# feldroop/floxer

Hardware: AMD Instinct MI355X
Metric: aligned reads/sec, 10 kb ONT-like reads @ 8 % error vs a GRCh38-size reference (seed-and-verify path, CIGAR) (higher is better)
Workload: dtype u64

## Files before the change

floxer_amd/__init__.py:

```python
import ctypes as C

import numpy as np

from . import capi
from .capi import FloxerError, check, lib, ptr, as_u8, u8p, u32p, u64p

if capi.os.path.exists(capi.LIB_PATH):
    lib()

CIGAR_OPS = "MIDNSHP=X"
NULL_ID = 0xFFFFFFFF

ORDER = {"errors_first": 0, "count_first": 1, "none": 2}
CHOICE = {"round_robin": 0, "full_groups": 1, "first_reported": 2}
MODE_EXISTS, MODE_WITHOUT_CIGAR, MODE_WITH_CIGAR = 0, 1, 2


def hw_queue_request():
    requested, found = C.c_int(0), C.c_int(-1)
    check(lib().flx_hw_queue_request(C.byref(requested), C.byref(found)))
    return requested.value, found.value


def cigar_string(words):
# ... 21 lines not shown

def reverse_complement_rank(r):
    r = as_u8(r)
    out = np.zeros_like(r)
    lib().flx_reverse_complement_rank(ptr(r, u8p), len(r), ptr(out, u8p))
    return out


class pex_tree:

    def __init__(self, total_query_length, query_num_errors, leaf_max_num_errors, bottom_up=False):
        cap = 4 * (query_num_errors + 2) + 16
        nodes = (capi.PexNode * cap)()
        ni, nl = C.c_uint64(), C.c_uint64()
        check(lib().flx_pex_tree_build(total_query_length, query_num_errors, leaf_max_num_errors, int(bottom_up), nodes, cap,
                                       C.byref(ni), C.byref(nl)))
        rows = [(n.parent_id, n.from_, n.to, n.num_errors) for n in nodes[: ni.value + nl.value]]
        self.inner_nodes = rows[: ni.value]
        self.leaves = rows[ni.value:]

    def root(self):
        return self.inner_nodes[0] if self.inner_nodes else self.leaves[0]

    def get_leaves(self):
        return self.leaves

    def generate_seeds(self, step=1):
        return [(l[1], l[2] - l[1] + 1, l[3], i) for i, l in enumerate(self.leaves)][::step]


class fmindex:
    def __init__(self, references=None, path=None, device=None):
        self.h = C.c_void_p()
        if path is not None and references is None:
            check(lib().flx_index_load(path.encode(), C.byref(self.h)))
        else:
            refs = [as_u8(r) for r in references]
            pool = np.concatenate(refs) if refs else np.zeros(0, np.uint8)
            lens = np.array([len(r) for r in refs], dtype=np.uint64)
            if device is None:
                check(lib().flx_index_build(ptr(pool, u8p), ptr(lens, u64p), len(refs), C.byref(self.h)))
            else:
                check(lib().flx_index_build_on_device(int(device), ptr(pool, u8p), ptr(lens, u64p), len(refs), C.byref(self.h)))

    def save(self, path):
        check(lib().flx_index_save(self.h, path.encode()))

    def meta(self):
        n = C.c_uint64(0)
        lib().flx_index_meta_export(self.h, None, C.byref(n))
        buf = np.zeros(n.value, dtype=np.uint8)
        check(lib().flx_index_meta_export(self.h, ptr(buf, u8p), C.byref(n)))
        return buf.tobytes()

    @classmethod
    def from_meta(cls, meta):
        self = cls.__new__(cls)
        self.h = C.c_void_p()
        buf = np.frombuffer(meta, dtype=np.uint8).copy()
        check(lib().flx_index_meta_import(ptr(buf, u8p), len(buf), C.byref(self.h)))
        return self

    def image_layout(self):
        out = np.zeros(5, dtype=np.uint64)
        check(lib().flx_index_image_layout(self.h, ptr(out, u64p)))
        return [int(x) for x in out]

    def image_upload(self, device, pointers):
        arr = (C.c_void_p * 5)(*[C.c_void_p(int(p)) for p in pointers])
        check(lib().flx_index_image_upload(self.h, int(device), arr))

    def __del__(self):
        if getattr(self, "h", None):
            lib().flx_index_free(self.h)
            self.h = None

    @property
    def text_length(self):
        return lib().flx_index_text_length(self.h)

    @property
    def num_references(self):
        return lib().flx_index_num_references(self.h)

    @property
    def device_bytes(self):
        return lib().flx_index_device_bytes(self.h)

    @property
    def derived_device_bytes(self):
        return lib().flx_index_derived_device_bytes(self.h)

    def suffix_array(self):
        out = np.zeros(self.text_length, dtype=np.uint64)
        check(lib().flx_index_copy_sa(self.h, ptr(out, u64p)))
        return out

    def suffix_array_u32(self):
        out = np.empty(self.text_length, dtype=np.uint32)
        check(lib().flx_index_copy_sa_u32(self.h, ptr(out, u32p)))
        return out

    def bwt(self, reversed_text=False):
        out = np.zeros(self.text_length, dtype=np.uint8)
        check(lib().flx_index_copy_bwt(self.h, int(reversed_text), ptr(out, u8p)))
        return out


class context:

    def __init__(self, index, device=0, image=None):
        self.index = index
        self.image = image
        self.h = C.c_void_p()
        if image is None:
            check(lib().flx_ctx_create(device, index.h, C.byref(self.h)))
        else:
            arr = (C.c_void_p * 5)(*[C.c_void_p(int(b.data_ptr())) for b in image])
            sizes = np.array([int(b.numel()) * int(b.element_size()) for b in image], dtype=np.uint64)
            check(lib().flx_ctx_create_on_image(device, index.h, arr, ptr(sizes, u64p), C.byref(self.h)))

    def close(self):
        if getattr(self, "h", None):
            lib().flx_ctx_destroy(self.h)
            self.h = None

    __del__ = close

    def set_stream(self, hip_stream):
        check(lib().flx_ctx_set_stream(self.h, hip_stream))

    def enable_kernel_timing(self, on=True):
        check(lib().flx_ctx_enable_kernel_timing(self.h, int(on)))

    def reset_kernel_stats(self):
        check(lib().flx_ctx_reset_kernel_stats(self.h))

    def path_counters(self, reset=False):
        pc = capi.PathCounters()
        check(lib().flx_ctx_get_path_counters(self.h, C.byref(pc)))
        if reset:
            check(lib().flx_ctx_reset_path_counters(self.h))
        out = {n: int(getattr(pc, n)) for n, _ in capi.PathCounters._fields_ if n != "reserved"}
        out["records_dropped"] = int(pc.reserved[0])
        out["partial_records"] = int(pc.reserved[1])
        out["reads_rescued"] = int(pc.reserved[2])
        out["reads_split"] = int(pc.reserved[3])
        return out

    def search_counters(self):
        sc = capi.SearchCounters()
        check(lib().flx_ctx_get_search_counters(self.h, C.byref(sc)))
        return {n: int(getattr(sc, n)) for n, _ in capi.SearchCounters._fields_ if n != "reserved"}

    def derived_info(self):
        di = capi.DerivedInfo()
        check(lib().flx_ctx_derived_info(self.h, C.byref(di)))
        return {n: int(getattr(di, n)) for n, _ in capi.DerivedInfo._fields_ if n != "reserved"}

    def copy_derived(self, which):
        if which == "isa":
            out = np.empty(self.index.text_length, dtype=np.uint32)
        else:
            out = np.empty((4 ** self.derived_info()["filter_k"] + 63) // 64, dtype=np.uint64)
        check(lib().flx_ctx_copy_derived(self.h, {"isa": 0, "filter": 1, "filter_mirrored": 2}[which], out.ctypes.data_as(C.c_void_p), out.nbytes))
        return out

    def lane_overlap(self, n_lanes, iterations):
        start, stop = (C.c_float * n_lanes)(), (C.c_float * n_lanes)()
        check(lib().flx_ctx_lane_overlap(self.h, n_lanes, iterations, start, stop))
        return list(start), list(stop)

    def kernel_stats(self):
        arr = (capi.KernelStat * 64)()
        n = C.c_uint32(64)
        check(lib().flx_ctx_get_kernel_stats(self.h, arr, C.byref(n)))
        return {a.name.decode(): dict(launches=a.launches, device_ms=a.device_ms, algorithmic_bytes=a.algorithmic_bytes,
                                      work_units=a.work_units) for a in arr[: n.value]}


class statistics:

    def __init__(self, input_hint=None):
        self.h = C.c_void_p()
        check(lib().flx_stats_create(input_hint.encode() if input_hint else None, C.byref(self.h)))

    def __del__(self):
        if getattr(self, "h", None):
            lib().flx_stats_free(self.h)
            self.h = None

    def attach(self, ctx):
        check(lib().flx_ctx_set_stats(ctx.h, self.h))
        return self

    @property
    def num_queries(self):
        return lib().flx_stats_num_queries(self.h)

    def format(self, toml=True):
        n = C.c_uint64(0)
        lib().flx_stats_format(self.h, int(toml), None, C.byref(n))
        buf = C.create_string_buffer(n.value)
        check(lib().flx_stats_format(self.h, int(toml), buf, C.byref(n)))
        return buf.value.decode()


def search_config(max_num_anchors_hard=500, max_num_anchors_soft=50, anchor_group_order="count_first",
                  anchor_choice_strategy="round_robin", erase_useless_anchors=True):
    return capi.SearchConfig(max_num_anchors_hard, max_num_anchors_soft, ORDER[anchor_group_order], CHOICE[anchor_choice_strategy],
                             int(erase_useless_anchors), 0)


class searcher:
    def __init__(self, ctx, config=None):
        self.ctx = ctx
        self.config = config or search_config()

    def _seeds(self, seeds):
        arr = (capi.Seed * len(seeds))()
        for i, (off, ln, err, leaf) in enumerate(seeds):
            arr[i] = capi.Seed(off, ln, err, leaf, 0)
        return arr

    def search_seeds(self, sequence, seeds):
        seq = as_u8(sequence)
        arr = self._seeds(seeds)
        cap = max(64, len(seeds) * (self.config.max_num_anchors_soft + 1))
        out = (capi.Anchor * cap)()
        n = C.c_uint64(cap)
        stats = (capi.SeedStats * max(1, len(seeds)))()
        check(lib().flx_search_seeds(self.ctx.h, ptr(seq, u8p), len(seq), arr, len(seeds), C.byref(self.config), out, C.byref(n), stats))
        anchors = np.array([(a.seed_index, a.pex_leaf_index, a.reference_id, a.reference_position, a.num_errors) for a in out[: n.value]],
                           dtype=np.uint64).reshape(-1, 5)
        st = np.array([(s.num_kept_useful_anchors, s.num_kept_raw_anchors, s.num_excluded_raw_anchors_by_soft_cap, s.fully_excluded)
                       for s in stats[: len(seeds)]], dtype=np.uint64).reshape(-1, 4)
        return anchors, st

    def search_groups(self, sequence, seeds, max_hits=501):
        seq = as_u8(sequence)
        arr = self._seeds(seeds)
        cap = 1 << 16
        while True:
            out = (capi.HitGroup * cap)()
            n = C.c_uint64(cap)
            rc = lib().flx_search_groups(self.ctx.h, ptr(seq, u8p), len(seq), arr, len(seeds), max_hits, out, C.byref(n))
            if rc == -3:
                cap = n.value
                continue
            check(rc)
            break
        return np.array([(g.seed_index, g.lb, g.len, g.num_errors) for g in out[: n.value]], dtype=np.uint64).reshape(-1, 4)


def align_batch(ctx, query_pool, jobs, reference_pool=None, md=False, gaps=None):
    q = as_u8(query_pool)
    arr = (capi.AlignJob * max(1, len(jobs)))()
    cap_words = 16
    for i, (ro, rl, qo, ql, k, mode) in enumerate(jobs):
        arr[i] = capi.AlignJob(ro, qo, rl, ql, k, mode)
        cap_words += 2 * k + 2
    res = (capi.AlignResult * max(1, len(jobs)))()
    cig = np.zeros(cap_words, dtype=np.uint32)
    words = C.c_uint64(cap_words)
    if reference_pool is None:
        rp, rl_ = None, 0
    else:
        ref = as_u8(reference_pool)
        rp, rl_ = ptr(ref, u8p), len(ref)
    if md:
        cap_md = 16 + sum(8 * k + 6 for (_, _, _, _, k, mode) in jobs if mode == MODE_WITH_CIGAR)
        refs = (capi.MdRef * max(1, len(jobs)))()
        mdp = np.zeros(cap_md, dtype=np.uint8)
        md_bytes = C.c_uint64(cap_md)
        if gaps is not None:
            check(lib().flx_align_batch_gaps(ctx.h, rp, rl_, ptr(q, u8p), len(q), arr, len(jobs), res, ptr(cig, u32p), C.byref(words),
                                             refs, ptr(mdp, u8p), C.byref(md_bytes), C.byref(gaps)))
        else:
            check(lib().flx_align_batch_md(ctx.h, rp, rl_, ptr(q, u8p), len(q), arr, len(jobs), res, ptr(cig, u32p), C.byref(words),
                                           refs, ptr(mdp, u8p), C.byref(md_bytes)))
        out = []
        for r, m in zip(res[: len(jobs)], refs[: len(jobs)]):
            out.append((r.num_errors, r.begin, cigar_string(cig[r.cigar_offset: r.cigar_offset + r.cigar_length]),
                        mdp[m.offset: m.offset + m.length].tobytes() if m.length else None) if r.exists else None)
        return out
    if gaps is not None:
        check(lib().flx_align_batch_gaps(ctx.h, rp, rl_, ptr(q, u8p), len(q), arr, len(jobs), res, ptr(cig, u32p), C.byref(words),
                                         None, None, None, C.byref(gaps)))
    else:
        check(lib().flx_align_batch(ctx.h, rp, rl_, ptr(q, u8p), len(q), arr, len(jobs), res, ptr(cig, u32p), C.byref(words)))
    out = []
    for r in res[: len(jobs)]:
        out.append((r.num_errors, r.begin, cigar_string(cig[r.cigar_offset: r.cigar_offset + r.cigar_length])) if r.exists else None)
    return out


def _realign_room(options):
    if options is None or not options.enable:
        return (lambda nm: 2 * nm + 2), (lambda nm: 8 * nm + 6)
    sc = {k: int(getattr(options, k)) or v for k, v in REALIGN_DEFAULTS.items()}
    c_max = max(sc["match"] + sc["mismatch"], sc["gap_open"] + sc["gap_extend"] + sc["match"])
    c_min = min(sc["match"] + sc["mismatch"], sc["gap_open"] + sc["gap_extend"])
    col_min = min(sc["match"] + sc["mismatch"], sc["gap_extend"])
    return (lambda nm: max(2 * nm + 2, 2 * (nm * c_max // c_min) + 1)), (lambda nm: 8 * (nm * c_max // col_min) + 6)


# ... 1395 lines not shown
```

floxer_amd/capi.py:

```python
import ctypes as C
import importlib.util
import os
import sys

import numpy as np

_HERE = os.path.dirname(os.path.abspath(__file__))
LIB_PATH = os.environ.get("FLX_LIBRARY") or os.path.join(_HERE, "libfloxer_amd.so")

u8p = C.POINTER(C.c_uint8)
u32p = C.POINTER(C.c_uint32)
u64p = C.POINTER(C.c_uint64)


class FloxerError(RuntimeError):
    pass


class PexNode(C.Structure):
    _fields_ = [("parent_id", C.c_uint32), ("from_", C.c_uint32), ("to", C.c_uint32), ("num_errors", C.c_uint32)]


class Seed(C.Structure):
    _fields_ = [("seq_offset", C.c_uint64), ("length", C.c_uint32), ("num_errors", C.c_uint32), ("pex_leaf_index", C.c_uint32),
# ... 100 lines not shown
    _fields_ = [("offset", C.c_uint64), ("length", C.c_uint32), ("num_errors", C.c_uint32), ("score", C.c_int32), ("diag_lo", C.c_int32),
                ("diag_hi", C.c_int32), ("kept", C.c_uint32)]


class RealignCounters(C.Structure):
    _fields_ = [("paths_realigned", C.c_uint64), ("paths_changed", C.c_uint64), ("paths_kept", C.c_uint64), ("reserved", C.c_uint64 * 5)]


class CsOptions(C.Structure):
    _fields_ = [("form", C.c_uint32), ("reserved", C.c_uint32 * 7)]


CsJob = LeftAlignJob


class CoverageOptions(C.Structure):
    _fields_ = [("count_deletions", C.c_uint32), ("count_secondary", C.c_uint32), ("min_mapq", C.c_uint32), ("report_zero", C.c_uint32),
                ("reserved", C.c_uint32 * 4)]


class DepthRun(C.Structure):
    _fields_ = [("reference_id", C.c_int32), ("depth", C.c_uint32), ("start", C.c_uint64), ("end", C.c_uint64)]


class DepthWindow(C.Structure):
    _fields_ = [("reference_id", C.c_int32), ("max_depth", C.c_uint32), ("start", C.c_uint64), ("end", C.c_uint64), ("depth_sum", C.c_uint64),
                ("covered", C.c_uint64)]


class PileupOptions(C.Structure):
    _fields_ = [("count_secondary", C.c_uint32), ("min_mapq", C.c_uint32), ("min_depth", C.c_uint32), ("min_count", C.c_uint32),
                ("min_permille", C.c_uint32), ("reserved", C.c_uint32 * 3)]


class PileupSite(C.Structure):
    _fields_ = [("reference_id", C.c_int32), ("position", C.c_uint32), ("depth", C.c_uint32), ("del_", C.c_uint32), ("ins", C.c_uint32),
                ("alt", C.c_uint32 * 4), ("reserved", C.c_uint32)]


class SvOptions(C.Structure):
    _fields_ = [("min_length", C.c_uint32), ("max_distance", C.c_uint32), ("min_support", C.c_uint32), ("count_secondary", C.c_uint32),
                ("min_mapq", C.c_uint32), ("reserved", C.c_uint32 * 3), ("initial_capacity", C.c_uint64)]


class SvSignature(C.Structure):
    _fields_ = [("type", C.c_uint32), ("side_a", C.c_uint32), ("side_b", C.c_uint32), ("reserved", C.c_uint32), ("ref_a", C.c_int32),
                ("ref_b", C.c_int32), ("pos_a", C.c_uint32), ("q", C.c_uint32)]


class SvCluster(C.Structure):
    _fields_ = [("type", C.c_uint32), ("side_a", C.c_uint32), ("side_b", C.c_uint32), ("support", C.c_uint32), ("ref_a", C.c_int32),
                ("ref_b", C.c_int32), ("pos_a_min", C.c_uint32), ("pos_a_max", C.c_uint32), ("q_min", C.c_uint32), ("q_median", C.c_uint32),
                ("q_max", C.c_uint32), ("reserved", C.c_uint32)]


class ErrprofOptions(C.Structure):
    _fields_ = [("count_secondary", C.c_uint32), ("min_mapq", C.c_uint32), ("flush_threshold", C.c_uint32), ("reserved", C.c_uint32 * 5)]


class ConsensusOptions(C.Structure):
    _fields_ = [("count_secondary", C.c_uint32), ("min_mapq", C.c_uint32), ("min_depth", C.c_uint32), ("min_count", C.c_uint32),
                ("min_permille", C.c_uint32), ("mask_low_depth", C.c_uint32), ("reserved", C.c_uint32 * 2)]


class ConsensusChange(C.Structure):
    _fields_ = [("reference_id", C.c_int32), ("position", C.c_uint32), ("kind", C.c_uint32), ("ref_rank", C.c_uint32), ("alt_rank", C.c_uint32),
                ("length", C.c_uint32), ("count", C.c_uint32), ("cov", C.c_uint32), ("letters", C.c_uint64)]


class ConsensusAllele(C.Structure):
    _fields_ = [("reference_id", C.c_int32), ("position", C.c_uint32), ("length", C.c_uint32), ("count", C.c_uint32), ("letters", C.c_uint64)]


class VariantsOptions(C.Structure):
    _fields_ = [("count_secondary", C.c_uint32), ("min_mapq", C.c_uint32), ("min_depth", C.c_uint32), ("min_qual", C.c_uint32), ("max_del", C.c_uint32),
                ("cost_match", C.c_uint32), ("cost_mismatch", C.c_uint32), ("cost_het", C.c_uint32), ("prior_het", C.c_uint32), ("prior_hom", C.c_uint32),
                ("reserved", C.c_uint32 * 2)]


class Variant(C.Structure):
    _fields_ = [("reference_id", C.c_int32), ("position", C.c_uint32), ("kind", C.c_uint32), ("ref_rank", C.c_uint32), ("alt_rank", C.c_uint32),
                ("length", C.c_uint32), ("ref_count", C.c_uint32), ("alt_count", C.c_uint32), ("cov", C.c_uint32), ("gt", C.c_uint32), ("gq", C.c_uint32),
                ("qual", C.c_uint32), ("pl", C.c_uint32 * 3), ("reserved", C.c_uint32), ("letters", C.c_uint64)]


class VariantAllele(C.Structure):
    _fields_ = [("reference_id", C.c_int32), ("position", C.c_uint32), ("kind", C.c_uint32), ("length", C.c_uint32), ("count", C.c_uint32),
                ("reserved", C.c_uint32), ("letters", C.c_uint64)]


ERRPROF_SECTIONS = (("PAIR_EQ", 36), ("PAIR_X", 36), ("INS_LEN", 64), ("DEL_LEN", 64), ("INS_LETTER", 6), ("DEL_LETTER", 6), ("HP_DEL", 34), ("HP_INS", 34),
                    ("POS_MATCH", 100), ("POS_MISMATCH", 100), ("POS_INS", 100), ("POS_CLIP", 100), ("POS_DEL", 100), ("EQ_RUN", 256), ("IDENTITY", 101),
                    ("TOTALS", 8), ("reserved", 7))


class ErrprofTable(C.Structure):
    _fields_ = [(name, C.c_uint64 * n) for name, n in ERRPROF_SECTIONS]


class SortOptions(C.Structure):
    _fields_ = [("initial_capacity", C.c_uint64), ("tile_keys", C.c_uint32), ("reserved", C.c_uint32 * 5)]


class SortEntry(C.Structure):
    _fields_ = [("ordinal", C.c_uint64), ("reference_id", C.c_int32), ("position", C.c_int32), ("end", C.c_uint32), ("flag", C.c_uint32)]


class PafSummary(C.Structure):
    _fields_ = [(n, C.c_uint32) for n in ("query_start", "query_end", "ref_end", "matches", "mismatches", "ins_bases", "del_bases", "gap_opens")]


class PafOptions(C.Structure):
    _fields_ = [("write_cigar", C.c_uint32), ("write_unmapped", C.c_uint32), ("mapq_from_records", C.c_uint32), ("skip_secondary", C.c_uint32),
                ("reserved", C.c_uint32 * 4)]


class TailJob(C.Structure):
    _fields_ = [("cigar_offset", C.c_uint64), ("cigar_length", C.c_uint32), ("error_weight", C.c_uint32), ("x_drop", C.c_uint32),
                ("min_tail_rows", C.c_uint32)]


class TailResult(C.Structure):
    _fields_ = [(n, C.c_uint32) for n in ("left_rows", "left_cols", "left_errors", "left_words", "right_rows", "right_cols", "right_errors",
                                          "right_words")]


class ExtendJob(C.Structure):
    _fields_ = [("text_pos", C.c_uint64), ("q_pos", C.c_uint64), ("ref_limit", C.c_uint32), ("row_limit", C.c_uint32),
                ("direction", C.c_int32), ("error_weight", C.c_uint32), ("x_drop", C.c_uint32), ("max_errors", C.c_uint32)]


class ExtendResult(C.Structure):
    _fields_ = [("rows", C.c_uint32), ("cols", C.c_uint32), ("errors", C.c_uint32), ("stop_reason", C.c_uint32)]


class PartialCandidate(C.Structure):
    _fields_ = [("read_index", C.c_uint64), ("q_from", C.c_uint32), ("q_to", C.c_uint32), ("orientation", C.c_uint32),
                ("reference_id", C.c_int32), ("start", C.c_uint64), ("nm", C.c_uint32), ("cigar_length", C.c_uint32),
                ("cigar_offset", C.c_uint64)]


class MdRef(C.Structure):
    _fields_ = [("offset", C.c_uint64), ("length", C.c_uint32), ("reserved", C.c_uint32)]


class PathCounters(C.Structure):
    _fields_ = [(n, C.c_uint64) for n in ("seeds", "seeds_with_anchors", "seeds_excluded_by_hard_cap", "seeds_selected_on_host", "anchors",
                                          "cursor_extensions", "inner_tests_requested", "root_alignments_requested",
                                          "root_alignments_found", "records", "reads", "search_reruns")] + [("reserved", C.c_uint64 * 4)]


class SearchCounters(C.Structure):
    _fields_ = [(n, C.c_uint64) for n in ("launches", "subtrees_queued", "lane_handovers", "wave_handovers", "walks_abandoned")] + [("reserved", C.c_uint64 * 3)]


class ClimbAnchor(C.Structure):
    _fields_ = [("read", C.c_uint32), ("orientation", C.c_uint32), ("leaf", C.c_uint32), ("reference_id", C.c_uint32), ("position", C.c_uint64)]


class ClimbOptions(C.Structure):
    _fields_ = [("driver", C.c_uint32), ("reserved", C.c_uint32 * 3)]


class DerivedInfo(C.Structure):
    _fields_ = [(n, C.c_uint32) for n in ("filter_k", "filter_tmin", "have_isa", "have_filter", "have_filter_mirrored")] + [("reserved", C.c_uint32 * 3)]


class KernelStat(C.Structure):
    _fields_ = [("name", C.c_char * 32), ("launches", C.c_uint64), ("device_ms", C.c_double), ("algorithmic_bytes", C.c_uint64),
                ("work_units", C.c_uint64)]


EXPORTED = [
    "flx_last_error", "flx_version", "flx_ceil_div", "flx_floating_point_error_aware_ceil", "flx_saturate_value_to_int32_max",
    "flx_chars_to_rank_sequence", "flx_reverse_complement_rank", "flx_pex_tree_build", "flx_index_build", "flx_index_build_on_device", "flx_index_save",
    "flx_index_load", "flx_index_free", "flx_index_text_length", "flx_index_num_references", "flx_index_device_bytes", "flx_index_derived_device_bytes",
    "flx_index_copy_sa", "flx_index_copy_sa_u32", "flx_index_copy_bwt", "flx_ctx_create", "flx_ctx_destroy", "flx_ctx_set_stream", "flx_search_seeds",
    "flx_search_groups", "flx_align_batch", "flx_params_default", "flx_align_reads", "flx_reads_upload", "flx_reads_free",
    "flx_align_reads_resident", "flx_run_num_records",
    "flx_run_num_cigar_words", "flx_run_copy", "flx_run_free", "flx_ctx_enable_kernel_timing", "flx_ctx_reset_kernel_stats",
    "flx_ctx_get_kernel_stats", "flx_sam_open", "flx_sam_write", "flx_sam_close", "flx_sim_genome", "flx_sim_genome_repeats", "flx_sim_reads", "flx_ctx_get_path_counters",
    "flx_ctx_reset_path_counters", "flx_stats_create", "flx_stats_free", "flx_stats_merge", "flx_stats_num_queries", "flx_stats_format",
    "flx_ctx_set_stats", "flx_device_count", "flx_index_matches_reference", "flx_sam_set_threads", "flx_index_image_layout",
    "flx_index_image_upload", "flx_index_meta_export", "flx_index_meta_import", "flx_ctx_create_on_image",
    "flx_align_reads_with_options", "flx_align_reads_resident_with_options", "flx_select_records", "flx_assign_mapq", "flx_sam_set_mapq",
    "flx_align_reads_with_tags", "flx_align_reads_resident_with_tags", "flx_run_num_md_bytes", "flx_run_copy_md", "flx_align_batch_md",
    "flx_sam_write_tagged", "flx_align_reads_opt", "flx_align_reads_resident_opt", "flx_choose_partials", "flx_partial_mapq",
    "flx_extend_batch", "flx_sam_set_sa", "flx_align_reads_split", "flx_align_reads_resident_split", "flx_cigar_tails", "flx_cigar_tails_batch",
    "flx_align_shapes", "flx_align_reads_gaps", "flx_align_reads_resident_gaps", "flx_align_batch_gaps", "flx_left_align", "flx_left_align_batch",
    "flx_realign", "flx_realign_batch", "flx_align_batch_realign", "flx_ctx_get_realign_counters", "flx_align_reads_realign",
    "flx_align_reads_resident_realign", "flx_run_copy_scores", "flx_sam_write_scored",
    "flx_ctx_get_search_counters", "flx_climb_anchors", "flx_ctx_derived_info", "flx_ctx_copy_derived",
    "flx_hw_queue_request", "flx_ctx_lane_overlap",
    "flx_align_reads_cs", "flx_align_reads_resident_cs", "flx_run_num_cs_bytes", "flx_run_copy_cs", "flx_align_batch_cs", "flx_cs", "flx_cs_batch",
    "flx_sam_write_cs",
    "flx_coverage_create", "flx_coverage_create_for_lengths", "flx_coverage_free", "flx_coverage_add_run", "flx_coverage_add_records",
    "flx_coverage_absorb", "flx_coverage_finish", "flx_coverage_num_runs", "flx_coverage_copy_runs", "flx_coverage_num_windows",
    "flx_coverage_copy_windows", "flx_coverage_copy_depth", "flx_coverage_geometry", "flx_coverage_host",
    "flx_pileup_create", "flx_pileup_create_for_lengths", "flx_pileup_free", "flx_pileup_add_records", "flx_pileup_add_run",
    "flx_pileup_add_run_resident", "flx_pileup_absorb", "flx_pileup_finish", "flx_pileup_num_sites", "flx_pileup_copy_sites",
    "flx_pileup_copy_counts", "flx_pileup_host", "flx_pileup_sites_host",
    "flx_sort_create", "flx_sort_free", "flx_sort_add_records", "flx_sort_add_run", "flx_sort_finish", "flx_sort_num_records", "flx_sort_copy",
    "flx_sort_geometry", "flx_sort_host", "flx_sam_open_sorted",
    "flx_paf_create", "flx_paf_free", "flx_paf_summarize", "flx_paf_summarize_host", "flx_paf_open", "flx_paf_write", "flx_paf_close",
    "flx_sv_create", "flx_sv_create_for_lengths", "flx_sv_free", "flx_sv_add_records", "flx_sv_add_run", "flx_sv_absorb", "flx_sv_finish",
    "flx_sv_num_signatures", "flx_sv_copy_signatures", "flx_sv_num_clusters", "flx_sv_copy_clusters", "flx_sv_host", "flx_sv_clusters_host",
    "flx_errprof_create", "flx_errprof_create_for_text", "flx_errprof_free", "flx_errprof_add_records", "flx_errprof_add_run",
    "flx_errprof_add_run_resident", "flx_errprof_absorb", "flx_errprof_copy", "flx_errprof_host",
    "flx_consensus_create", "flx_consensus_create_for_text", "flx_consensus_free", "flx_consensus_add_records", "flx_consensus_add_run",
    "flx_consensus_add_run_resident", "flx_consensus_finish", "flx_consensus_num_letters", "flx_consensus_copy_letters",
    "flx_consensus_num_changes", "flx_consensus_copy_changes", "flx_consensus_num_alleles", "flx_consensus_copy_alleles",
    "flx_consensus_geometry", "flx_consensus_host",
    "flx_variants_create", "flx_variants_create_for_text", "flx_variants_free", "flx_variants_add_records", "flx_variants_add_run",
    "flx_variants_add_run_resident", "flx_variants_finish", "flx_variants_num_rows", "flx_variants_copy_rows", "flx_variants_num_alleles",
    "flx_variants_copy_alleles", "flx_variants_geometry", "flx_variants_genotype", "flx_variants_host",
    "flx_grid_caps",
]

_lib = None


def _share_torchs_hip_runtime():
    if os.environ.get("FLX_SYSTEM_HIP") == "1" or "torch" in sys.modules:
        return
    try:
        spec = importlib.util.find_spec("torch")
    except (ImportError, ValueError):
        spec = None
    if spec is None or not spec.origin:
        return
    path = os.path.join(os.path.dirname(spec.origin), "lib", "libamdhip64.so")
    if os.path.exists(path):
        C.CDLL(path, mode=C.RTLD_GLOBAL)


def hip_runtime_paths():
    with open("/proc/self/maps") as f:
        return sorted({line.split()[-1] for line in f if "libamdhip64" in line})


def lib():
    global _lib
    if _lib is not None:
        return _lib
    if not os.path.exists(LIB_PATH):
        raise FloxerError(f"{LIB_PATH} is missing: build it with `python -c 'import __graft_entry__ as g; g.build()'` "
                          "(floxer_amd has no CPU fallback)")
    _share_torchs_hip_runtime()
    L = C.CDLL(LIB_PATH)
    getenv = C.CDLL(None).getenv
    getenv.restype, getenv.argtypes = C.c_char_p, [C.c_char_p]
    value = getenv(b"GPU_MAX_HW_QUEUES")
    if value is None:
        os.environ.pop("GPU_MAX_HW_QUEUES", None)
    else:
        os.environ["GPU_MAX_HW_QUEUES"] = value.decode()
    L.flx_last_error.restype = C.c_char_p
    L.flx_version.restype = C.c_char_p
    L.flx_ceil_div.restype = C.c_uint64
    L.flx_ceil_div.argtypes = [C.c_uint64, C.c_uint64]
    L.flx_floating_point_error_aware_ceil.restype = C.c_uint64
    L.flx_floating_point_error_aware_ceil.argtypes = [C.c_double]
    L.flx_saturate_value_to_int32_max.restype = C.c_int32
    L.flx_saturate_value_to_int32_max.argtypes = [C.c_uint64]
    L.flx_chars_to_rank_sequence.argtypes = [C.c_char_p, C.c_uint64, u8p]
    L.flx_reverse_complement_rank.argtypes = [u8p, C.c_uint64, u8p]
    L.flx_pex_tree_build.argtypes = [C.c_uint64, C.c_uint64, C.c_uint64, C.c_int, C.POINTER(PexNode), C.c_uint64, u64p, u64p]
    L.flx_index_build.argtypes = [u8p, u64p, C.c_uint32, C.POINTER(C.c_void_p)]
    L.flx_index_build_on_device.argtypes = [C.c_int, u8p, u64p, C.c_uint32, C.POINTER(C.c_void_p)]
    L.flx_index_save.argtypes = [C.c_void_p, C.c_char_p]
    L.flx_index_load.argtypes = [C.c_char_p, C.POINTER(C.c_void_p)]
    L.flx_index_free.argtypes = [C.c_void_p]
    L.flx_index_text_length.restype = C.c_uint64
    L.flx_index_text_length.argtypes = [C.c_void_p]
    L.flx_index_num_references.restype = C.c_uint32
    L.flx_index_num_references.argtypes = [C.c_void_p]
    L.flx_index_device_bytes.restype = C.c_uint64
    L.flx_index_device_bytes.argtypes = [C.c_void_p]
    L.flx_index_derived_device_bytes.restype = C.c_uint64
    L.flx_index_derived_device_bytes.argtypes = [C.c_void_p]
    L.flx_index_copy_sa.argtypes = [C.c_void_p, u64p]
    L.flx_index_copy_sa_u32.argtypes = [C.c_void_p, u32p]
    L.flx_index_copy_bwt.argtypes = [C.c_void_p, C.c_int, u8p]
    L.flx_ctx_create.argtypes = [C.c_int, C.c_void_p, C.POINTER(C.c_void_p)]
    L.flx_ctx_destroy.argtypes = [C.c_void_p]
    L.flx_index_image_layout.argtypes = [C.c_void_p, u64p]
    L.flx_index_image_upload.argtypes = [C.c_void_p, C.c_int, C.POINTER(C.c_void_p)]
    L.flx_index_meta_export.argtypes = [C.c_void_p, u8p, u64p]
    L.flx_index_meta_import.argtypes = [u8p, C.c_uint64, C.POINTER(C.c_void_p)]
    L.flx_ctx_create_on_image.argtypes = [C.c_int, C.c_void_p, C.POINTER(C.c_void_p), u64p, C.POINTER(C.c_void_p)]
    L.flx_ctx_set_stream.argtypes = [C.c_void_p, C.c_void_p]
    L.flx_search_seeds.argtypes = [C.c_void_p, u8p, C.c_uint64, C.POINTER(Seed), C.c_uint64, C.POINTER(SearchConfig),
                                   C.POINTER(Anchor), u64p, C.POINTER(SeedStats)]
    L.flx_search_groups.argtypes = [C.c_void_p, u8p, C.c_uint64, C.POINTER(Seed), C.c_uint64, C.c_uint64, C.POINTER(HitGroup), u64p]
    L.flx_align_batch.argtypes = [C.c_void_p, u8p, C.c_uint64, u8p, C.c_uint64, C.POINTER(AlignJob), C.c_uint64,
                                  C.POINTER(AlignResult), u32p, u64p]
    L.flx_align_shapes.argtypes = [C.POINTER(AlignJob), C.c_uint64, C.POINTER(AlignShape)]
    L.flx_params_default.argtypes = [C.POINTER(Params)]
    L.flx_align_reads.argtypes = [C.c_void_p, C.POINTER(Params), u8p, u64p, C.c_uint64, C.POINTER(C.c_void_p)]
    L.flx_reads_upload.argtypes = [C.c_void_p, u8p, u64p, C.c_uint64, C.POINTER(C.c_void_p)]
    L.flx_reads_free.argtypes = [C.c_void_p]
    L.flx_align_reads_resident.argtypes = [C.c_void_p, C.POINTER(Params), C.c_void_p, C.POINTER(C.c_void_p)]
    L.flx_align_reads_with_options.argtypes = [C.c_void_p, C.POINTER(Params), u8p, u64p, C.c_uint64, C.POINTER(OutputOptions),
                                               C.POINTER(C.c_void_p)]
    L.flx_align_reads_resident_with_options.argtypes = [C.c_void_p, C.POINTER(Params), C.c_void_p, C.POINTER(OutputOptions),
                                                        C.POINTER(C.c_void_p)]
    L.flx_align_reads_with_tags.argtypes = [C.c_void_p, C.POINTER(Params), u8p, u64p, C.c_uint64, C.POINTER(OutputOptions),
                                            C.POINTER(TagOptions), C.POINTER(C.c_void_p)]
    L.flx_align_reads_resident_with_tags.argtypes = [C.c_void_p, C.POINTER(Params), C.c_void_p, C.POINTER(OutputOptions),
                                                     C.POINTER(TagOptions), C.POINTER(C.c_void_p)]
    L.flx_align_reads_opt.argtypes = [C.c_void_p, C.POINTER(Params), u8p, u64p, C.c_uint64, C.POINTER(RunOptions), C.POINTER(C.c_void_p)]
    L.flx_align_reads_resident_opt.argtypes = [C.c_void_p, C.POINTER(Params), C.c_void_p, C.POINTER(RunOptions), C.POINTER(C.c_void_p)]
    L.flx_align_reads_split.argtypes = [C.c_void_p, C.POINTER(Params), u8p, u64p, C.c_uint64, C.POINTER(RunOptions), C.POINTER(SplitOptions),
                                        C.POINTER(C.c_void_p)]
    L.flx_align_reads_resident_split.argtypes = [C.c_void_p, C.POINTER(Params), C.c_void_p, C.POINTER(RunOptions), C.POINTER(SplitOptions),
                                                 C.POINTER(C.c_void_p)]
    L.flx_align_reads_gaps.argtypes = [C.c_void_p, C.POINTER(Params), u8p, u64p, C.c_uint64, C.POINTER(RunOptions), C.POINTER(SplitOptions),
                                       C.POINTER(GapOptions), C.POINTER(C.c_void_p)]
    L.flx_align_reads_resident_gaps.argtypes = [C.c_void_p, C.POINTER(Params), C.c_void_p, C.POINTER(RunOptions), C.POINTER(SplitOptions),
                                                C.POINTER(GapOptions), C.POINTER(C.c_void_p)]
    L.flx_align_batch_gaps.argtypes = [C.c_void_p, u8p, C.c_uint64, u8p, C.c_uint64, C.POINTER(AlignJob), C.c_uint64,
                                       C.POINTER(AlignResult), u32p, u64p, C.POINTER(MdRef), u8p, u64p, C.POINTER(GapOptions)]
    L.flx_left_align.argtypes = [u8p, C.c_uint64, u8p, C.c_uint64, u32p, C.c_uint64, C.POINTER(LeftAlignJob), C.c_uint64, u32p, u64p,
                                 C.POINTER(CigarRef)]
    L.flx_left_align_batch.argtypes = [C.c_void_p] + L.flx_left_align.argtypes
    L.flx_realign.argtypes = [u8p, C.c_uint64, u8p, C.c_uint64, u32p, C.c_uint64, C.POINTER(RealignJob), C.c_uint64, C.POINTER(RealignOptions), u32p, u64p,
                              C.POINTER(RealignResult)]
    L.flx_realign_batch.argtypes = [C.c_void_p] + L.flx_realign.argtypes
    L.flx_align_batch_realign.argtypes = L.flx_align_batch_gaps.argtypes + [C.POINTER(RealignOptions), C.POINTER(C.c_int32)]
    L.flx_ctx_get_realign_counters.argtypes = [C.c_void_p, C.POINTER(RealignCounters)]
    L.flx_align_reads_realign.argtypes = L.flx_align_reads_gaps.argtypes[:-1] + [C.POINTER(RealignOptions), C.POINTER(C.c_void_p)]
    L.flx_align_reads_resident_realign.argtypes = L.flx_align_reads_resident_gaps.argtypes[:-1] + [C.POINTER(RealignOptions), C.POINTER(C.c_void_p)]
    L.flx_run_copy_scores.argtypes = [C.c_void_p, C.POINTER(C.c_int32)]
    L.flx_align_reads_cs.argtypes = L.flx_align_reads_realign.argtypes[:-1] + [C.POINTER(CsOptions), C.POINTER(C.c_void_p)]
    L.flx_align_reads_resident_cs.argtypes = L.flx_align_reads_resident_realign.argtypes[:-1] + [C.POINTER(CsOptions), C.POINTER(C.c_void_p)]
    L.flx_run_num_cs_bytes.restype = C.c_uint64
    L.flx_run_num_cs_bytes.argtypes = [C.c_void_p]
    L.flx_run_copy_cs.argtypes = [C.c_void_p, C.POINTER(MdRef), u8p]
    L.flx_align_batch_cs.argtypes = L.flx_align_batch_realign.argtypes + [C.POINTER(CsOptions), C.POINTER(MdRef), u8p, u64p]
    L.flx_cs.argtypes = [u8p, C.c_uint64, u8p, C.c_uint64, u32p, C.c_uint64, C.POINTER(CsJob), C.c_uint64, C.POINTER(CsOptions), u8p, u64p,
                         C.POINTER(MdRef)]
    L.flx_cs_batch.argtypes = [C.c_void_p] + L.flx_cs.argtypes
    L.flx_coverage_create.argtypes = [C.c_void_p, C.POINTER(CoverageOptions), C.POINTER(C.c_void_p)]
    L.flx_coverage_create_for_lengths.argtypes = [C.c_int, u64p, C.c_uint32, C.POINTER(CoverageOptions), C.POINTER(C.c_void_p)]
    L.flx_coverage_free.restype = None
# ... 7 lines not shown
    L.flx_coverage_copy_runs.argtypes = [C.c_void_p, C.POINTER(DepthRun), C.c_uint64]
    L.flx_coverage_num_windows.restype = C.c_uint64
    L.flx_coverage_num_windows.argtypes = [C.c_void_p, C.c_uint64]
    L.flx_coverage_copy_windows.argtypes = [C.c_void_p, C.c_uint64, C.POINTER(DepthWindow), C.c_uint64]
    L.flx_coverage_copy_depth.argtypes = [C.c_void_p, C.c_uint32, C.c_uint64, C.c_uint64, u32p]
    L.flx_coverage_geometry.argtypes = [u32p]
    L.flx_coverage_host.argtypes = [u64p, C.c_uint32, C.POINTER(CoverageOptions), C.POINTER(Record), C.c_uint64, u32p, C.c_uint64, u32p]
    L.flx_sort_create.argtypes = [C.c_int, C.c_uint32, C.POINTER(SortOptions), C.POINTER(C.c_void_p)]
    L.flx_sort_free.restype = None
    L.flx_sort_free.argtypes = [C.c_void_p]
    L.flx_sort_add_records.argtypes = [C.c_void_p, C.POINTER(Record), C.c_uint64, u32p, C.c_uint64, C.c_uint64, u32p]
    L.flx_sort_add_run.argtypes = [C.c_void_p, C.c_void_p, C.c_uint64, u32p]
    L.flx_sort_finish.argtypes = [C.c_void_p]
    L.flx_sort_num_records.restype = C.c_uint64
    L.flx_sort_num_records.argtypes = [C.c_void_p]
    L.flx_sort_copy.argtypes = [C.c_void_p, C.c_uint64, C.c_uint64, C.POINTER(SortEntry)]
    L.flx_sort_geometry.argtypes = [u32p]
    L.flx_grid_caps.argtypes = [u32p]
    L.flx_sort_host.argtypes = [C.c_uint32, C.POINTER(Record), C.c_uint64, u32p, C.c_uint64, u64p, C.POINTER(SortEntry)]
    L.flx_pileup_create.argtypes = [C.c_void_p, C.POINTER(PileupOptions), C.POINTER(C.c_void_p)]
    L.flx_pileup_create_for_lengths.argtypes = [C.c_int, u64p, C.c_uint32, C.POINTER(PileupOptions), C.POINTER(C.c_void_p)]
    L.flx_pileup_free.restype = None
    L.flx_pileup_free.argtypes = [C.c_void_p]
    L.flx_pileup_add_records.argtypes = [C.c_void_p, C.POINTER(Record), C.c_uint64, u32p, C.c_uint64, u8p, u64p, C.c_uint64]
    L.flx_pileup_add_run.argtypes = [C.c_void_p, C.c_void_p, u8p, u64p, C.c_uint64]
    L.flx_pileup_add_run_resident.argtypes = [C.c_void_p, C.c_void_p, C.c_void_p]
    L.flx_pileup_absorb.argtypes = [C.c_void_p, C.c_void_p]
    L.flx_pileup_finish.argtypes = [C.c_void_p]
    L.flx_pileup_num_sites.restype = C.c_uint64
    L.flx_pileup_num_sites.argtypes = [C.c_void_p]
    L.flx_pileup_copy_sites.argtypes = [C.c_void_p, C.POINTER(PileupSite), C.c_uint64]
    L.flx_pileup_copy_counts.argtypes = [C.c_void_p, C.c_uint32, C.c_uint64, C.c_uint64, u32p]
    L.flx_pileup_host.argtypes = [u64p, C.c_uint32, C.POINTER(PileupOptions), C.POINTER(Record), C.c_uint64, u32p, C.c_uint64, u8p, u64p, C.c_uint64, u32p]
    L.flx_pileup_sites_host.argtypes = [u64p, C.c_uint32, C.POINTER(PileupOptions), u32p, C.POINTER(PileupSite), u64p]
    L.flx_sv_create.argtypes = [C.c_void_p, C.POINTER(SvOptions), C.POINTER(C.c_void_p)]
    L.flx_sv_create_for_lengths.argtypes = [C.c_int, u64p, C.c_uint32, C.POINTER(SvOptions), C.POINTER(C.c_void_p)]
    L.flx_sv_free.restype = None
    L.flx_sv_free.argtypes = [C.c_void_p]
    L.flx_sv_add_records.argtypes = [C.c_void_p, C.POINTER(Record), C.c_uint64, u32p, C.c_uint64, u64p, C.c_uint64]
    L.flx_sv_add_run.argtypes = [C.c_void_p, C.c_void_p, u64p, C.c_uint64]
    L.flx_sv_absorb.argtypes = [C.c_void_p, C.c_void_p]
    L.flx_sv_finish.argtypes = [C.c_void_p]
    L.flx_sv_num_signatures.restype = C.c_uint64
    L.flx_sv_num_signatures.argtypes = [C.c_void_p]
    L.flx_sv_copy_signatures.argtypes = [C.c_void_p, C.c_uint64, C.c_uint64, C.POINTER(SvSignature)]
    L.flx_sv_num_clusters.restype = C.c_uint64
    L.flx_sv_num_clusters.argtypes = [C.c_void_p]
    L.flx_sv_copy_clusters.argtypes = [C.c_void_p, C.POINTER(SvCluster), C.c_uint64]
    L.flx_sv_host.argtypes = [u64p, C.c_uint32, C.POINTER(SvOptions), C.POINTER(Record), C.c_uint64, u32p, C.c_uint64, u64p, C.c_uint64,
                              C.POINTER(SvSignature), u64p]
    L.flx_sv_clusters_host.argtypes = [C.POINTER(SvOptions), C.POINTER(SvSignature), C.c_uint64, C.POINTER(SvCluster), u64p]
    L.flx_errprof_create.argtypes = [C.c_void_p, C.POINTER(ErrprofOptions), C.POINTER(C.c_void_p)]
    L.flx_errprof_create_for_text.argtypes = [C.c_int, u8p, u64p, C.c_uint32, C.POINTER(ErrprofOptions), C.POINTER(C.c_void_p)]
    L.flx_errprof_free.restype = None
    L.flx_errprof_free.argtypes = [C.c_void_p]
    L.flx_errprof_add_records.argtypes = [C.c_void_p, C.POINTER(Record), C.c_uint64, u32p, C.c_uint64, u8p, u64p, C.c_uint64]
    L.flx_errprof_add_run.argtypes = [C.c_void_p, C.c_void_p, u8p, u64p, C.c_uint64]
    L.flx_errprof_add_run_resident.argtypes = [C.c_void_p, C.c_void_p, C.c_void_p]
    L.flx_errprof_absorb.argtypes = [C.c_void_p, C.c_void_p]
    L.flx_errprof_copy.argtypes = [C.c_void_p, C.POINTER(ErrprofTable)]
    L.flx_errprof_host.argtypes = [u8p, u64p, C.c_uint32, C.POINTER(ErrprofOptions), C.POINTER(Record), C.c_uint64, u32p, C.c_uint64, u8p, u64p, C.c_uint64,
                                   C.POINTER(ErrprofTable)]
    L.flx_consensus_create.argtypes = [C.c_void_p, C.POINTER(ConsensusOptions), C.POINTER(C.c_void_p)]
    L.flx_consensus_create_for_text.argtypes = [C.c_int, u8p, u64p, C.c_uint32, C.POINTER(ConsensusOptions), C.POINTER(C.c_void_p)]
    L.flx_consensus_free.restype = None
    L.flx_consensus_free.argtypes = [C.c_void_p]
    L.flx_consensus_add_records.argtypes = [C.c_void_p, C.POINTER(Record), C.c_uint64, u32p, C.c_uint64, u8p, u64p, C.c_uint64]
    L.flx_consensus_add_run.argtypes = [C.c_void_p, C.c_void_p, u8p, u64p, C.c_uint64]
    L.flx_consensus_add_run_resident.argtypes = [C.c_void_p, C.c_void_p, C.c_void_p]
    L.flx_consensus_finish.argtypes = [C.c_void_p]
    L.flx_consensus_num_letters.restype = C.c_uint64
    L.flx_consensus_num_letters.argtypes = [C.c_void_p, C.c_uint32]
    L.flx_consensus_copy_letters.argtypes = [C.c_void_p, C.c_uint32, C.c_char_p, C.c_uint64]
    L.flx_consensus_num_changes.restype = C.c_uint64
    L.flx_consensus_num_changes.argtypes = [C.c_void_p]
    L.flx_consensus_copy_changes.argtypes = [C.c_void_p, C.POINTER(ConsensusChange), C.c_uint64]
    L.flx_consensus_num_alleles.restype = C.c_uint64
    L.flx_consensus_num_alleles.argtypes = [C.c_void_p]
    L.flx_consensus_copy_alleles.argtypes = [C.c_void_p, C.POINTER(ConsensusAllele), C.c_uint64]
    L.flx_consensus_geometry.argtypes = [u32p]
    L.flx_consensus_host.argtypes = [u8p, u64p, C.c_uint32, C.POINTER(ConsensusOptions), C.POINTER(Record), C.c_uint64, u32p, C.c_uint64, u8p, u64p, C.c_uint64,
                                     u64p, C.c_char_p, u64p, C.POINTER(ConsensusChange), u64p, C.POINTER(ConsensusAllele), u64p]
    L.flx_variants_create.argtypes = [C.c_void_p, C.POINTER(VariantsOptions), C.POINTER(C.c_void_p)]
    L.flx_variants_create_for_text.argtypes = [C.c_int, u8p, u64p, C.c_uint32, C.POINTER(VariantsOptions), C.POINTER(C.c_void_p)]
    L.flx_variants_free.restype = None
    L.flx_variants_free.argtypes = [C.c_void_p]
    L.flx_variants_add_records.argtypes = [C.c_void_p, C.POINTER(Record), C.c_uint64, u32p, C.c_uint64, u8p, u64p, C.c_uint64]
    L.flx_variants_add_run.argtypes = [C.c_void_p, C.c_void_p, u8p, u64p, C.c_uint64]
    L.flx_variants_add_run_resident.argtypes = [C.c_void_p, C.c_void_p, C.c_void_p]
    L.flx_variants_finish.argtypes = [C.c_void_p]
    L.flx_variants_num_rows.restype = C.c_uint64
    L.flx_variants_num_rows.argtypes = [C.c_void_p]
    L.flx_variants_copy_rows.argtypes = [C.c_void_p, C.POINTER(Variant), C.c_uint64]
    L.flx_variants_num_alleles.restype = C.c_uint64
    L.flx_variants_num_alleles.argtypes = [C.c_void_p]
    L.flx_variants_copy_alleles.argtypes = [C.c_void_p, C.POINTER(VariantAllele), C.c_uint64]
    L.flx_variants_geometry.argtypes = [u32p]
    L.flx_variants_genotype.argtypes = [C.POINTER(VariantsOptions), C.c_uint64, C.c_uint64, C.c_uint64, u32p]
    L.flx_variants_host.argtypes = [u8p, u64p, C.c_uint32, C.POINTER(VariantsOptions), C.POINTER(Record), C.c_uint64, u32p, C.c_uint64, u8p, u64p, C.c_uint64,
                                    C.POINTER(Variant), u64p, C.POINTER(VariantAllele), u64p]
    L.flx_paf_create.argtypes = [C.c_int, C.POINTER(C.c_void_p)]
    L.flx_paf_free.restype = None
    L.flx_paf_free.argtypes = [C.c_void_p]
    L.flx_paf_summarize.argtypes = [C.c_void_p, C.POINTER(Record), C.c_uint64, u32p, C.c_uint64, u64p, C.c_uint64, u64p, C.c_uint32, C.POINTER(PafSummary)]
    L.flx_paf_summarize_host.argtypes = [C.POINTER(Record), C.c_uint64, u32p, C.c_uint64, u64p, C.c_uint64, u64p, C.c_uint32, C.POINTER(PafSummary)]
    L.flx_paf_open.argtypes = [C.c_char_p, C.POINTER(C.c_char_p), u64p, C.c_uint32, C.POINTER(PafOptions), C.POINTER(C.c_void_p)]
    L.flx_paf_write.argtypes = [C.c_void_p, C.POINTER(C.c_char_p), u64p, C.POINTER(Record), C.c_uint64, u32p, C.POINTER(PafSummary), C.POINTER(C.c_int32),
                                C.POINTER(MdRef), u8p]
    L.flx_paf_close.argtypes = [C.c_void_p]
    L.flx_cigar_tails.argtypes = [u32p, C.c_uint64, C.POINTER(TailJob), C.c_uint64, C.POINTER(TailResult)]
    L.flx_cigar_tails_batch.argtypes = [C.c_void_p, u32p, C.c_uint64, C.POINTER(TailJob), C.c_uint64, C.POINTER(TailResult)]
    L.flx_choose_partials.argtypes = [C.POINTER(PartialCandidate), C.c_uint64, u32p, C.POINTER(PartialOptions), C.POINTER(C.c_int32)]
    L.flx_partial_mapq.argtypes = [C.POINTER(PartialCandidate), C.c_uint64, u32p, C.POINTER(C.c_int32), u8p]
    L.flx_run_num_md_bytes.restype = C.c_uint64
    L.flx_run_num_md_bytes.argtypes = [C.c_void_p]
    L.flx_run_copy_md.argtypes = [C.c_void_p, C.POINTER(MdRef), u8p]
    L.flx_align_batch_md.argtypes = [C.c_void_p, u8p, C.c_uint64, u8p, C.c_uint64, C.POINTER(AlignJob), C.c_uint64,
                                     C.POINTER(AlignResult), u32p, u64p, C.POINTER(MdRef), u8p, u64p]
    L.flx_sam_write_tagged.argtypes = [C.c_void_p, C.POINTER(C.c_char_p), u8p, u64p, C.POINTER(C.c_char_p), C.POINTER(Record), C.c_uint64, u32p,
                                       C.POINTER(MdRef), u8p]
    L.flx_sam_write_scored.argtypes = L.flx_sam_write_tagged.argtypes + [C.POINTER(C.c_int32)]
    L.flx_sam_write_cs.argtypes = L.flx_sam_write_scored.argtypes + [C.POINTER(MdRef), u8p]
    L.flx_select_records.argtypes = [C.POINTER(Record), C.c_uint64, u32p, C.POINTER(OutputOptions), u8p]
    L.flx_assign_mapq.argtypes = [C.POINTER(Record), C.c_uint64, u32p, u64p, u8p]
    L.flx_run_num_records.restype = C.c_uint64
    L.flx_run_num_records.argtypes = [C.c_void_p]
    L.flx_run_num_cigar_words.restype = C.c_uint64
    L.flx_run_num_cigar_words.argtypes = [C.c_void_p]
    L.flx_run_copy.argtypes = [C.c_void_p, C.POINTER(Record), u32p, u8p]
    L.flx_run_free.argtypes = [C.c_void_p]
    L.flx_ctx_enable_kernel_timing.argtypes = [C.c_void_p, C.c_int]
    L.flx_ctx_reset_kernel_stats.argtypes = [C.c_void_p]
    L.flx_ctx_get_kernel_stats.argtypes = [C.c_void_p, C.POINTER(KernelStat), u32p]
    L.flx_sam_open.argtypes = [C.c_char_p, C.POINTER(C.c_char_p), u64p, C.c_uint32, C.POINTER(C.c_void_p)]
    L.flx_sam_write.argtypes = [C.c_void_p, C.POINTER(C.c_char_p), u8p, u64p, C.POINTER(C.c_char_p), C.POINTER(Record), C.c_uint64, u32p]
    L.flx_sam_close.argtypes = [C.c_void_p]
    L.flx_sam_open_sorted.argtypes = [C.c_char_p, C.c_char_p, C.c_int, C.c_int, C.POINTER(C.c_char_p), u64p, C.c_uint32, C.POINTER(C.c_void_p)]
    L.flx_stats_create.argtypes = [C.c_char_p, C.POINTER(C.c_void_p)]
    L.flx_stats_free.argtypes = [C.c_void_p]
    L.flx_stats_merge.argtypes = [C.c_void_p, C.c_void_p]
    L.flx_stats_num_queries.restype = C.c_uint64
    L.flx_stats_num_queries.argtypes = [C.c_void_p]
    L.flx_stats_format.argtypes = [C.c_void_p, C.c_int, C.c_char_p, u64p]
    L.flx_ctx_set_stats.argtypes = [C.c_void_p, C.c_void_p]
    L.flx_device_count.restype = C.c_int
    L.flx_index_matches_reference.argtypes = [C.c_void_p, u8p, u64p, C.c_uint32]
    L.flx_sam_set_threads.argtypes = [C.c_void_p, C.c_uint32]
    L.flx_sam_set_mapq.argtypes = [C.c_void_p, C.c_int]
    L.flx_sam_set_sa.argtypes = [C.c_void_p, C.c_int]
    L.flx_extend_batch.argtypes = [C.c_void_p, u8p, C.c_uint64, u8p, C.c_uint64, C.POINTER(ExtendJob), C.c_uint64, C.POINTER(ExtendResult)]
    L.flx_ctx_get_path_counters.argtypes = [C.c_void_p, C.POINTER(PathCounters)]
    L.flx_ctx_reset_path_counters.argtypes = [C.c_void_p]
    L.flx_ctx_get_search_counters.argtypes = [C.c_void_p, C.POINTER(SearchCounters)]
    L.flx_climb_anchors.argtypes = [C.c_void_p, C.POINTER(Params), C.c_void_p, C.c_void_p, C.c_uint64, C.POINTER(ClimbOptions), u8p, u32p, u64p]
    L.flx_ctx_derived_info.argtypes = [C.c_void_p, C.POINTER(DerivedInfo)]
    L.flx_ctx_copy_derived.argtypes = [C.c_void_p, C.c_int, C.c_void_p, C.c_uint64]
    L.flx_hw_queue_request.argtypes = [C.POINTER(C.c_int), C.POINTER(C.c_int)]
    L.flx_ctx_lane_overlap.argtypes = [C.c_void_p, C.c_uint32, C.c_uint32, C.POINTER(C.c_float), C.POINTER(C.c_float)]
    L.flx_sim_genome.argtypes = [C.c_uint64, C.c_uint64, u8p]
    L.flx_sim_genome_repeats.argtypes = [C.c_uint64, C.c_uint64, u8p]
    L.flx_sim_reads.argtypes = [u8p, u64p, C.c_uint32, C.c_uint64, C.c_uint32, C.c_double, C.c_double, C.c_uint64, u8p, C.c_uint64,
                                u64p, u32p, u64p, u8p]
    _lib = L
    return L


def check(rc):
    if rc != 0:
        raise FloxerError(f"floxer_amd error {rc}: {lib().flx_last_error().decode()}")


def ptr(a, t):
    return a.ctypes.data_as(t)


def as_u8(x):
    return np.ascontiguousarray(np.asarray(x, dtype=np.uint8))
```

floxer_amd/csrc/flx_capi.cpp:

```cpp
#include <algorithm>
#include <cstdlib>
#include <cstring>
#include <malloc.h>
#include <memory>
#include <mutex>
#include <thread>

#include "flx_context.hpp"
#include "flx_fm_core.hpp"

namespace flx {
const char* last_error_cstr();
}
using namespace flx;

extern "C" {

int flx_index_build_on_device(int hip_device, const uint8_t* concat, const uint64_t* lens, uint32_t n_refs, flx_index** out) {
    if (!concat || !lens || !out || n_refs == 0) { set_error("flx_index_build_on_device: null argument or no reference"); return FLX_ERR_INVALID; }
    int count = 0;
    if (hipGetDeviceCount(&count) != hipSuccess || count <= 0) { (void)hipGetLastError(); set_error("flx_index_build_on_device: no HIP device"); return FLX_ERR_NO_DEVICE; }
    if (hip_device < 0 || hip_device >= count) { set_error("flx_index_build_on_device: device ordinal out of range"); return FLX_ERR_INVALID; }
    HostIndex* h = build_host_index(concat, lens, n_refs, hip_device);
    if (!h) return FLX_ERR_INVALID;
// ... 126 lines not shown
        (void)DeviceApi::derived_bytes(H.n, &fk);
        bool have_isa = false;
        {
            size_t free_i = 0, total_i = 0;
            FLX_HIP(hipMemGetInfo(&free_i, &total_i));
            size_t const want = (size_t)H.n * 4 + 64;
            have_isa = want < free_i / 2 && ctx->isa.ensure(want, true) == FLX_OK;
        }
        bool have_filter = false, have_filter_m = false;
        if (fk) {
            size_t free_f = 0, total_f = 0;
            FLX_HIP(hipMemGetInfo(&free_f, &total_f));
            size_t const want = (size_t)(((1ull << (2 * fk)) + 63) / 64) * 8;
            have_filter = want < free_f / 2 && ctx->filter.ensure(want, true) == FLX_OK;
            if (have_filter && getenv("FLX_MIRRORED_FILTER")) {
                FLX_HIP(hipMemGetInfo(&free_f, &total_f));
                have_filter_m = want < free_f / 2 && ctx->filter_m.ensure(want, true) == FLX_OK;
            }
        }
        int const e = DeviceApi::derive_index(s0, ctx->didx, have_isa ? ctx->isa.as<u32>() : nullptr, have_filter ? ctx->filter.as<u64>() : nullptr, have_filter_m ? ctx->filter_m.as<u64>() : nullptr);
        if (e) { set_error(std::string("derive_index: ") + hipGetErrorString((hipError_t)e)); return FLX_ERR_NO_DEVICE; }
        FLX_HIP(hipStreamSynchronize(s0));
    }
    if (getenv("FLX_ALLOC_DEBUG"))
        fprintf(stderr, "[flx alloc] context: occ0 %p occ1 %p sa %p text %p kmer %p (n %llu) isa %p filter %p (K %u, tmin %u) seq_start %p\n", img[0], img[1], img[2], img[3],
                img[4], (unsigned long long)H.n, ctx->isa.ptr, ctx->filter.ptr, ctx->didx.filter_k, ctx->didx.filter_tmin, ctx->seq_start.ptr);
    for (auto& lane : ctx->lanes) {
        int const e = DeviceApi::warm_scratch(lane->stream);
        if (e) { set_error(std::string("warm_scratch: ") + hipGetErrorString((hipError_t)e)); return FLX_ERR_NO_DEVICE; }
    }
    for (auto& lane : ctx->lanes) FLX_HIP(hipStreamSynchronize(lane->stream));
    size_t free_b = 0, total_b = 0;
    FLX_HIP(hipMemGetInfo(&free_b, &total_b));
    size_t budget = std::min<size_t>(free_b / 10 * 4, n_lanes * ((size_t)4 << 30));
    if (const char* env = getenv("FLX_TRACE_ARENA_MB")) { size_t const mb = strtoull(env, nullptr, 10); if (mb) budget = mb << 20; }
    budget = std::max<size_t>(budget, (size_t)256 << 20);
    for (auto& lane : ctx->lanes) lane->trace_budget_bytes = std::max<size_t>(budget / n_lanes, (size_t)128 << 20);
    if (const char* env = getenv("FLX_TRACE_ARENA_KB")) { size_t const kb = strtoull(env, nullptr, 10); if (kb) for (auto& lane : ctx->lanes) lane->trace_budget_bytes = kb << 10; }
    *out = ctx.release();
    return FLX_OK;
}
}

int flx_ctx_create(int hip_device, const flx_index* index, flx_ctx** out) {
    if (!index || !out) { set_error("flx_ctx_create: null argument"); return FLX_ERR_INVALID; }
    if (int const rc = check_device(hip_device, "flx_ctx_create")) return rc;
    if (!has_arrays(*index->host)) { set_error("flx_ctx_create: this index holds no arrays (flx_index_meta_import): use flx_ctx_create_on_image"); return FLX_ERR_INVALID; }
    return make_context(hip_device, index, nullptr, true, out);
}

int flx_ctx_create_on_image(int hip_device, const flx_index* index, void* const device_buffers[5], const flx_index_image* sizes, flx_ctx** out) {
    if (!index || !out || !device_buffers || !sizes) { set_error("flx_ctx_create_on_image: null argument"); return FLX_ERR_INVALID; }
    for (int i = 0; i < 5; ++i) if (!device_buffers[i]) { set_error("flx_ctx_create_on_image: null device buffer"); return FLX_ERR_INVALID; }
    {
        uint64_t want[5];
        image_sizes(*index->host, want);
        for (int i = 0; i < 5; ++i)
            if (sizes->bytes[i] != want[i]) { set_error("flx_ctx_create_on_image: the buffers' sizes are not this index's image layout (flx_index_image_layout)"); return FLX_ERR_INVALID; }
    }
    if (int const rc = check_device(hip_device, "flx_ctx_create_on_image")) return rc;
    return make_context(hip_device, index, device_buffers, false, out);
}

int flx_index_image_layout(const flx_index* index, flx_index_image* out) {
    if (!index || !out) { set_error("flx_index_image_layout: null argument"); return FLX_ERR_INVALID; }
    image_sizes(*index->host, out->bytes);
    return FLX_OK;
}

int flx_index_image_upload(const flx_index* index, int hip_device, void* const device_buffers[5]) {
    if (!index || !device_buffers) { set_error("flx_index_image_upload: null argument"); return FLX_ERR_INVALID; }
    if (!has_arrays(*index->host)) { set_error("flx_index_image_upload: this index holds no arrays"); return FLX_ERR_INVALID; }
    if (int const rc = check_device(hip_device, "flx_index_image_upload")) return rc;
    FLX_HIP(hipSetDevice(hip_device));
    return upload_image(*index->host, device_buffers, nullptr);
}

flx_ctx::~flx_ctx() {
    (void)hipSetDevice(device);
    for (auto& lane : lanes) { if (lane->stream) (void)hipStreamSynchronize(lane->stream); lane->release_all(); }
    for (DeviceBuffer* b : {&occ0, &occ1, &sa, &text, &text_rev, &kmer, &seq_start, &isa, &filter}) b->release();
    if (upload_stream) (void)hipStreamDestroy(upload_stream);
}

int flx_ctx_destroy(flx_ctx* ctx) {
    if (!ctx) return FLX_OK;
    {
        std::lock_guard<std::mutex> g(ctx->spare_mu);
        if (ctx->live_reads > 0) { set_error("flx_ctx_destroy: " + std::to_string(ctx->live_reads) + " read batch(es) of this context are still alive (flx_reads_free them first)"); return FLX_ERR_INVALID; }
        if (ctx->live_errprofs > 0) { set_error("flx_ctx_destroy: " + std::to_string(ctx->live_errprofs) + " error-profile object(s) of this context are still alive (flx_errprof_free them first)"); return FLX_ERR_INVALID; }
        if (ctx->live_consensus > 0) { set_error("flx_ctx_destroy: " + std::to_string(ctx->live_consensus) + " consensus object(s) of this context are still alive (flx_consensus_free them first)"); return FLX_ERR_INVALID; }
        if (ctx->live_variants > 0) { set_error("flx_ctx_destroy: " + std::to_string(ctx->live_variants) + " variants object(s) of this context are still alive (flx_variants_free them first)"); return FLX_ERR_INVALID; }
    }
    delete ctx;
    return FLX_OK;
}

int flx_ctx_set_stream(flx_ctx* ctx, void* hip_stream) {
    if (!ctx) { set_error("null context"); return FLX_ERR_INVALID; }
    int rc = ctx->sync_all();
    if (rc) return rc;
    Lane* l0 = ctx->lane0();
    l0->stream = hip_stream ? (hipStream_t)hip_stream : l0->own_stream;
    ctx->external_stream = hip_stream != nullptr;
    return FLX_OK;
}

int flx_ctx_enable_kernel_timing(flx_ctx* ctx, int enable) {
    if (!ctx) { set_error("null context"); return FLX_ERR_INVALID; }
    int rc = ctx->sync_all();
    if (rc) return rc;
    ctx->timing = enable != 0;
    return FLX_OK;
}
int flx_ctx_reset_kernel_stats(flx_ctx* ctx) {
    if (!ctx) { set_error("null context"); return FLX_ERR_INVALID; }
    int rc = ctx->sync_all();
    if (rc) return rc;
    std::lock_guard<std::mutex> g(ctx->mu);
    ctx->stats.clear();
    ctx->stat_order.clear();
    return FLX_OK;
}
int flx_ctx_get_kernel_stats(flx_ctx* ctx, flx_kernel_stat* out, uint32_t* n) {
    if (!ctx || !n) { set_error("null argument"); return FLX_ERR_INVALID; }
    int rc = ctx->sync_all();
    if (rc) return rc;
    std::lock_guard<std::mutex> g(ctx->mu);
    uint32_t const cap = *n;
    *n = (uint32_t)ctx->stat_order.size();
    if (ctx->stat_order.size() > cap || (!out && cap)) { set_error("stat buffer too small"); return FLX_ERR_CAPACITY; }
    for (size_t i = 0; i < ctx->stat_order.size(); ++i) out[i] = ctx->stats[ctx->stat_order[i]];
    return FLX_OK;
}

int flx_ctx_set_stats(flx_ctx* ctx, flx_stats* stats) {
    if (!ctx) { set_error("null context"); return FLX_ERR_INVALID; }
    int const rc = ctx->sync_all();
    if (rc) return rc;
    ctx->read_stats = stats;
    return FLX_OK;
}
int flx_ctx_get_path_counters(flx_ctx* ctx, flx_path_counters* out) {
    if (!ctx || !out) { set_error("null argument"); return FLX_ERR_INVALID; }
    std::lock_guard<std::mutex> g(ctx->mu);
    *out = ctx->path;
    return FLX_OK;
}
int flx_ctx_reset_path_counters(flx_ctx* ctx) {
    if (!ctx) { set_error("null context"); return FLX_ERR_INVALID; }
    std::lock_guard<std::mutex> g(ctx->mu);
    ctx->path = flx_path_counters{};
    ctx->search = flx_search_counters{};
    ctx->realign = flx_realign_counters{};
    return FLX_OK;
}
int flx_ctx_get_realign_counters(flx_ctx* ctx, flx_realign_counters* out) {
    if (!ctx || !out) { set_error("null argument"); return FLX_ERR_INVALID; }
    std::lock_guard<std::mutex> g(ctx->mu);
    *out = ctx->realign;
    return FLX_OK;
}
int flx_ctx_get_search_counters(flx_ctx* ctx, flx_search_counters* out) {
    if (!ctx || !out) { set_error("null argument"); return FLX_ERR_INVALID; }
    std::lock_guard<std::mutex> g(ctx->mu);
    *out = ctx->search;
    return FLX_OK;
}

int flx_ctx_derived_info(flx_ctx* ctx, flx_derived_info* out) {
    if (!ctx || !out) { set_error("flx_ctx_derived_info: null argument"); return FLX_ERR_INVALID; }
    *out = flx_derived_info{};
    out->filter_k = ctx->didx.filter_k;
    out->filter_tmin = ctx->didx.filter_tmin;
    out->have_isa = ctx->didx.isa != nullptr;
    out->have_filter = ctx->didx.filter != nullptr;
    out->have_filter_mirrored = ctx->didx.filter_m != nullptr;
    return FLX_OK;
}
int flx_ctx_copy_derived(flx_ctx* ctx, int which, void* out, uint64_t bytes) {
    if (!ctx || !out) { set_error("flx_ctx_copy_derived: null argument"); return FLX_ERR_INVALID; }
    const void* src = nullptr;
    uint64_t want = 0;
    switch (which) {
        case 0: src = ctx->didx.isa; want = (uint64_t)ctx->didx.n * 4; break;
        case 1: src = ctx->didx.filter; want = filter_words(ctx->didx.filter_k) * 8; break;
        case 2: src = ctx->didx.filter_m; want = filter_words(ctx->didx.filter_k) * 8; break;
        default: set_error("flx_ctx_copy_derived: which must be 0 (inverse suffix array), 1 (filter) or 2 (mirrored filter)"); return FLX_ERR_INVALID;
    }
    if (!src) { set_error("flx_ctx_copy_derived: this context has no such table"); return FLX_ERR_INVALID; }
    if (bytes != want) { set_error("flx_ctx_copy_derived: the table holds " + std::to_string(want) + " bytes, the caller gave " + std::to_string(bytes)); return FLX_ERR_INVALID; }
    FLX_HIP(hipSetDevice(ctx->device));
    FLX_HIP(hipMemcpy(out, src, want, hipMemcpyDeviceToHost));
    return FLX_OK;
}

int flx_ctx_lane_overlap(flx_ctx* ctx, uint32_t n_lanes, uint32_t iterations, float* start_ms, float* stop_ms) {
    if (!ctx || !start_ms || !stop_ms) { set_error("flx_ctx_lane_overlap: null argument"); return FLX_ERR_INVALID; }
    if (n_lanes == 0 || n_lanes > ctx->lanes.size()) { set_error("flx_ctx_lane_overlap: the context has " + std::to_string(ctx->lanes.size()) + " lanes, the caller asked for " + std::to_string(n_lanes)); return FLX_ERR_INVALID; }
    for (uint32_t l = 0; l < n_lanes; ++l)
        if (!ctx->lanes[l]->own_stream) { set_error("flx_ctx_lane_overlap: lane " + std::to_string(l) + " has no stream of its own (FLX_STREAMS)"); return FLX_ERR_INVALID; }
    iterations = std::min<uint32_t>(iterations, 1u << 24);
    int rc = ctx->sync_all();
    if (rc) return rc;
    FLX_HIP(hipSetDevice(ctx->device));
    struct Probe {
        hipEvent_t ref = nullptr;
        std::vector<hipEvent_t> a, b;
        u32* out = nullptr;
        ~Probe() {
            for (hipEvent_t e : a) if (e) (void)hipEventDestroy(e);
            for (hipEvent_t e : b) if (e) (void)hipEventDestroy(e);
            if (ref) (void)hipEventDestroy(ref);
            if (out) (void)hipFree(out);
        }
    } p;
    p.a.assign(n_lanes, nullptr);
    p.b.assign(n_lanes, nullptr);
    FLX_HIP(hipEventCreate(&p.ref));
    for (uint32_t l = 0; l < n_lanes; ++l) { FLX_HIP(hipEventCreate(&p.a[l])); FLX_HIP(hipEventCreate(&p.b[l])); }
    FLX_HIP(hipMalloc((void**)&p.out, (size_t)n_lanes * 64 * sizeof(u32)));
    FLX_HIP(hipEventRecord(p.ref, ctx->lanes[0]->own_stream));
    for (uint32_t l = 0; l < n_lanes && !rc; ++l) {
        hipStream_t const s = ctx->lanes[l]->own_stream;
        FLX_HIP(hipEventRecord(p.a[l], s));
        rc = DeviceApi::lane_overlap_probe(s, iterations, p.out + (size_t)l * 64);
        FLX_HIP(hipEventRecord(p.b[l], s));
    }
    for (uint32_t l = 0; l < n_lanes; ++l) FLX_HIP(hipStreamSynchronize(ctx->lanes[l]->own_stream));
    if (rc) { set_error(std::string("lane_overlap_probe: ") + hipGetErrorString((hipError_t)rc)); return FLX_ERR_NO_DEVICE; }
    for (uint32_t l = 0; l < n_lanes; ++l) {
        FLX_HIP(hipEventElapsedTime(&start_ms[l], p.ref, p.a[l]));
        FLX_HIP(hipEventElapsedTime(&stop_ms[l], p.ref, p.b[l]));
    }
    return FLX_OK;
}

}
```

floxer_amd/csrc/flx_context.hpp:

```cpp
#pragma once

#include <hip/hip_runtime.h>

#include <condition_variable>
#include <map>
#include <memory>
#include <mutex>
#include <string>
#include <vector>

#include "flx_internal.hpp"

namespace flx {

#define FLX_HIP(expr)                                                                                   \
    do {                                                                                                \
        hipError_t const e__ = (expr);                                                                  \
        if (e__ != hipSuccess) {                                                                        \
            set_error(std::string(#expr) + ": " + hipGetErrorString(e__));                              \
            return FLX_ERR_NO_DEVICE;                                                                   \
        }                                                                                               \
    } while (0)

#define FLX_LAUNCH(name, rc)                                                                            \
    do {                                                                                                \
        int const e__ = (rc);                                                                           \
        if (e__ != 0) {                                                                                 \
            set_error(std::string(name) + ": launch failed: " + hipGetErrorString((hipError_t)e__));    \
            return FLX_ERR_NO_DEVICE;                                                                   \
        }                                                                                               \
    } while (0)

struct DeviceBuffer {
    void* ptr = nullptr;
    size_t cap = 0;
    DeviceBuffer() = default;
    DeviceBuffer(DeviceBuffer const&) = delete;
    DeviceBuffer& operator=(DeviceBuffer const&) = delete;
    ~DeviceBuffer() { release(); }
    int ensure(size_t bytes, bool exact = false);
    void release();
    void take(DeviceBuffer& other) { release(); ptr = other.ptr; cap = other.cap; other.ptr = nullptr; other.cap = 0; }
    template <class T> T* as() const { return reinterpret_cast<T*>(ptr); }
};

struct PinnedBuffer {
    void* ptr = nullptr;
    size_t cap = 0;
    PinnedBuffer() = default;
    PinnedBuffer(PinnedBuffer const&) = delete;
    PinnedBuffer& operator=(PinnedBuffer const&) = delete;
    ~PinnedBuffer() { release(); }
    int ensure(size_t bytes);
    void release();
};

struct PendingTiming { std::string name; hipEvent_t start, stop; u64 bytes, units; };

}


struct flx_ctx;
struct flx_stats;

namespace flx {
struct Lane {
    flx_ctx* ctx = nullptr;
    int id = 0;
    hipStream_t own_stream = nullptr, stream = nullptr;
    DeviceBuffer seq, seq_rev, peq, peq_rev, scheme, seeds, stack, hits, counters, rows, rows_out, qpack, items;
    DeviceBuffer jobs, job_out, trace, tjobs, tjob_out, cigar, md, md_out, user_text, user_text_rev, lastrow, row_windows, row_out,
        seed_cnt, hit_off, grouped, sel_stat, sel_n, sel_off, sel_out, sel_tmp, sel_rows, sel_row_off, sel_sparse, sel_lists, vr, seed_gen, mailboxes, ext_jobs, ext_out, tail_jobs, tail_out, cigar_la, la_jobs, la_stat, cigar_ra, ra_jobs, ra_stat, cs, cs_jobs, cs_out;
    size_t trace_budget_bytes = 0;
    std::vector<PendingTiming> pending;
    std::vector<hipEvent_t> event_pool;
    hipEvent_t sync_event = nullptr;
    u32* vr_host_scalars = nullptr;
    PinnedBuffer staging;
    void* stage_begin(size_t bytes);
    PinnedBuffer results;
    size_t results_used = 0;
    static constexpr size_t RESULT_BLOCK_BYTES = 1u << 20;
    size_t results_limit = RESULT_BLOCK_BYTES;
    bool results_limit_read = false;
    void* result_slot(size_t bytes);
    bool has_run = false;
    double hits_per_seed = 0, items_per_seed = 0, sel_rows_per_seed = 0;
    int wait_idle();
    int sync();
    std::vector<DeviceBuffer*> workspaces();
    int size_like(Lane& other);
    hipEvent_t get_event();
    void release_all();
};
}

struct flx_ctx {
    ~flx_ctx();
    int device = 0;
    const flx::HostIndex* hidx = nullptr;
    flx::DevIndex didx{};
    flx::DeviceBuffer occ0, occ1, sa, text, text_rev, kmer, seq_start;
    flx::DeviceBuffer isa, filter, filter_m;
    bool text_rev_ready = false;
    std::mutex mu;
    std::vector<std::unique_ptr<flx::Lane>> lanes;
    hipStream_t upload_stream = nullptr;
    std::mutex spare_mu;
    std::vector<std::unique_ptr<flx::DeviceBuffer>> spare_read_buffers[5];
    int live_reads = 0;
    int live_errprofs = 0;
    int live_consensus = 0;
    int live_variants = 0;
    bool external_stream = false;
    bool timing = false;
    std::map<std::string, flx_kernel_stat> stats;
    std::vector<std::string> stat_order;
    flx_path_counters path{};
    flx_realign_counters realign{};
    flx_search_counters search{};
    flx_stats* read_stats = nullptr;

    std::mutex lane_mu;
    std::condition_variable lane_cv;
    std::vector<int> free_lanes;
    flx::Lane* acquire_lane(int wanted = -1);
    void release_lane(flx::Lane* lane);
    void warm_one_cold_lane(flx::Lane* like);

    int k1_tokens = 0;
    int k1_running = 0;
    void k1_acquire();
    void k1_release();

    flx::Lane* lane0() { return lanes[0].get(); }
    int sync_all();
    void account(const char* name, flx::u64 bytes, flx::u64 units, hipEvent_t start, hipEvent_t stop);
    void account_more(const char* name, flx::u64 bytes, flx::u64 units);
};

namespace flx {

struct LaneLease {
    flx_ctx* ctx;
    Lane* lane;
    explicit LaneLease(flx_ctx* c, int wanted = -1) : ctx(c), lane(c->acquire_lane(wanted)) {}
    ~LaneLease() { ctx->release_lane(lane); }
    LaneLease(LaneLease const&) = delete;
    LaneLease& operator=(LaneLease const&) = delete;
};

struct ResultScope {
    Lane* lane;
    size_t mark;
    explicit ResultScope(Lane* l) : lane(l), mark(l->results_used) {}
    ~ResultScope() { lane->results_used = mark; }
    ResultScope(ResultScope const&) = delete;
    ResultScope& operator=(ResultScope const&) = delete;
};

template <class F>
int timed_launch(Lane* lane, const char* name, u64 bytes, u64 units, F&& launch) {
    if (!lane->ctx->timing) {
        FLX_LAUNCH(name, launch());
        return FLX_OK;
    }
    hipEvent_t const a = lane->get_event(), b = lane->get_event();
    FLX_HIP(hipEventRecord(a, lane->stream));
    int const rc = launch();
    FLX_HIP(hipEventRecord(b, lane->stream));
    FLX_LAUNCH(name, rc);
    lane->pending.push_back(PendingTiming{name, a, b, bytes, units});
    return FLX_OK;
}

}
```

floxer_amd/csrc/flx_device.hip:

```cpp
#include <hip/hip_runtime.h>

#include <algorithm>
#include <cstdio>
#include <cstdlib>
#include <type_traits>
#include <utility>

#include "flx_internal.hpp"
#include "flx_wave.hpp"

namespace flx {

__device__ __forceinline__ u32 wave_max_u32(u32 v) {
#pragma unroll
    for (int off = 32; off > 0; off >>= 1) {
        u32 const o = (u32)__shfl_xor((int)v, off);
        v = v > o ? v : o;
    }
    return (u32)__builtin_amdgcn_readfirstlane((int)v);
}

__global__ void __launch_bounds__(256) peq_build_kernel(const u8* __restrict__ seq, u64 len, u64* __restrict__ peq, u64 n_words) {
    u64 const wave = ((u64)blockIdx.x * blockDim.x + threadIdx.x) >> 6;
    if (wave >= n_words) return;
    u64 const pos = wave * 64 + lane_id();
    u32 const sym = pos < len ? seq[pos] : 7u;
#pragma unroll
    for (u32 s = 0; s < 6; ++s) {
        u64 const m = __ballot(sym == s);
        if (lane_id() == s) peq[wave * 6 + s] = m;
    }
}

int DeviceApi::build_peq(void* stream, const u8* d_seq, u64 len, u64* d_peq) {
    u64 const n_words = len / 64 + 2;
    u64 const threads = n_words * 64;
    hipLaunchKernelGGL(peq_build_kernel, dim3((unsigned)((threads + 255) / 256)), dim3(256), 0, (hipStream_t)stream, d_seq, len,
                       d_peq, n_words);
    return (int)hipGetLastError();
}

static const u32 kWordsPerLane[] = {1, 2, 3, 4, 5, 6, 8, 13, 25};

template <int W, bool TRACE>
__device__ __forceinline__ void ed_block_body(const u8* __restrict__ text, const u64* __restrict__ peq, const DevAlignJob* __restrict__ jobs, u32 n_jobs,
                                              u32 log2_r, DevAlignOut* __restrict__ out, u32 blk, u64* __restrict__ lds_eq,
                                              u64* __restrict__ trace, u16* __restrict__ lastrow, u32 queue, u32* __restrict__ err) {
    u32 const lane = lane_id();
    u32 const R = 1u << log2_r;
    u32 const p = lane & (R - 1u);
    u32 const jobs_per_wave = 64u >> log2_r;
    u32 const job_id = blk * jobs_per_wave + (lane >> log2_r);
    bool valid = job_id < n_jobs;
    DevAlignJob job;
    if (valid) job = jobs[job_id];
    else { job.ref_off = 0; job.q_off = 0; job.trace_off = 0; job.n = 0; job.m = 1; job.k = 0; job.out_index = 0; }
    int const n = (int)job.n, m = (int)job.m, k = (int)job.k;
    if (valid && (n == 0 || n + k < m)) {
        if (p == 0u) { DevAlignOut o; o.score = (n == 0 && m <= k) ? (u32)m : 0xFFFFFFFFu; o.end_col = 0u; out[job.out_index] = o; }
        valid = false;
    }
    int const nw = (m + 63) >> 6;
    int const Lg = (nw + W - 1) / W;
    int const band_hi = n - m + k;
    u32 const src_lane = (lane & ~(R - 1u)) | ((lane - 1u) & (R - 1u));
    int delay = valid ? (int)ring_delay((u32)n, (u32)m, (u32)k, (u32)W, R) : 0;
    if (delay > 0 && (u32)delay + 1u > queue) {
        if (err && p == 0u) atomicOr(err, 1u);
        if (p == 0u) { DevAlignOut o; o.score = 0xFFFFFFFFu; o.end_col = 0u; out[job.out_index] = o; }
        valid = false;
        delay = 0;
    }
    bool const any_delay = __any(delay > 0);
    uint2* __restrict__ const hand = reinterpret_cast<uint2*>(lds_eq + 7u * 64u * W) + (size_t)(lane >> log2_r) * queue;
    u32 const qmask = queue - 1u;
    auto offset_of = [&](int gg) { return gg + (gg >> log2_r) * delay; };
#pragma unroll
    for (int w = 0; w < W; ++w) lds_eq[(6u * 64u + lane) * W + w] = 0ull;

    int const pad = Lg * 64 * W - m;
    int g = (int)p;
    int b_lo = 0, b_hi = -1, rows_g = 0;
    int above_b_hi = 0;
    int off_g = 0;
    u64 vp[W], vn[W];
    auto enter_group = [&]() {
        int const r0 = max(0, 64 * W * g - pad);
        int const r1 = 64 * W * (g + 1) - pad;
        rows_g = r1 - r0;
        b_lo = max(0, r0 - k) >> 4;
        b_hi = min(n - 1, r1 - 1 + band_hi) >> 4;
        if (g + 1 < Lg) b_hi = max(b_hi, max(0, r1 - k) >> 4);
        above_b_hi = max(min(n - 1, r0 - 1 + band_hi) >> 4, b_lo);
        off_g = offset_of(g);
#pragma unroll
        for (int w = 0; w < W; ++w) {
            int const rs = 64 * (g * W + w) - pad;
            u64 const padmask = rs <= -64 ? ~0ull : rs < 0 ? (1ull << (u32)(-rs)) - 1ull : 0ull;
            i64 const off = (i64)job.q_off + rs;
#pragma unroll
            for (u32 s = 0; s < 6; ++s) {
                u64 v = 0;
                if (rs > -64) {
                    if (off >= 0) {
                        u64 const a = (u64)off >> 6;
                        u32 const sh = (u32)off & 63u;
                        u64 const lo = peq[a * 6 + s];
                        u64 const hi = peq[(a + 1) * 6 + s];
                        v = sh ? (lo >> sh) | (hi << (64 - sh)) : lo;
                    } else v = peq[s] << (u32)(-off);
                }
                lds_eq[(s * 64u + lane) * W + w] = v | padmask;
            }
            lds_eq[(6u * 64u + lane) * W + w] = padmask;
            vp[w] = ~padmask;
            vn[w] = 0ull;
        }
    };
    bool const has_group = valid && g < Lg;
    if (has_group) enter_group();
    else {
#pragma unroll
        for (int w = 0; w < W; ++w) { vp[w] = ~0ull; vn[w] = 0ull; }
    }
    u32 const my_steps = valid ? (u32)(((n - 1) >> 4) + offset_of(Lg - 1) + 1) : 0u;
    u32 const t_max = wave_max_u32(my_steps);
    const u8* __restrict__ ref = text + job.ref_off;
    u32* __restrict__ carry_out = nullptr;
    ulonglong2* __restrict__ ckpt_out = nullptr;
    if (TRACE) {
        TraceLayout const tl = ckpt_trace_layout(job.n, job.m, job.k, (u32)W, R);
        carry_out = reinterpret_cast<u32*>(reinterpret_cast<ulonglong2*>(trace) + job.trace_off);
        ckpt_out = reinterpret_cast<ulonglong2*>(trace) + job.trace_off + tl.carry_slots;
    }

    u32 cw_out = 0x55555555u;
    int botv_out = 0;
    int bot = 0, best = m, best_col = 0;
    uint4 tq_pre = make_uint4(0, 0, 0, 0);
    int pre_b = -1;
    bool pend = false, pend_last = false;
    u64 pend_slot = 0;
    int pend_b = 0;
    u32 cbits[W];
    u32 rowv[8];
    auto flush = [&]() {
        if (TRACE && pend) {
#pragma unroll
            for (int w = 0; w < W; ++w) carry_out[pend_slot + w] = cbits[w];
            if (pend_last && lastrow) {
                uint4* __restrict__ dst = reinterpret_cast<uint4*>(lastrow + job.lastrow_off + 16 * (u64)pend_b);
                dst[0] = make_uint4(rowv[0], rowv[1], rowv[2], rowv[3]);
                dst[1] = make_uint4(rowv[4], rowv[5], rowv[6], rowv[7]);
            }
            pend = false;
        }
    };
    for (u32 T = 0; T < t_max; ++T) {
        int b = (int)T - off_g;
        if (has_group && b > b_hi && g + (int)R < Lg) {
            g += (int)R;
            enter_group();
            b = (int)T - off_g;
        }
        u32 cw_in = (u32)__shfl((int)cw_out, (int)src_lane);
        int botv_in = __shfl(botv_out, (int)src_lane);
        if (any_delay) {
            if (delay > 0 && p == R - 1u) hand[(T - 1u) & qmask] = make_uint2(cw_out, (u32)botv_out);
            if (delay > 0 && p == 0u && g >= (int)R) { uint2 const h = hand[(T - 1u - (u32)delay) & qmask]; cw_in = h.x; botv_in = (int)h.y; }
        }
        bool const active = has_group && b >= b_lo && b <= b_hi;
        if (active) {
            if (g == 0) { cw_in = 0u; botv_in = 0; }
            else if (b > above_b_hi) cw_in = 0x55555555u;
            if (b == b_lo) bot = botv_in + rows_g;
            int const bot_start = bot;
            bool const last = g == Lg - 1;
            uint4 tq = tq_pre;
            if (pre_b != b) __builtin_memcpy(&tq, ref + 16 * b, 16);
            u32 const quad[4] = {tq.x, tq.y, tq.z, tq.w};
            u32 cw = 0;
            u64 const slot = ((u64)T * R + p) * W;
            flush();
            if (TRACE) {
#pragma unroll
                for (int w = 0; w < W; ++w) {
                    ulonglong2 v;
                    v.x = vp[w];
                    v.y = vn[w];
                    ckpt_out[slot + w] = v;
                    cbits[w] = 0;
                }
#pragma unroll
                for (int q = 0; q < 8; ++q) rowv[q] = 0xFFFFFFFFu;
            }
            if (b < b_hi) { __builtin_memcpy(&tq_pre, ref + 16 * (b + 1), 16); pre_b = b + 1; }
            auto block16 = [&](auto track_tag) {
                constexpr bool TRACK = decltype(track_tag)::value;
                u32 qv[4] = {quad[0], quad[1], quad[2], quad[3]};
                u32 cwi = cw_in;
                int bb = b;
                asm volatile("" : "+v"(qv[0]), "+v"(qv[1]), "+v"(qv[2]), "+v"(qv[3]), "+v"(cwi), "+v"(bb));
                u32 acc = 0;
#pragma unroll
                for (int qd = 0; qd < 4; ++qd) {
                    __builtin_amdgcn_sched_barrier(0);
#pragma unroll
                    for (int i = 0; i < 4; ++i) {
                        int const j = 4 * qd + i;
                        int const c = 16 * bb + j;
                        u32 sym = (qv[qd] >> (8 * i)) & 0xFFu;
                        sym = c < n ? sym : 6u;
                        u64 c_hp = (cwi >> (2 * j)) & 1u, c_hn = (cwi >> (2 * j + 1)) & 1u;
                        const u64* __restrict__ eqp = &lds_eq[(sym * 64u + lane) * W];
                        u64 hp_last = 0, hn_last = 0;
#pragma unroll
                        for (int w = 0; w < W; ++w) {
                            if (TRACE) cbits[w] |= ((u32)c_hp | ((u32)c_hn << 1)) << (2 * j);
                            u64 const eq = eqp[w];
                            u64 const pv = vp[w], mv = vn[w];
                            u64 const x = eq | mv;
                            u64 const tt = pv + (x & pv) + c_hn;
                            u64 const d0 = (tt ^ pv) | x;
                            u64 const hn = pv & d0;
                            u64 const hp = mv | ~(pv | d0);
                            u64 const xh = (hp << 1) | c_hp;
                            vn[w] = xh & d0;
                            vp[w] = (hn << 1) | ~(xh | d0) | c_hn;
                            if (w + 1 < W || TRACK) { c_hp = hp >> 63; c_hn = hn >> 63; }
                            if (w + 1 == W) { hp_last = hp; hn_last = hn; }
                        }
                        if (TRACK) {
                            acc |= ((u32)c_hp | ((u32)c_hn << 1)) << (2 * j);
                            bot += (int)(u32)c_hp - (int)(u32)c_hn;
                            if (last && c < n && bot <= best) { best = bot; best_col = c + 1; }
                            if (TRACE && c < n) {
                                u32 const v16 = (u32)min(bot, 0xFFFF);
                                rowv[j >> 1] = (j & 1) ? (rowv[j >> 1] & 0xFFFFu) | (v16 << 16) : (rowv[j >> 1] & 0xFFFF0000u) | v16;
                            }
                        } else {
                            acc = (acc >> 2) | (((u32)(hp_last >> 32) >> 1) & 0x40000000u) | ((u32)(hn_last >> 32) & 0x80000000u);
                        }
                    }
                }
                if (!TRACK) bot += (int)__popc(acc & 0x55555555u) - (int)__popc(acc & 0xAAAAAAAAu);
                return acc;
            };
            cw = __any(last) ? block16(std::true_type{}) : block16(std::false_type{});
            if (TRACE) { pend = true; pend_last = last; pend_slot = slot; pend_b = b; }
            cw_out = cw;
            botv_out = bot_start;
        } else {
            cw_out = 0x55555555u;
            botv_out = 0;
        }
    }
    flush();
    if (valid && has_group && g == Lg - 1) {
        DevAlignOut o;
        o.score = best <= k ? (u32)best : 0xFFFFFFFFu;
        o.end_col = (u32)best_col;
        out[job.out_index] = o;
    }
}


template <int W>
__global__ void __launch_bounds__(64, (W <= 2 ? 4 : W <= 5 ? 3 : W <= 8 ? 2 : 1)) ed_exists_block_kernel(const u8* __restrict__ text, const u64* __restrict__ peq,
                                                             const DevAlignJob* __restrict__ jobs, u32 n_jobs, u32 log2_r,
                                                             DevAlignOut* __restrict__ out, const u32* __restrict__ n_jobs_dev, u32 queue, u32* __restrict__ err) {
    extern __shared__ __attribute__((aligned(16))) u64 lds_eq[];
    if (n_jobs_dev) n_jobs = min(n_jobs, *n_jobs_dev);
    u32 const jobs_per_wave = 64u >> log2_r;
    for (u32 blk = blockIdx.x; blk * jobs_per_wave < n_jobs; blk += gridDim.x)
        ed_block_body<W, false>(text, peq, jobs, n_jobs, log2_r, out, blk, lds_eq, nullptr, nullptr, queue, err);
}

template <int W>
__global__ void __launch_bounds__(64, (W <= 4 ? 3 : W <= 6 ? 2 : 1)) ed_trace_block_kernel(const u8* __restrict__ text, const u64* __restrict__ peq,
                                                            const DevAlignJob* __restrict__ jobs, u32 n_jobs, u32 log2_r,
                                                            u64* __restrict__ trace, DevAlignOut* __restrict__ out, u16* __restrict__ lastrow, u32 queue) {
    extern __shared__ __attribute__((aligned(16))) u64 lds_eq[];
    __builtin_amdgcn_s_setprio(2);
    ed_block_body<W, true>(text, peq, jobs, n_jobs, log2_r, out, blockIdx.x, lds_eq, trace, lastrow, queue, nullptr);
}

static u64 shape_width_cap(u32 nw, AlignShape sh) {
    u32 const w = sh.words_per_lane, r = sh.lanes_per_job;
    if ((nw + w - 1) / w <= r) return 0xFFFFFFFFull;
    u64 const no_wait = (u64)64 * w * (r - 1) + r;
    if (sh.queue < 8) return no_wait;
    return no_wait + 16ull * (sh.queue - 5u);
}
u64 DeviceApi::shape_width_cap(u32 nw, AlignShape sh) { return flx::shape_width_cap(nw, sh); }

static AlignShape choose_align_shape_uncached(u32 n, u32 m, u32 k, bool parallel) {
    u32 const nw = (m + 63) / 64;
    i64 const width = (i64)n - (i64)m + 2 * (i64)k;
    static int const stretch = [] { const char* e = getenv("FLX_RING_STRETCH"); int const v = e ? atoi(e) : 135; return v < 100 ? 100 : v; }();
    bool const may_wait = !parallel && stretch > 100;
    AlignShape best{0, 0};
    u64 best_cost = ~0ull;
    u64 shortest = ~0ull, shortest_key = ~0ull;
    for (int pass = 0; pass < (may_wait ? 2 : 1); ++pass)
    for (u32 w : kWordsPerLane)
        for (u32 r = 1; r <= 64; r *= 2) {
            u32 const groups = (nw + w - 1) / w;
            bool ok = groups <= r;
            if (!ok) ok = (i64)64 * w * (r - 1) + r + 1 > width;
            u32 delay = 0;
            if (!ok && may_wait && pass == 1) {
                delay = ring_delay(n, m, k, w, r);
                ok = delay + 1u <= RING_QUEUE_MAX;
            }
            if (!ok) continue;
            u64 const steps = ring_steps(n, m, k, w, r);
            if (pass == 0 && may_wait) { u64 const key = (u64)w * r * 1000 + w; if (key < shortest_key) { shortest_key = key; shortest = steps; } continue; }
            u64 cost;
            if (may_wait) {
                if (steps * 100 > shortest * (u64)stretch) continue;
                cost = steps * r * (8 * w + 1);
            } else cost = parallel ? (u64)w * 1000 + r : (u64)w * r * 1000 + w;
            if (cost < best_cost) { best_cost = cost; best = AlignShape{w, r, ring_queue_for(delay)}; }
        }
    return best;
}

AlignShape choose_align_shape(u32 n, u32 m, u32 k, bool parallel) {
    u32 const nw = (m + 63) / 64;
    i64 const width = (i64)n - (i64)m + 2 * (i64)k;
    if (const char* forced = getenv("FLX_FORCE_SHAPE")) {
        u32 w = 0, r = 0;
        if (sscanf(forced, "%u,%u", &w, &r) == 2 && w && r) {
            if ((nw + w - 1) / w <= r || (i64)64 * w * (r - 1) + r + 1 > width) return AlignShape{w, r};
            u32 const delay = ring_delay(n, m, k, w, r);
            if (delay + 1u <= RING_QUEUE_MAX) return AlignShape{w, r, ring_queue_for(delay)};
        }
    }
    struct Entry { u32 n, m, k; AlignShape shape; bool valid; };
    thread_local Entry memo[2][256] = {};
    Entry& e = memo[parallel ? 1 : 0][(m * 31u + n * 7u + k) & 255u];
    if (e.valid && e.n == n && e.m == m && e.k == k) return e.shape;
    e = Entry{n, m, k, choose_align_shape_uncached(n, m, k, parallel), true};
    return e.shape;
}
u32 align_supported_max_query() { return 25u * 64u * 64u; }

u64 align_trace_slots(u32 n, u32 m, u32 k, AlignShape sh) {
    TraceLayout const tl = ckpt_trace_layout(n, m, k, sh.words_per_lane, sh.lanes_per_job);
    return tl.carry_slots + tl.ckpt_slots;
}

template <class F, int... Ws>
static int with_words_per_lane(u32 words_per_lane, F&& f, std::integer_sequence<int, Ws...>) {
    int rc = (int)hipErrorInvalidValue;
    (void)((words_per_lane == (u32)Ws && ((rc = f(std::integral_constant<int, Ws>{})), true)) || ...);
    return rc;
}
template <class F>
static int with_words_per_lane(u32 words_per_lane, F&& f) {
    return with_words_per_lane(words_per_lane, f, std::integer_sequence<int, 1, 2, 3, 4, 5, 6, 8, 13, 25>{});
}
static u32 log2_lanes(AlignShape shape) {
    u32 log2_g = 0;
    while ((1u << log2_g) < shape.lanes_per_job) ++log2_g;
    return log2_g;
}
static size_t block_lds_bytes(u32 w, u32 jobs_per_wave, u32 queue) {
    return (size_t)7 * 64 * w * sizeof(u64) + (size_t)jobs_per_wave * queue * sizeof(uint2);
}

template <int W>
static int launch_align(hipStream_t s, const u8* d_text, const u64* d_peq, const DevAlignJob* d_jobs, u32 n_jobs, u32 log2_g, bool trace,
                        u64* d_trace, DevAlignOut* d_out, u16* d_lastrow, u32 queue) {
    u32 const jobs_per_wave = 64u >> log2_g;
    u32 const blocks = (n_jobs + jobs_per_wave - 1) / jobs_per_wave;
    size_t const lds_b = block_lds_bytes(W, jobs_per_wave, queue);
    if (trace) {
        (void)hipFuncSetAttribute(reinterpret_cast<const void*>(&ed_trace_block_kernel<W>), hipFuncAttributeMaxDynamicSharedMemorySize, (int)lds_b);
        hipLaunchKernelGGL((ed_trace_block_kernel<W>), dim3(blocks), dim3(64), lds_b, s, d_text, d_peq, d_jobs, n_jobs, log2_g, d_trace, d_out, d_lastrow, queue);
    } else {
        (void)hipFuncSetAttribute(reinterpret_cast<const void*>(&ed_exists_block_kernel<W>), hipFuncAttributeMaxDynamicSharedMemorySize, (int)lds_b);
        hipLaunchKernelGGL((ed_exists_block_kernel<W>), dim3(blocks), dim3(64), lds_b, s, d_text, d_peq, d_jobs, n_jobs, log2_g, d_out, (const u32*)nullptr, queue, (u32*)nullptr);
    }
    return (int)hipGetLastError();
}

template <int W>
static int launch_exists_counted(hipStream_t s, const u8* d_text, const u64* d_peq, const DevAlignJob* d_jobs, u32 max_jobs, u32 log2_g, DevAlignOut* d_out,
                                 const u32* d_n_jobs, u32 max_waves, u32 queue, u32* d_err) {
    u32 const jobs_per_wave = 64u >> log2_g;
    u32 const blocks = std::max(1u, std::min((max_jobs + jobs_per_wave - 1) / jobs_per_wave, max_waves));
    size_t const lds_b = block_lds_bytes(W, jobs_per_wave, queue);
    (void)hipFuncSetAttribute(reinterpret_cast<const void*>(&ed_exists_block_kernel<W>), hipFuncAttributeMaxDynamicSharedMemorySize, (int)lds_b);
    hipLaunchKernelGGL((ed_exists_block_kernel<W>), dim3(blocks), dim3(64), lds_b, s, d_text, d_peq, d_jobs, max_jobs, log2_g, d_out, d_n_jobs, queue, d_err);
    return (int)hipGetLastError();
}
int DeviceApi::align_exists_counted(void* stream, const u8* d_text, const u64* d_peq, const DevAlignJob* d_jobs, u32 max_jobs, const u32* d_n_jobs,
                                    AlignShape shape, u32 max_waves, DevAlignOut* d_out, u32* d_err) {
    if (max_jobs == 0) return 0;
    return with_words_per_lane(shape.words_per_lane, [&](auto w) {
        return launch_exists_counted<decltype(w)::value>((hipStream_t)stream, d_text, d_peq, d_jobs, max_jobs, log2_lanes(shape), d_out, d_n_jobs, max_waves, shape.queue, d_err);
    });
}
AlignShape DeviceApi::shape_holding(u32 nw, i64 width, bool parallel) {
    u32 const m = 64u * nw, k = (u32)(std::max<i64>(width, 1) / 4), n = (u32)((i64)m + std::max<i64>(width, 1) - 2 * (i64)k);
    AlignShape sh = choose_align_shape_uncached(n, m, k, parallel);
    if (sh.queue) { u32 const wider = ring_queue_for(ring_delay(n + (u32)(width / 4), m, k, sh.words_per_lane, sh.lanes_per_job) + 3u); if (wider <= RING_QUEUE_MAX) sh.queue = std::max(sh.queue, wider); }
    return sh;
}

int DeviceApi::align(void* stream, const u8* d_text, const u64* d_peq, const DevAlignJob* d_jobs, u32 n_jobs, AlignShape shape, bool trace,
                     u64* d_trace, DevAlignOut* d_out, u16* d_lastrow) {
    if (n_jobs == 0) return 0;
    u32 const queue = RING_QUEUE_MAX;
    return with_words_per_lane(shape.words_per_lane, [&](auto w) {
        return launch_align<decltype(w)::value>((hipStream_t)stream, d_text, d_peq, d_jobs, n_jobs, log2_lanes(shape), trace, d_trace, d_out, d_lastrow, queue);
    });
}

__global__ void __launch_bounds__(64) lastrow_min_kernel(const u16* __restrict__ lastrow, const DevRowWindow* __restrict__ windows,
                                                         u32 n_windows, DevAlignOut* __restrict__ out) {
    u32 const id = blockIdx.x;
    if (id >= n_windows) return;
    DevRowWindow const w = windows[id];
    u32 const lane = threadIdx.x & 63u;
    const u16* __restrict__ row = lastrow + w.first;
    u32 best = 0xFFFFu, col = 0;
    for (u32 c = lane; c < w.n; c += 64u) {
        u32 const v = c < w.skip ? 0xFFFFu : row[c];
        if (v <= best) { best = v; col = c + 1u; }
    }
    u64 key = ((u64)best << 32) | (u64)(0xFFFFFFFFu - col);
#pragma unroll
    for (int off = 32; off > 0; off >>= 1) {
        u64 const other = __shfl_xor(key, off);
        key = other < key ? other : key;
    }
    if (lane == 0) {
        u32 const v = (u32)(key >> 32), c = 0xFFFFFFFFu - (u32)key;
        DevAlignOut o;
        o.score = (v != 0xFFFFu && v <= w.k) ? v : 0xFFFFFFFFu;
        o.end_col = c;
        out[w.out_index] = o;
    }
}

int DeviceApi::lastrow_min(void* stream, const u16* d_lastrow, const DevRowWindow* d_windows, u32 n_windows, DevAlignOut* d_out) {
    if (n_windows == 0) return 0;
    hipLaunchKernelGGL(lastrow_min_kernel, dim3(n_windows), dim3(64), 0, (hipStream_t)stream, d_lastrow, d_windows, n_windows, d_out);
    return (int)hipGetLastError();
}

constexpr u32 TBW_WORDS = 8, TBW_BLOCKS = 8;
constexpr u32 TBW_REF = 1024;

__global__ void __launch_bounds__(64) ed_traceback_wave_kernel(const u8* __restrict__ text, const u64* __restrict__ peq,
                                                               const u64* __restrict__ trace, const DevTraceJob* __restrict__ jobs,
                                                               u32 n_jobs, u32* __restrict__ cigar, DevTraceOut* __restrict__ out) {
    __shared__ ulonglong2 win[64 * 17];
    __shared__ u32 win_valid[64];
    __shared__ u64 eqm[TBW_WORDS][6];
    __shared__ u8 refs[TBW_REF];
    u32 const lane = threadIdx.x & 63u;
    __builtin_amdgcn_s_setprio(2);
    for (u32 id = blockIdx.x; id < n_jobs; id += gridDim.x) {
    __syncthreads();
    DevTraceJob const job = jobs[id];
    const u8* __restrict__ r = text + job.ref_off;
    u32* __restrict__ slab = cigar + job.cigar_off;
    int const W = (int)job.words_per_lane, R = (int)job.lanes;
    int const n = (int)job.n, m = (int)job.m, k = (int)job.k;
    int const band_hi = n - m + k;
    int const nw = (max(m, 1) + 63) >> 6;
    int const Lg = (nw + W - 1) / W;
    int const pad = Lg * 64 * W - max(m, 1);
    TraceLayout const tl = ckpt_trace_layout(job.n, job.m ? job.m : 1u, job.k, (u32)W, (u32)R);
    int const ring_wait = (int)ring_delay(job.n, job.m ? job.m : 1u, job.k, (u32)W, (u32)R);
    const u32* __restrict__ carry = reinterpret_cast<const u32*>(reinterpret_cast<const ulonglong2*>(trace) + job.trace_off);
    const ulonglong2* __restrict__ ckpt = reinterpret_cast<const ulonglong2*>(trace) + job.trace_off + tl.carry_slots;

    u32 wpos = job.cigar_cap;
    int i = m, j = (int)job.end_col;
    u32 cur_op = 0xFFu, cur_len = 0;
    bool overflow = false;
    auto emit = [&](u32 op, u32 len) {
        if (len == 0) return;
        if (op == cur_op) { cur_len += len; return; }
        if (cur_len) {
            if (wpos == 0) overflow = true;
            else { --wpos; if (lane == 0) slab[wpos] = (cur_len << 4) | cur_op; }
        }
        cur_op = op;
        cur_len = len;
    };
    auto first_block = [&](int w, int diag) {
        int const c_lo = 64 * w - pad + diag;
        return (c_lo >= 0 ? c_lo / 16 : -((-c_lo + 15) / 16)) - 1;
    };

    while (i > 0 && !overflow) {
        if (j == 0) { emit(1u, (u32)i); i = 0; break; }
        int const gw_top = (i - 1 + pad) >> 6;
        int const diag = j - i;
        int const ref_base = max(0, j - 640) & ~15;
        __syncthreads();
        for (u32 x = lane; x < TBW_REF; x += 64u) { int const c = ref_base + (int)x; refs[x] = c < n ? r[c] : (u8)7; }
        __syncthreads();
        {
            int const w = gw_top - (int)(lane / TBW_BLOCKS);
            u32 valid = 0;
            if (w >= 0) {
                int const g = w / W, ww = w - g * W, p = g % R;
                int const b = first_block(w, diag) + (int)(lane % TBW_BLOCKS);
                int const r0 = max(0, 64 * W * g - pad), r1 = 64 * W * (g + 1) - pad;
                int const b_lo = max(0, r0 - k) >> 4;
                int b_hi = min(n - 1, r1 - 1 + band_hi) >> 4;
                if (g + 1 < Lg) b_hi = max(b_hi, max(0, r1 - k) >> 4);
                u64 eq[6];
                int const rs = 64 * w - pad;
                u64 const padmask = rs <= -64 ? ~0ull : rs < 0 ? (1ull << (u32)(-rs)) - 1ull : 0ull;
                {
                    i64 const off = (i64)job.q_off + rs;
#pragma unroll
                    for (u32 sy = 0; sy < 6; ++sy) {
                        u64 v = 0;
                        if (rs > -64) {
                            if (off >= 0) {
                                u64 const a = (u64)off >> 6;
                                u32 const sh = (u32)off & 63u;
                                u64 const lo = peq[a * 6 + sy];
                                u64 const hi = peq[(a + 1) * 6 + sy];
                                v = sh ? (lo >> sh) | (hi << (64 - sh)) : lo;
                            } else v = peq[sy] << (u32)(-off);
                        }
                        eq[sy] = v | padmask;
                    }
                    if (lane % TBW_BLOCKS == 0) {
#pragma unroll
                        for (u32 sy = 0; sy < 6; ++sy) eqm[lane / TBW_BLOCKS][sy] = eq[sy];
                    }
                }
                if (b >= b_lo && b <= b_hi && 16 * b >= ref_base && 16 * b + 16 <= ref_base + (int)TBW_REF) {
                    u64 const slot = ((u64)(b + g + (g / R) * ring_wait) * R + p) * W + ww;
                    ulonglong2 const v = ckpt[slot];
                    u64 pv = v.x, mv = v.y;
                    u32 const cw = carry[slot];
#pragma unroll 4
                    for (u32 sidx = 0; sidx < 16u; ++sidx) {
                        u32 const cb = (cw >> (2u * sidx)) & 3u;
                        u64 const c_hp = cb & 1u, c_hn = cb >> 1;
                        u32 const rsym = refs[16 * b + (int)sidx - ref_base] & 7u;
                        u64 const e = rsym == 0 ? eq[0] : rsym == 1 ? eq[1] : rsym == 2 ? eq[2] : rsym == 3 ? eq[3] : rsym == 4 ? eq[4] : rsym == 5 ? eq[5] : padmask;
                        u64 const x_ = e | mv;
                        u64 const sum = pv + (x_ & pv) + c_hn;
// ... 100 lines not shown
```

floxer_amd/csrc/flx_internal.hpp:

```cpp
#pragma once

#include <atomic>
#include <cstddef>
#include <cstdint>
#include <string>
#include <vector>

#include "../../include/floxer_amd.h"

namespace flx {

using u8 = uint8_t;
using u16 = uint16_t;
using u32 = uint32_t;
using u64 = uint64_t;
using i64 = int64_t;

void set_error(const std::string& msg);

void* host_pool_get(size_t bytes);
void host_pool_put(void* p, size_t bytes);
extern std::atomic<void (*)(void* p, size_t bytes, int pin)> host_pool_pin_hook;
template <class T>
struct PoolAlloc {
// ... 24 lines not shown
    std::vector<u32> kmer_table;
};
constexpr u32 KMER_Q = 8;
inline bool index_has_arrays(HostIndex const& H) { return H.text.size() == H.n && H.sa.size() == H.n && !H.occ[0].empty() && !H.occ[1].empty() && !H.kmer_table.empty(); }

struct DevIndex {
    const OccBlock* occ[2];
    const u32* sa;
    const u8* text;
    const u32* kmer;
    const u32* isa;
    const u64* filter;
    const u64* filter_m;
    u32 filter_k, filter_tmin;
    u32 C[7];
    u32 n;
};

constexpr u32 SCH_POS_MASK = 0xFFFFF;
inline u32 sch_pack(u32 pos, u32 l, u32 u, bool right, bool exact_prefix) {
    return pos | (l << 20) | (u << 23) | ((right ? 1u : 0u) << 26) | ((exact_prefix ? 1u : 0u) << 27);
}

struct DevSeed {
    u64 seq_off;
    u64 stack_off;
    u32 length;
    u32 scheme_off;
    u32 frames_searches;
    u32 id;
    u32 flags;
    u32 pad;
};

struct DevFrame {
    u32 v[16];
};
static_assert(sizeof(DevFrame) == 64, "frame is four 16-byte slots");

struct DevHit { u32 seed, lb, len, errors; u64 key; };
struct DevSeedLeaf { u32 from, length, cls, rank; };
struct DevSeedClass { u32 pos_base, count, scheme_off, frames_searches; };
struct DevSeedRead { u64 pool_fwd, pool_rev; u32 leaf_first, n_leaves, seed_base, class_first, flags, pad; };
struct SeedGen {
    std::vector<DevSeedRead, PoolAlloc<DevSeedRead>> reads;
    std::vector<DevSeedLeaf, PoolAlloc<DevSeedLeaf>> leaves;
    std::vector<DevSeedClass, PoolAlloc<DevSeedClass>> classes;
    std::vector<u64, PoolAlloc<u64>> scheme_table;
    u64 n_seeds = 0;
    u32 max_errors = 0, max_length = 0;
};
struct DevSelStat { u8 useful, raw, flag, excluded; u32 excluded_soft; };
struct DevOutAnchor { u32 seed_index, leaf, ref_id, errors; u64 pos; };

struct DevAlignJob {
    u64 ref_off;
    u64 q_off;
    u64 trace_off;
    u32 n, m, k;
    u32 out_index;
    u64 lastrow_off;
};
struct DevAlignOut { u32 score; u32 end_col; };

struct DevRowWindow { u64 first; u32 n, k; u32 out_index, skip; };

struct DevTraceJob {
    u64 ref_off, q_off, trace_off, cigar_off;
    u32 n, m, lanes, words_per_lane;
    u32 end_col, cigar_cap, out_index;
    u32 k;
};
struct DevTraceOut { u32 begin; u32 cigar_start; u32 cigar_len; u32 pad; };

struct DevMdJob {
    u64 ref_off, cigar_off, md_off;
    u32 n;
    u32 md_cap;
    u32 out_index, pad;
};
struct DevMdOut { u32 len; u32 pad; };
constexpr u64 md_slab_bytes(u64 nm) { return 8 * nm + 6; }
constexpr u32 MD_GRID_CAP = 1u << 16;

struct DevCsJob {
    u64 ref_off, q_off;
    u64 cigar_off, cs_off;
    u32 n, m;
    u32 cs_cap;
    u32 out_index;
};
struct DevCsOut { u32 len; u32 pad; };
static_assert(sizeof(DevCsJob) == 48, "device layout");
constexpr u64 cs_slab_bytes(u64 nm, u64 m, u32 form) { return form == 2u ? m + 3 * nm + 1 : 10 * nm + 7; }
constexpr u32 CS_GRID_CAP = 1u << 16;

struct DevTailJob {
    u64 cigar_off;
    u32 out_index;
    u32 w, x_drop, min_rows;
};
struct DevTailOut { u32 left_rows, left_cols, left_errors, left_words, right_rows, right_cols, right_errors, right_words; };
static_assert(sizeof(DevTailOut) == 32 && sizeof(DevTailOut) == sizeof(flx_tail_result), "one 32-byte result per job");
constexpr u32 TAILS_GRID_CAP = 1u << 16;

struct DevLeftAlignJob {
    u64 ref_off, q_off;
    u64 cigar_off, out_off;
    u32 n, m;
    u32 out_cap;
    u32 out_index;
};
struct DevLeftAlignStat { u32 words_in, letters, gaps, moved; };
constexpr u32 LEFT_ALIGN_GRID_CAP = 1u << 16;

struct DevRealignJob {
    u64 ref_off, q_off;
    u64 cigar_off, out_off;
    u64 trace_off;
    u32 n, m;
    u32 out_cap;
    u32 out_index;
    u32 trace_cap;
    u32 pad;
};
struct DevRealignStat { int32_t score; u32 num_errors; int32_t diag_lo, diag_hi; u32 kept, changed; u64 cells; };
static_assert(sizeof(DevRealignJob) == 64 && sizeof(DevRealignStat) == 32, "device layouts");
struct RealignScores;

struct DevExtendJob {
    u64 text_pos, q_pos;
    u32 ref_limit, row_limit;
    int direction;
    u32 w, x_drop, d_max;
    u32 out_index, pad;
};
struct DevExtendOut { u32 rows, cols, errors, reason; u32 last_d; u32 pad[3]; };
constexpr u32 EXTEND_DEFAULT_WEIGHT = 4, EXTEND_DEFAULT_XDROP = 100, EXTEND_DEFAULT_MAX_ERRORS = 1024;
constexpr u32 EXTEND_MAX_ERRORS = 4093;
constexpr u32 EXTEND_GRID_CAP = 1u << 16;
constexpr u32 EXTEND_MAX_WEIGHT = 0xFFFFu, EXTEND_MAX_XDROP = 1u << 30, EXTEND_MAX_ROWS = (1u << 19) - 1;

struct DevVrAnchor {
    i64 diag_rel;
    u64 seq_start, seq_len;
    u64 q_base;
    u32 tree_base;
    u32 query;
};
struct DevVrNode { u32 parent, from, rows, errors; };
enum : u8 { VR_CLIMBING = 0, VR_DEAD = 1, VR_AT_ROOT = 2, VR_SOLO = 3 };

enum : u32 { VR2_N_JOBS = 0 , VR2_N_CLIMBING = 2, VR2_SMALLEST = 3, VR2_WORD_STEPS = 4, VR2_BYTES = 6, VR2_N_REQ = 8, VR2_DONE = 9,
             VR2_QUEUE_ERR = 11 , VR2_SCALARS = 16 };
struct Vr2Buffers {
    const DevVrAnchor* anchors; const DevVrNode* nodes;
    const u32* q_first;
    u32* node; u8* status;
    u32* a_slot;
    DevAlignJob* jobs; DevAlignOut* outs;
    u32* scalars;
};

struct AlignShape { u32 words_per_lane; u32 lanes_per_job; u32 queue = 0; };

struct TraceLayout { u64 steps, carry_words, carry_slots, ckpt_slots; };
#if defined(__HIPCC__)
#define FLX_HD __host__ __device__
#else
#define FLX_HD
#endif

constexpr u32 RING_QUEUE_MAX = 128;
inline u32 ring_queue_for(u32 delay) {
    if (delay == 0) return 0;
    u32 q = 32;
    while (q < delay + 1u) q *= 2;
    return q;
}
FLX_HD inline void ring_group_blocks(int n, int m, int k, int W, int Lg, int pad, int g, int& b_lo, int& b_hi) {
    int const band_hi = n - m + k;
    int const r0 = 64 * W * g - pad > 0 ? 64 * W * g - pad : 0, r1 = 64 * W * (g + 1) - pad;
    b_lo = (r0 - k > 0 ? r0 - k : 0) >> 4;
    int const hi = r1 - 1 + band_hi < n - 1 ? r1 - 1 + band_hi : n - 1;
    b_hi = hi >> 4;
    if (g + 1 < Lg) { int const next_lo = (r1 - k > 0 ? r1 - k : 0) >> 4; if (next_lo > b_hi) b_hi = next_lo; }
}
FLX_HD inline u32 ring_delay(u32 n, u32 m, u32 k, u32 W, u32 R) {
    if (n == 0 || m == 0 || (u64)n + k < m) return 0;
    int const nw = (int)((m + 63u) / 64u), Lg = (nw + (int)W - 1) / (int)W, pad = Lg * 64 * (int)W - (int)m;
    int delay = 0;
    for (int g = 0; g + (int)R < Lg; ++g) {
        int lo0, hi0, lo1, hi1;
        ring_group_blocks((int)n, (int)m, (int)k, (int)W, Lg, pad, g, lo0, hi0);
        ring_group_blocks((int)n, (int)m, (int)k, (int)W, Lg, pad, g + (int)R, lo1, hi1);
        int const d = hi0 - lo1 + 1 - (int)R;
        if (d > delay) delay = d;
    }
    return (u32)delay;
}
FLX_HD inline u32 lastrow_first_written(u32 n, u32 m, u32 k, u32 W) {
    if (n == 0 || m == 0 || (u64)n + k < m) return n;
    int const nw = (int)((m + 63u) / 64u), Lg = (nw + (int)W - 1) / (int)W, pad = Lg * 64 * (int)W - (int)m;
    int lo, hi;
    ring_group_blocks((int)n, (int)m, (int)k, (int)W, Lg, pad, Lg - 1, lo, hi);
    return (u32)lo * 16u;
}
FLX_HD inline u64 ring_offset(u32 g, u32 R, u32 delay) { return (u64)g + (u64)(g / R) * delay; }
FLX_HD inline u64 ring_steps(u32 n, u32 m, u32 k, u32 W, u32 R) {
    u64 const nw = (m + 63u) / 64u, groups = (nw + W - 1) / W;
    return (n ? (u64)(n - 1) / 16 : 0) + ring_offset((u32)groups - 1u, R, ring_delay(n, m, k, W, R)) + 1;
}
FLX_HD inline TraceLayout ckpt_trace_layout(u32 n, u32 m, u32 k, u32 W, u32 R) {
    TraceLayout l;
    l.steps = ring_steps(n, m, k, W, R);
    l.carry_words = l.steps * R * W;
    l.carry_slots = (l.carry_words + 3) / 4;
    l.ckpt_slots = l.steps * R * W;
    return l;
}
AlignShape choose_align_shape(u32 n, u32 m, u32 k, bool parallel = false);
u64 align_trace_slots(u32 n, u32 m, u32 k, AlignShape sh);
u32 align_supported_max_query();
u32 fm_search_max_keyed_length();

struct KernelTimer;

struct ClearItem { u32* ptr; u32 words; u32 value; };
struct ClearList {
    static constexpr u32 MAX = 8;
    ClearItem item[MAX];
    u32 n = 0;
    bool add(void* p, size_t words, u32 value = 0) {
        if (n == MAX || words > 0xFFFFFFFFull) return false;
        if (words) item[n++] = ClearItem{(u32*)p, (u32)words, value};
        return true;
    }
};
struct PublishItem { const u32* src; u32* dst; u32 words; };
struct PublishList {
    static constexpr u32 MAX = 4;
    PublishItem item[MAX];
    u32 n = 0;
    bool add(const void* src, void* dst, size_t words) {
        if (n == MAX || words > 0xFFFFFFFFull) return false;
        if (words) item[n++] = PublishItem{(const u32*)src, (u32*)dst, (u32)words};
        return true;
    }
};

struct DeviceApi {
    static int clear_stage(void* stream, ClearList const& L);
    static int publish_stage(void* stream, PublishList const& L);
    static int lane_overlap_probe(void* stream, u32 iterations, u32* d_out);
    static int suffix_array(int hip_device, const u8* text, u64 n, u32* out);
    static int index_arrays(int hip_device, const u8* text, u64 n, u32* out_sa, u8* out_bwt0, u8* out_bwt1, OccBlock* out_occ0, OccBlock* out_occ1);
    static int build_peq(void* stream, const u8* d_seq, u64 len, u64* d_peq);
    static int search(void* stream, const DevIndex& idx, const u8* d_seq, const u64* d_scheme, const DevSeed* d_seeds,
                      u32 n_seeds, u32 max_hits_per_seed, DevFrame* d_stack, DevHit* d_hits, u32 hit_cap,
                      u32* d_counters, u32* d_seed_cnt = nullptr);
    static int search_filtered(void* stream, const DevIndex& idx, const u8* d_seq, const u32* d_qpack, const u64* d_scheme, const DevSeed* d_seeds,
                               u32 n_seeds, u32 max_hits_per_seed, u32 frame_levels, DevHit* d_hits, u32 hit_cap, DevHit* d_items, u32 item_cap,
                               u32* d_counters, u32* d_seed_cnt, u32* d_seed_rows, void* d_mailboxes, u32 mailbox_waves, u32 concurrent_launches,
                               bool long_seeds, ClearList clears);
    static size_t mailbox_bytes(u32 waves);
    static size_t derived_bytes(u64 n, u32* filter_k_out);
    static int derive_index(void* stream, DevIndex& idx, u32* d_isa, u64* d_filter, u64* d_filter_mirrored = nullptr);
    static int warm_scratch(void* stream);
    static int build_seeds(void* stream, const DevSeedRead* reads, u32 n_reads, const DevSeedLeaf* leaves, const DevSeedClass* classes, DevSeed* out);
    static int pack_pool(void* stream, const u8* d_seq, u64 len, u32* d_qpack);
    static size_t select_scan_bytes(u32 n_seeds);
    static int select(void* stream, const DevHit* d_hits, const u32* d_counters, u32 hit_cap, u32* d_seed_cnt, u32* d_hit_offset,
                      DevHit* d_grouped, u32 n_seeds, const DevIndex& idx, const u64* d_seq_start, u32 n_ref, u32 hard_cap, u32 soft_cap,
                      bool erase, void* d_stat, u32* d_n_out, u32* d_out_offset, DevOutAnchor* d_out, u32 out_cap, u32* d_rows,
                      u32* d_row_offset, DevOutAnchor* d_sparse, u32 sparse_cap, void* d_scan_tmp, size_t scan_bytes, u32* d_lists);
    static int locate(void* stream, const DevIndex& idx, const u32* d_rows, u32 n, u32* d_out);
    static int align(void* stream, const u8* d_text, const u64* d_peq, const DevAlignJob* d_jobs, u32 n_jobs, AlignShape shape,
                     bool trace, u64* d_trace, DevAlignOut* d_out, u16* d_lastrow = nullptr);
    static int vr2_request(void* stream, Vr2Buffers const& B, u32 n_queries, u32 limit, u32 acct_words, u32 width_cap, u32 parity);
    static int vr2_apply(void* stream, Vr2Buffers const& B, u32 n_anchors, u32* host_scalars);
    static int align_exists_counted(void* stream, const u8* d_text, const u64* d_peq, const DevAlignJob* d_jobs, u32 max_jobs, const u32* d_n_jobs,
                                    AlignShape shape, u32 max_waves, DevAlignOut* d_out, u32* d_err = nullptr);
    static AlignShape shape_holding(u32 nw, i64 width, bool parallel);
    static u64 shape_width_cap(u32 nw, AlignShape sh);
    static int lastrow_min(void* stream, const u16* d_lastrow, const DevRowWindow* d_windows, u32 n_windows, DevAlignOut* d_out);
    static int traceback(void* stream, const u8* d_text, const u64* d_peq, const u64* d_trace, const DevTraceJob* d_jobs, u32 n_jobs,
                         u32* d_cigar, DevTraceOut* d_out);
    static int md_build(void* stream, const u8* d_text, const u32* d_cigar, const DevTraceOut* d_trace_out, const DevMdJob* d_jobs, u32 n_jobs,
                        u8* d_md, DevMdOut* d_out);
    static int cs_build(void* stream, const u8* d_text, const u8* d_query, const u32* d_cigar, const DevTraceOut* d_trace_out, const DevCsJob* d_jobs,
                        u32 n_jobs, u32 form, u8* d_cs, DevCsOut* d_out);
    static int cigar_tails(void* stream, const u32* d_cigar, const DevTraceOut* d_trace_out, const DevTailJob* d_jobs, u32 n_jobs, DevTailOut* d_out);
    static int cigar_left_align(void* stream, const u8* d_text, const u8* d_query, const u32* d_cigar, DevTraceOut* d_trace_out, const DevLeftAlignJob* d_jobs,
                                u32 n_jobs, u32* d_cigar_out, DevLeftAlignStat* d_stats);
    static int cigar_realign(void* stream, const u8* d_text, const u8* d_query, const u32* d_cigar, DevTraceOut* d_trace_out, const DevRealignJob* d_jobs,
                             u32 n_jobs, RealignScores const& scores, u32* d_trace, u32* d_cigar_out, DevRealignStat* d_stats);
    static size_t extend_lds_bytes(u32 d_max);
    static int extend(void* stream, const u8* d_text, const u8* d_query, const DevExtendJob* d_jobs, u32 n_jobs, u32 lds_d, DevExtendOut* d_out);
};

u64 ceil_div(u64 a, u64 b);
u64 fp_aware_ceil(double v);
int32_t saturate_i32(u64 v);
u8 char_to_rank(char c);
char rank_to_char(u8 r);
void reverse_complement(const u8* in, u64 n, u8* out);

struct PexTree {
    std::vector<flx_pex_node> inner, leaves;
    const flx_pex_node& root() const { return inner.empty() ? leaves[0] : inner[0]; }
};
PexTree build_pex_tree(u64 len, u64 k, u64 s, bool bottom_up);

struct SearchDef { std::vector<u32> pi, l, u; };
const std::vector<SearchDef>& optimum_scheme(u32 k);
std::vector<u64> expanded_scheme(u32 k, u32 len);

HostIndex* build_host_index(const u8* concat, const u64* lens, u32 n_refs, int hip_device = -1);
int save_host_index(const HostIndex& idx, const char* path);
HostIndex* load_host_index(const char* path);

}

struct flx_index { flx::HostIndex* host = nullptr; };
```

floxer_amd/csrc/flx_rounds.hip:

```cpp
#include <hip/hip_runtime.h>

#include <algorithm>

#include "flx_internal.hpp"

namespace flx {

namespace {

constexpr u32 VR2_TILE = 256;
constexpr u32 VR2_THREADS = 64;
constexpr u64 VR2_NO_KEY = ~0ull;

__device__ __forceinline__ u64 vr2_word_steps(u32 n, u32 m, u32 k, u32 W) {
    u64 const nw = (m + 63u) / 64u;
    i64 const band_hi = (i64)n - (i64)m + (i64)k;
    u64 total = 0;
    for (i64 g = 0; g * W < (i64)nw; ++g) {
        i64 const r0 = 64 * (i64)W * g, r1 = min((i64)m, r0 + 64 * (i64)W);
        i64 const lo = max((i64)0, r0 - (i64)k), hi = min((i64)n - 1, r1 - 1 + band_hi);
        if (hi >= lo) total += (u64)(hi - lo + 1) * (u64)min((i64)W, (i64)nw - g * W);
    }
    return total;
}

__device__ __forceinline__ u64 vr2_key(u32 node, u64 start, u32 solo) { return ((u64)node << 33) | (start << 1) | solo; }

}

__global__ void __launch_bounds__(VR2_THREADS) vr2_request_kernel(Vr2Buffers B, u32 limit, u32 acct_words, u32 width_cap, u32 parity) {
    __shared__ u64 s_key[VR2_TILE];
    __shared__ u32 s_len[VR2_TILE];
    __shared__ u16 s_val[VR2_TILE];
    __shared__ u8 s_flag[VR2_TILE];
    __shared__ u32 s_jobs[VR2_TILE];
    __shared__ u32 s_count, s_base;
    u32 const tid = threadIdx.x;
    u32 const q = blockIdx.x;
    if (q == 0 && tid == 0) {
        B.scalars[VR2_N_CLIMBING] = 0u; B.scalars[VR2_SMALLEST] = 0xFFFFFFFFu; B.scalars[VR2_DONE] = 0u;
        B.scalars[VR2_N_JOBS + (parity ^ 1u)] = 0u;
    }
    u32 const a0 = B.q_first[q], a1 = B.q_first[q + 1];
    u32* const n_jobs = &B.scalars[VR2_N_JOBS + parity];
    for (u32 tile = a0; tile < a1; tile += VR2_TILE) {
        u32 const n_here = min(VR2_TILE, a1 - tile);
        u32 size = 64;
        while (size < n_here) size <<= 1;
        __syncthreads();
        if (tid == 0) s_count = 0;
        __syncthreads();
        u32 mine = 0;
        u32 tree_base = 0;
        for (u32 t = tid; t < size; t += VR2_THREADS) {
            u64 key = VR2_NO_KEY;
            if (t < n_here) {
                u32 const i = tile + t;
                u8 const st = B.status[i];
                if (st == VR_CLIMBING || st == VR_SOLO) {
                    DevVrAnchor const a = B.anchors[i];
                    u32 const nd_i = B.node[i];
                    DevVrNode const nd = B.nodes[a.tree_base + nd_i];
                    if (nd.rows <= limit) {
                        i64 const start_signed = a.diag_rel + (i64)nd.from - (i64)nd.errors;
                        u64 const start = start_signed > 0 ? (u64)start_signed : 0ull;
                        u64 const base = (u64)nd.rows + 2ull * nd.errors + 1ull;
                        key = vr2_key(nd_i, a.seq_start + start, st == VR_SOLO ? 1u : 0u);
                        s_len[t] = (u32)min(base, a.seq_len - start);
                        ++mine;
                    }
                }
            }
            s_key[t] = key;
            s_val[t] = (u16)t;
        }
        if (mine) atomicAdd(&s_count, mine);
        __syncthreads();
        u32 const cnt = s_count;
        if (cnt == 0) continue;
        DevVrAnchor const a_first = B.anchors[tile];
        tree_base = a_first.tree_base;
        for (u32 k = 2; k <= size; k <<= 1)
            for (u32 j = k >> 1; j > 0; j >>= 1) {
                for (u32 t = tid; t < size; t += VR2_THREADS) {
                    u32 const p = t ^ j;
                    if (p > t) {
                        u64 const x = s_key[t], y = s_key[p];
                        bool const up = (t & k) == 0;
                        if ((x > y) == up) { s_key[t] = y; s_key[p] = x; u16 const v = s_val[t]; s_val[t] = s_val[p]; s_val[p] = v; }
                    }
                }
                __syncthreads();
            }
        for (u32 t = tid; t < cnt; t += VR2_THREADS) {
            u64 const key = s_key[t];
            u32 const node = (u32)(key >> 33);
            if (t > 0 && (u32)(s_key[t - 1] >> 33) == node) continue;
            DevVrNode const nd = B.nodes[tree_base + node];
            u64 const d = max((u64)8, (u64)nd.rows / 8ull);
            u64 const first = (key >> 1) & 0xFFFFFFFFull;
            u64 prev_key = VR2_NO_KEY, prev_bucket = ~0ull, c_lo = 0, c_hi = 0;
            bool prev_solo = false;
            for (u32 j = t; j < cnt && (u32)(s_key[j] >> 33) == node; ++j) {
                u64 const kj = s_key[j];
                bool const solo = kj & 1ull;
                u64 const st = (kj >> 1) & 0xFFFFFFFFull;
                u64 const bucket = (st - first) / d;
                u8 f = 0;
                if (kj != prev_key) {
                    u64 const en = st + s_len[s_val[j]];
                    f = 1;
                    u64 const u_hi = max(c_hi, en);
                    bool const too_wide = (u_hi - c_lo) + 2ull * nd.errors > (u64)nd.rows + width_cap;
                    if (j == t || solo || prev_solo || bucket != prev_bucket || too_wide) { f = 3; c_lo = st; c_hi = en; }
                    else c_hi = u_hi;
                }
                s_flag[j] = f;
                prev_key = kj; prev_bucket = bucket; prev_solo = solo;
            }
        }
        __syncthreads();
        for (u32 t = tid; t < size; t += VR2_THREADS) {
            u32 nj = 0;
            if (t < cnt && (s_flag[t] & 2u)) {
                u32 distinct = 0;
                u64 hi_start = 0, lo_end = 0;
                for (u32 j = t; j < cnt && (j == t || !(s_flag[j] & 2u)); ++j) {
                    if (!(s_flag[j] & 1u)) continue;
                    u64 const st = (s_key[j] >> 1) & 0xFFFFFFFFull, en = st + s_len[s_val[j]];
                    if (distinct == 0) { hi_start = st; lo_end = en; } else { hi_start = max(hi_start, st); lo_end = min(lo_end, en); }
                    ++distinct;
                }
                nj = distinct > 1 && lo_end > hi_start ? 2u : 1u;
            }
            s_jobs[t] = nj;
        }
        __syncthreads();
        {
            u32 const per = size / VR2_THREADS;
            u32 const first = tid * per;
            u32 run = 0;
            for (u32 x = 0; x < per; ++x) run += s_jobs[first + x];
            u32 incl = run;
#pragma unroll
            for (u32 off = 1; off < 64u; off <<= 1) { u32 const up = (u32)__shfl_up((int)incl, off); if (tid >= off) incl += up; }
            u32 at = incl - run;
            for (u32 x = 0; x < per; ++x) { u32 const v = s_jobs[first + x]; s_jobs[first + x] = at; at += v; }
            if (tid == VR2_THREADS - 1u) s_base = incl ? atomicAdd(n_jobs, incl) : 0u;
            __syncthreads();
        }
        u32 const base_slot = s_base;
        u64 steps = 0, bytes = 0;
        u32 n_req = 0;
        for (u32 t = tid; t < cnt; t += VR2_THREADS) {
            if (!(s_flag[t] & 2u)) continue;
            u32 const slot = base_slot + s_jobs[t];
            u32 distinct = 0;
            u64 lo_start = 0, hi_start = 0, lo_end = 0, hi_end = 0;
            u32 last = t;
            for (u32 j = t; j < cnt && (j == t || !(s_flag[j] & 2u)); ++j) {
                last = j;
                if (!(s_flag[j] & 1u)) continue;
                u64 const st = (s_key[j] >> 1) & 0xFFFFFFFFull, en = st + s_len[s_val[j]];
                if (distinct == 0) { lo_start = hi_start = st; lo_end = hi_end = en; }
                else { hi_start = max(hi_start, st); lo_start = min(lo_start, st); lo_end = min(lo_end, en); hi_end = max(hi_end, en); }
                ++distinct;
            }
            DevVrNode const nd = B.nodes[tree_base + (u32)(s_key[t] >> 33)];
            u64 const q_off = a_first.q_base + nd.from;
            u32 code;
            if (distinct == 1) {
                B.jobs[slot] = DevAlignJob{lo_start, q_off, 0, (u32)(hi_end - lo_start), nd.rows, nd.errors, slot, 0};
                code = (slot << 2) | 1u;
                steps += vr2_word_steps((u32)(hi_end - lo_start), nd.rows, nd.errors, acct_words); bytes += (hi_end - lo_start) + nd.rows;
            } else if (lo_end > hi_start) {
                B.jobs[slot] = DevAlignJob{hi_start, q_off, 0, (u32)(lo_end - hi_start), nd.rows, nd.errors, slot, 0};
                B.jobs[slot + 1u] = DevAlignJob{lo_start, q_off, 0, (u32)(hi_end - lo_start), nd.rows, nd.errors, slot + 1u, 0};
                code = (slot << 2) | 3u;
                steps += vr2_word_steps((u32)(lo_end - hi_start), nd.rows, nd.errors, acct_words) + vr2_word_steps((u32)(hi_end - lo_start), nd.rows, nd.errors, acct_words);
                bytes += (lo_end - hi_start) + (hi_end - lo_start) + 2ull * nd.rows;
            } else {
                B.jobs[slot] = DevAlignJob{lo_start, q_off, 0, (u32)(hi_end - lo_start), nd.rows, nd.errors, slot, 0};
                code = (slot << 2) | 2u;
                steps += vr2_word_steps((u32)(hi_end - lo_start), nd.rows, nd.errors, acct_words); bytes += (hi_end - lo_start) + nd.rows;
            }
            for (u32 j = t; j <= last; ++j) B.a_slot[tile + s_val[j]] = code;
            n_req += last - t + 1u;
        }
#pragma unroll
        for (int off = 32; off > 0; off >>= 1) { steps += __shfl_xor(steps, off); bytes += __shfl_xor(bytes, off); n_req += (u32)__shfl_xor((int)n_req, off); }
        if (tid == 0u && n_req) {
            atomicAdd(&B.scalars[VR2_N_REQ], n_req);
            atomicAdd((unsigned long long*)&B.scalars[VR2_WORD_STEPS], (unsigned long long)steps);
            atomicAdd((unsigned long long*)&B.scalars[VR2_BYTES], (unsigned long long)bytes);
        }
    }
}

__global__ void __launch_bounds__(256) vr2_apply_kernel(Vr2Buffers B, u32 n, u32* __restrict__ host_scalars) {
    __shared__ u32 s_cnt[4], s_min[4];
    u32 count = 0, smallest = 0xFFFFFFFFu;
    for (u32 i = blockIdx.x * blockDim.x + threadIdx.x; i < n; i += gridDim.x * blockDim.x) {
        u8 st = B.status[i];
        u32 const code = B.a_slot[i];
        if (code != 0xFFFFFFFFu) {
            B.a_slot[i] = 0xFFFFFFFFu;
            u32 const slot = code >> 2;
            bool const has_a = code & 1u, has_b = code & 2u;
            u8 dec;
            if (has_a && B.outs[slot].score != 0xFFFFFFFFu) dec = 1;
            else if (!has_b) dec = 2;
            else if (B.outs[slot + (has_a ? 1u : 0u)].score == 0xFFFFFFFFu) dec = 2;
            else dec = 0;
            if (dec == 1) {
                u32 const tb = B.anchors[i].tree_base;
                u32 const parent = B.nodes[tb + B.node[i]].parent;
                B.node[i] = parent;
                st = B.nodes[tb + parent].parent == 0xFFFFFFFFu ? VR_AT_ROOT : VR_CLIMBING;
            } else st = dec == 2 ? VR_DEAD : VR_SOLO;
            B.status[i] = st;
        }
        if (st == VR_CLIMBING || st == VR_SOLO) {
            ++count;
            u32 const rows = B.nodes[B.anchors[i].tree_base + B.node[i]].rows;
            smallest = min(smallest, rows);
        }
    }
#pragma unroll
    for (int off = 32; off > 0; off >>= 1) {
        count += (u32)__shfl_xor((int)count, off);
        smallest = min(smallest, (u32)__shfl_xor((int)smallest, off));
    }
    if ((threadIdx.x & 63u) == 0u) { s_cnt[threadIdx.x >> 6] = count; s_min[threadIdx.x >> 6] = smallest; }
    __syncthreads();
    if (threadIdx.x == 0) {
        u32 const c = s_cnt[0] + s_cnt[1] + s_cnt[2] + s_cnt[3], m = min(min(s_min[0], s_min[1]), min(s_min[2], s_min[3]));
        if (c) { atomicAdd(&B.scalars[VR2_N_CLIMBING], c); atomicMin(&B.scalars[VR2_SMALLEST], m); }
        __threadfence();
        if (atomicAdd(&B.scalars[VR2_DONE], 1u) == gridDim.x - 1u && host_scalars) {
            __threadfence();
            for (u32 w = 0; w < VR2_SCALARS; ++w) host_scalars[w] = __hip_atomic_load(&B.scalars[w], __ATOMIC_RELAXED, __HIP_MEMORY_SCOPE_AGENT);
            __threadfence_system();
        }
    }
}

int DeviceApi::vr2_request(void* stream, Vr2Buffers const& B, u32 n_queries, u32 limit, u32 acct_words, u32 width_cap, u32 parity) {
    if (n_queries == 0) return 0;
    hipLaunchKernelGGL(vr2_request_kernel, dim3(n_queries), dim3(VR2_THREADS), 0, (hipStream_t)stream, B, limit, std::max(1u, acct_words), width_cap, parity & 1u);
    return (int)hipGetLastError();
}
int DeviceApi::vr2_apply(void* stream, Vr2Buffers const& B, u32 n_anchors, u32* host_scalars) {
    if (n_anchors == 0) return 0;
    hipLaunchKernelGGL(vr2_apply_kernel, dim3(std::min<u32>((n_anchors + 255) / 256, 1024u)), dim3(256), 0, (hipStream_t)stream, B, n_anchors, host_scalars);
    return (int)hipGetLastError();
}

}
```

floxer_amd/csrc/flx_verify.cpp:

```cpp
#include <algorithm>
#include <chrono>
#include <cstdio>
#include <cstdlib>
#include <cstring>
#include <map>
#include <memory>
#include <mutex>
#include <queue>
#include <string>
#include <tuple>
#include <vector>

#include "flx_fm_core.hpp"
#include "flx_mapq.hpp"
#include "flx_partial.hpp"
#include "flx_pipeline.hpp"
#include "flx_realign.hpp"
#include "flx_select.hpp"
#include "flx_tails.hpp"

namespace flx {

namespace {

// ... 117 lines not shown
            }
            for (size_t c = 0; c < it->second.class_key.size(); ++c) global[it->second.class_key[c]].pos += 2ull * it->second.class_count[c];
        }
        if (gen.max_errors > 3) { set_error("seed errors must be in [0,3] (floxer_cli.cpp:299)"); return FLX_ERR_INVALID; }
        u64 pos = 0;
        for (auto& kv : global) {
            u32 const errors = 3u - (kv.first >> 24), length = kv.first & 0xFFFFFFu;
            auto const e = expanded_scheme(errors, length);
            kv.second.scheme_off = (u32)gen.scheme_table.size();
            kv.second.nsearch = e.empty() ? 0 : (u32)(e.size() / length);
            gen.scheme_table.insert(gen.scheme_table.end(), e.begin(), e.end());
            u64 const n = kv.second.pos;
            kv.second.pos = pos;
            pos += n;
        }
        gen.reads.reserve(reads.size());
        for (size_t r = 0; r < reads.size(); ++r) {
            ReadState const& rs = reads[r];
            TreePlan const& tp = plans.find(rs.tree_ptr)->second;
            gen.reads.push_back(DevSeedRead{rs.pool_off[0], rs.pool_off[1], tp.leaf_first, n_sampled(rs), seed_first[r], (u32)gen.classes.size(), RD->flags[rs.read_index], 0});
            for (size_t c = 0; c < tp.class_key.size(); ++c) {
                auto& g = global[tp.class_key[c]];
                u32 const errors = 3u - (tp.class_key[c] >> 24), length = tp.class_key[c] & 0xFFFFFFu;
                gen.classes.push_back(DevSeedClass{(u32)g.pos, tp.class_count[c], g.scheme_off, (length + errors + 3) | (g.nsearch << 24)});
                g.pos += 2ull * tp.class_count[c];
            }
        }
        gen.n_seeds = n_seeds_total;
    } else build_host_seeds(S, RD);
    return FLX_OK;
}

int search_seeds(Slice& S, Lane* lane, const flx_params* P, const flx_reads* RD) {
    hvec<u8> const& pool = RD->pool;
    const u8* d_pool = RD->d_pool.as<u8>();
    hvec<HostAnchor>& anchors = S.anchors;
    hvec<SeedStats>& sstats = S.sstats;
    if (lane->ctx->read_stats) S.st_local = std::make_unique<Stats>(stats_simulated(lane->ctx->read_stats));
    S.t_slice = std::chrono::steady_clock::now();
    FLX_HIP(hipStreamWaitEvent(lane->stream, RD->peq_event, 0));
    int rc = S.use_gen ? search_seeds_device(lane, d_pool, pool.data(), pool.size(), nullptr, 0, P->search, anchors, sstats, nullptr, 0,
                                       RD->d_pack.ptr ? RD->d_pack.as<u32>() : nullptr, nullptr, &S.gen)
                 : SEARCH_NEEDS_HOST_SEEDS;
    if (rc == SEARCH_NEEDS_HOST_SEEDS) {
        if (S.use_gen) build_host_seeds(S, RD);
        rc = search_seeds_device(lane, d_pool, pool.data(), pool.size(), S.seeds.data(), S.seeds.size(), P->search, anchors, sstats, nullptr, 0,
                                 RD->d_pack.ptr ? RD->d_pack.as<u32>() : nullptr, S.seed_flags.data());
    }
    return rc;
}

void anchors_to_reads(Slice& S) {
    hvec<ReadState>& reads = S.reads;
    hvec<u32> const& seed_first = S.seed_first;
    hvec<HostAnchor> const& anchors = S.anchors;
    hvec<SeedStats> const& sstats = S.sstats;
    u64 const step = S.step;
    auto n_sampled = [&](ReadState const& r) { return S.n_sampled(r); };
    Stats* const st_local = S.st_local.get();
    double const search_ms = S.search_ms = std::chrono::duration<double, std::milli>(std::chrono::steady_clock::now() - S.t_slice).count();
    if (st_local) {
        hvec<SeedStatRow> rows;
        for (size_t r = 0; r < reads.size(); ++r) {
            st_local->at(Stats::QUERY_LENGTHS).add(reads[r].len);
            rows.clear();
            u32 const nl = n_sampled(reads[r]);
            for (u32 si = seed_first[r]; si < seed_first[r + 1]; ++si) {
                flx_pex_node const& leaf = reads[r].tree_ref().leaves[(u64)((si - seed_first[r]) % nl) * step];
                st_local->at(Stats::ERRORS_PER_SEED).add(leaf.num_errors);
                st_local->at(Stats::SEED_LENGTHS).add(leaf.to - leaf.from + 1);
                rows.push_back(SeedStatRow{sstats[si].useful, sstats[si].raw, sstats[si].excluded_soft});
            }
            st_local->at(Stats::SEEDS_PER_QUERY).add(rows.size());
            st_local->add_search_result(rows.data(), rows.size());
            st_local->at(Stats::MS_SEARCH).add((u64)(search_ms / (double)std::max<size_t>(1, reads.size())));
        }
    }
    hvec<AnchorState>& A = S.A;
    A.assign(anchors.size(), AnchorState{});
    u32 rd_i = 0;
    for (size_t a = 0; a < anchors.size(); ++a) {
        u32 const si = anchors[a].seed_index;
        if (si < seed_first[rd_i] || si >= seed_first[rd_i + 1]) {
            if (si >= seed_first[rd_i + 1] && rd_i + 2 < seed_first.size() && si < seed_first[rd_i + 2]) ++rd_i;
            else rd_i = (u32)(std::upper_bound(seed_first.begin(), seed_first.end(), si) - seed_first.begin() - 1);
        }
        u32 const nl = n_sampled(reads[rd_i]), local = si - seed_first[rd_i];
        u8 const orientation = local >= nl ? 1 : 0;
        A[a].read = rd_i;
        A[a].orientation = orientation;
        A[a].leaf = (u32)((u64)(local - (orientation ? nl : 0u)) * step);
        A[a].ref_id = anchors[a].ref_id;
        A[a].pos = anchors[a].pos;
        reads[rd_i].anchor_ids[orientation].push_back((u32)a);
    }
}

void verification_order(Slice& S, const flx_params* P) {
    hvec<ReadState> const& reads = S.reads;
    hvec<hvec<u32>>& exec_order = S.exec_order;
    exec_order.assign(reads.size(), hvec<u32>{});
    for (size_t r = 0; r < reads.size(); ++r) {
        hvec<std::pair<u32, u32>> pkgs;
        hvec<u32> concat;
        for (int o = 0; o < 2; ++o) {
            auto const& ids = reads[r].anchor_ids[o];
            for (size_t i = 0; i < ids.size(); i += P->num_anchors_per_verification_task) {
                u32 const cnt = (u32)std::min<size_t>(P->num_anchors_per_verification_task, ids.size() - i);
                pkgs.emplace_back((u32)concat.size(), cnt);
                concat.insert(concat.end(), ids.begin() + i, ids.begin() + i + cnt);
            }
        }
        for (int pid : package_order((int)pkgs.size()))
            for (u32 j = 0; j < pkgs[pid].second; ++j) exec_order[r].push_back(concat[pkgs[pid].first + j]);
    }
}

u32 start_climb(Slice& S, const flx_params* P) {
    u32 n_climbing = 0;
    for (auto& a : S.A) {
        ReadState const& rs = S.reads[a.read];
        flx_pex_node const& leaf = rs.tree_ref().leaves[a.leaf];
        if (P->direct_full_verification || leaf.parent_id == FLX_NULL_ID) { a.at_root = true; continue; }
        a.node = leaf.parent_id;
        if (rs.tree_ref().inner[a.node].parent_id == FLX_NULL_ID) a.at_root = true;
        n_climbing += !a.at_root;
    }
    return n_climbing;
}

int climb_on_device(Slice& S, Lane* lane, const flx_reads* RD) {
    flx_ctx* ctx = lane->ctx;
    HostIndex const& H = *ctx->hidx;
    hvec<ReadState> const& reads = S.reads;
    hvec<AnchorState>& A = S.A;
    const u8* d_text = ctx->didx.text;
    const u64* const d_peq = RD->d_peq.as<u64>();
    int rc;
    u32 const n = (u32)A.size();
    PhaseTimer vprof("rounds");
    std::map<const PexTree*, u32> tree_base;
    hvec<DevVrNode> nodes;
    for (auto const& kv : S.tree_cache) {
        PexTree const& t = *kv.second;
        tree_base[&t] = (u32)nodes.size();
        for (auto const& nd : t.inner) nodes.push_back(DevVrNode{nd.parent_id, nd.from, nd.to - nd.from + 1, nd.num_errors});
    }
    if (nodes.empty()) nodes.push_back(DevVrNode{0xFFFFFFFFu, 0, 1, 0});
    u32 const n_queries = (u32)(2 * reads.size());
    size_t off = 0;
    auto take = [&](size_t bytes) { size_t const at = off; off += (bytes + 255) & ~(size_t)255; return at; };
    size_t const o_anchors = take((size_t)n * sizeof(DevVrAnchor)), o_nodes = take(nodes.size() * sizeof(DevVrNode)), o_qfirst = take(((size_t)n_queries + 1) * 4),
                 o_node = take((size_t)n * 4), o_status = take(n), o_slot = take((size_t)n * 4), o_scalars = take(VR2_SCALARS * 4), image_bytes = off,
                 o_jobs = take((size_t)n * 2 * sizeof(DevAlignJob)), o_outs = take((size_t)n * 2 * sizeof(DevAlignOut));
    if ((rc = lane->vr.ensure(off))) return rc;
    char* const image = (char*)lane->stage_begin(image_bytes);
    if (!image) return FLX_ERR_NO_DEVICE;
    memset(image, 0, image_bytes);
    DevVrAnchor* const da = (DevVrAnchor*)(image + o_anchors);
    u32* const q_first = (u32*)(image + o_qfirst);
    u32* const h_node = (u32*)(image + o_node);
    u8* const h_status = (u8*)(image + o_status);
    memcpy(image + o_nodes, nodes.data(), nodes.size() * sizeof(DevVrNode));
    memset(image + o_slot, 0xFF, (size_t)n * 4);
    u32 n_climbing = 0, smallest = 0xFFFFFFFFu;
    for (u32 i = 0; i < n; ++i) {
        AnchorState const& a = A[i];
        ReadState const& rs = reads[a.read];
        flx_pex_node const& leaf = rs.tree_ref().leaves[a.leaf];
        u32 const tb = tree_base[rs.tree_ptr];
        u32 const query = 2u * a.read + a.orientation;
        q_first[query + 1]++;
        da[i] = DevVrAnchor{(i64)a.pos - (i64)leaf.from, H.seq_start[a.ref_id], H.seq_len[a.ref_id], rs.pool_off[a.orientation], tb, query};
        bool const climbs = a.alive && !a.at_root;
        h_node[i] = climbs ? a.node : 0u;
        h_status[i] = climbs ? VR_CLIMBING : a.at_root ? VR_AT_ROOT : VR_DEAD;
        if (climbs) { ++n_climbing; smallest = std::min(smallest, nodes[tb + a.node].rows); }
        if (i > 0 && 2u * A[i - 1].read + A[i - 1].orientation > query) { set_error("verification rounds: anchors out of query order"); return FLX_ERR_INTERNAL; }
    }
    for (u32 qi = 0; qi < n_queries; ++qi) q_first[qi + 1] += q_first[qi];
    vprof.mark("anchor-table");
    char* const base = (char*)lane->vr.ptr;
    Vr2Buffers B{};
    B.anchors = (const DevVrAnchor*)(base + o_anchors); B.nodes = (const DevVrNode*)(base + o_nodes); B.q_first = (const u32*)(base + o_qfirst);
    B.node = (u32*)(base + o_node); B.status = (u8*)(base + o_status); B.a_slot = (u32*)(base + o_slot);
    B.jobs = (DevAlignJob*)(base + o_jobs); B.outs = (DevAlignOut*)(base + o_outs); B.scalars = (u32*)(base + o_scalars);
    FLX_HIP(hipMemcpyAsync(base, image, image_bytes, hipMemcpyHostToDevice, lane->stream));
    if (!lane->vr_host_scalars) FLX_HIP(hipHostMalloc((void**)&lane->vr_host_scalars, VR2_SCALARS * 4, hipHostMallocMapped));
    vprof.mark("upload");
    u64 const few_waves = align_few_waves();
    u64 prev_jobs = n_climbing / 2, acc_steps = 0, acc_bytes = 0, acc_req = 0;
    for (u32 round = 0; n_climbing > 0; ++round) {
        u64 const limit = (u64)smallest * round_span_percent() / 100;
        u32 nw_max = 0;
        i64 width_max = 0;
        for (auto const& nd : nodes)
            if (nd.rows >= smallest && nd.rows <= limit) {
                nw_max = std::max(nw_max, (nd.rows + 63u) / 64u);
                width_max = std::max<i64>(width_max, 4 * (i64)nd.errors + 1);
            }
        AlignShape const shape_t = DeviceApi::shape_holding(nw_max, width_max, false), shape_p = DeviceApi::shape_holding(nw_max, width_max, true);
        if (shape_t.words_per_lane == 0 || shape_p.words_per_lane == 0) { set_error("query longer than the supported maximum"); return FLX_ERR_UNSUPPORTED; }
        AlignShape const shape = prev_jobs * shape_t.lanes_per_job / 64 >= few_waves ? shape_t : shape_p;
        u64 const width_cap = DeviceApi::shape_width_cap(nw_max, shape);
        u32 const max_jobs = (u32)std::min<u64>(2ull * n_climbing, 2ull * n);
        int const e1 = DeviceApi::vr2_request(lane->stream, B, n_queries, (u32)std::min<u64>(limit, 0xFFFFFFFFu), shape.words_per_lane,
                                              (u32)std::min<u64>(width_cap, 0xFFFFFFFFull), round);
        if (e1) { set_error(std::string("verification round: ") + hipGetErrorString((hipError_t)e1)); return FLX_ERR_NO_DEVICE; }
        rc = timed_launch(lane, "ed_align_exists", 0, 0, [&] {
            static u32 const exists_waves = [] { const char* e = getenv("FLX_EXISTS_MAX_WAVES"); return (u32)(e ? std::max(64, atoi(e)) : 8192); }();
            return DeviceApi::align_exists_counted(lane->stream, d_text, d_peq, B.jobs, max_jobs, B.scalars + VR2_N_JOBS + (round & 1u), shape, exists_waves, B.outs, B.scalars + VR2_QUEUE_ERR);
        });
        if (rc) return rc;
        int const e2 = DeviceApi::vr2_apply(lane->stream, B, n, lane->vr_host_scalars);
        if (e2) { set_error(std::string("verification round: ") + hipGetErrorString((hipError_t)e2)); return FLX_ERR_NO_DEVICE; }
        if ((rc = lane->sync())) return rc;
        u32 sc[VR2_SCALARS];
        memcpy(sc, lane->vr_host_scalars, sizeof(sc));
        if (sc[VR2_QUEUE_ERR]) { set_error("existence tests: a window did not fit the row buffers"); return FLX_ERR_INTERNAL; }
        u64 ws, by;
        memcpy(&ws, &sc[VR2_WORD_STEPS], 8);
        memcpy(&by, &sc[VR2_BYTES], 8);
        if (ctx->timing) {
            std::lock_guard<std::mutex> g(ctx->mu);
            auto it = ctx->stats.find("ed_align_exists");
            if (it != ctx->stats.end()) { it->second.algorithmic_bytes += by - acc_bytes; it->second.work_units += ws - acc_steps; }
        }
        u64 const round_req = sc[VR2_N_REQ] - acc_req;
        acc_steps = ws; acc_bytes = by; acc_req = sc[VR2_N_REQ];
        S.n_inner_requested += round_req;
        if (round_req == 0 && sc[VR2_N_CLIMBING] >= n_climbing) { set_error("verification rounds do not advance"); return FLX_ERR_INTERNAL; }
        prev_jobs = sc[VR2_N_JOBS + (round & 1u)];
        n_climbing = sc[VR2_N_CLIMBING];
        smallest = sc[VR2_SMALLEST];
        vprof.mark("round");
    }
    if ((rc = lane->wait_idle())) return rc;
    if (n) FLX_HIP(hipMemcpyAsync(image + o_node, base + o_node, o_status + n - o_node, hipMemcpyDeviceToHost, lane->stream));
    if ((rc = lane->sync())) return rc;
    for (u32 i = 0; i < n; ++i) {
        AnchorState& a = A[i];
        if (h_status[i] == VR_DEAD && a.alive && !a.at_root) { a.alive = false; a.node = h_node[i]; }
        else if (h_status[i] == VR_AT_ROOT && !a.at_root) { a.at_root = true; a.node = h_node[i]; }
    }
    vprof.mark("read-back");
    return FLX_OK;
}

int climb_on_host(Slice& S, Lane* lane, const flx_reads* RD, ExistsTimes& times) {
    flx_ctx* ctx = lane->ctx;
    HostIndex const& H = *ctx->hidx;
    hvec<ReadState> const& reads = S.reads;
    hvec<AnchorState>& A = S.A;
    const u8* d_text = ctx->didx.text;
    const u64* const d_peq = RD->d_peq.as<u64>();
    int rc;
    hvec<u32> climbing;
    for (u32 ai = 0; ai < A.size(); ++ai) if (A[ai].alive && !A[ai].at_root) climbing.push_back(ai);
    hvec<AlignRequest> reqs;
    hvec<DevAlignOut> outs;
    auto rows_of = [&](AnchorState const& a) { flx_pex_node const& nd = reads[a.read].tree_ref().inner[a.node]; return nd.to - nd.from + 1; };
    struct Climber { u32 anchor, rows; };
    hvec<Climber> climbers, sel, wait, surv;
    u32 smallest = 0xFFFFFFFFu;
    climbers.reserve(climbing.size());
    for (u32 ai : climbing) { u32 const r = rows_of(A[ai]); climbers.push_back(Climber{ai, r}); smallest = std::min(smallest, r); }
    while (!climbers.empty()) {
        u64 const limit = (u64)smallest * round_span_percent() / 100;
        auto const tb0 = std::chrono::steady_clock::now();
        sel.clear();
        wait.clear();
        surv.clear();
        reqs.clear();
        u32 next_smallest = 0xFFFFFFFFu;
        for (Climber const& c : climbers) {
            if (c.rows <= limit) {
                sel.push_back(c);
                reqs.push_back(window_request(S, H, A[c.anchor], reads[A[c.anchor].read].tree_ref().inner[A[c.anchor].node], 0.0, nullptr));
            } else { wait.push_back(c); next_smallest = std::min(next_smallest, c.rows); }
        }
        times.build_requests += std::chrono::duration<double, std::milli>(std::chrono::steady_clock::now() - tb0).count();
        S.n_inner_requested += reqs.size();
        if ((rc = run_exists_jobs(lane, d_text, d_peq, reqs, outs, times))) return rc;
        for (size_t i = 0; i < outs.size(); ++i) {
            AnchorState& a = A[sel[i].anchor];
            if (outs[i].score == 0xFFFFFFFFu) { a.alive = false; continue; }
            a.node = reads[a.read].tree_ref().inner[a.node].parent_id;
            if (reads[a.read].tree_ref().inner[a.node].parent_id == FLX_NULL_ID) a.at_root = true;
            else { u32 const r = rows_of(a); surv.push_back(Climber{sel[i].anchor, r}); next_smallest = std::min(next_smallest, r); }
        }
        climbers.resize(wait.size() + surv.size());
        std::merge(wait.begin(), wait.end(), surv.begin(), surv.end(), climbers.begin(), [](Climber const& x, Climber const& y) { return x.anchor < y.anchor; });
        smallest = next_smallest;
    }
    return FLX_OK;
}

void interval_pass(Slice& S, const flx_params* P, HostIndex const& H) {
    hvec<ReadState> const& reads = S.reads;
    hvec<AnchorState>& A = S.A;
    hvec<hvec<u32>> const& exec_order = S.exec_order;
    Stats* const st_local = S.st_local.get();
    hvec<AlignRequest>& root_reqs = S.root_reqs;
    hvec<u32>& root_anchor = S.root_anchor;
    hvec<Span>& root_spans = S.root_spans;
    auto add_inner_spans = [&](AnchorState const& a) {
        auto const& tree = reads[a.read].tree_ref();
        flx_pex_node const& leaf = tree.leaves[a.leaf];
        if (P->direct_full_verification || leaf.parent_id == FLX_NULL_ID) return;
        for (u32 nd = leaf.parent_id; tree.inner[nd].parent_id != FLX_NULL_ID; nd = tree.inner[nd].parent_id) {
            st_local->at(Stats::SPAN_INNER).add(window_request(S, H, a, tree.inner[nd], 0.0, nullptr).n);
            if (!a.alive && nd == a.node) break;
        }
    };
    for (size_t r = 0; r < reads.size(); ++r) {
        hvec<VerifiedIntervals> cache[2];
        if (P->use_interval_optimization) { cache[0].resize(H.seq_len.size()); cache[1].resize(H.seq_len.size()); }
        for (u32 ai : exec_order[r]) {
            AnchorState& a = A[ai];
            ReadState const& rs = reads[a.read];
            Span sp;
            AlignRequest const req = window_request(S, H, a, rs.tree_ref().root(), P->extra_verification_ratio, &sp);
            if (P->use_interval_optimization) {
                auto& ivs = cache[a.orientation][a.ref_id];
                if (ivs.contains(trim_both({sp.offset, sp.offset + sp.length}, sp.extra))) {
                    if (st_local) st_local->at(Stats::SPAN_ROOT_AVOIDED).add(sp.length);
                    continue;
                }
                if (st_local) add_inner_spans(a);
                if (!(a.alive && a.at_root)) continue;
                ivs.insert({sp.offset, sp.offset + sp.length});
            } else {
                if (st_local) add_inner_spans(a);
                if (!(a.alive && a.at_root)) continue;
            }
            a.wants_root = true;
            if (st_local) st_local->at(Stats::SPAN_ROOT).add(sp.length);
            root_reqs.push_back(req);
            root_anchor.push_back(ai);
            root_spans.push_back(sp);
        }
    }
}

int align_roots(Slice& S, Lane* lane, const flx_params* P, RunOptions const& R, const flx_reads* RD) {
    flx_ctx* ctx = lane->ctx;
    HostIndex const& H = *ctx->hidx;
    hvec<u8> const& pool = RD->pool;
    hvec<AlignRequest> const& root_reqs = S.root_reqs;
    hvec<Span> const& root_spans = S.root_spans;
    hvec<RootAlignment>& root_res = S.root_res;
    root_res.assign(root_reqs.size(), RootAlignment{});
    int rc;
    if (P->without_cigar) {
        if ((rc = ensure_reversed_text(lane))) return rc;
        {
            std::lock_guard<std::mutex> g(RD->peq_mu);
            if (!RD->rev_built) {
                hvec<u8> qrev(pool.rbegin(), pool.rend());
                take_spare_read_buffer(ctx, 3, RD->d_pool_rev);
                take_spare_read_buffer(ctx, 4, RD->d_peq_rev);
                if ((rc = RD->d_pool_rev.ensure(qrev.size() + 256))) return rc;
                FLX_HIP(hipMemcpyAsync(RD->d_pool_rev.ptr, qrev.data(), qrev.size(), hipMemcpyHostToDevice, lane->stream));
                FLX_HIP(hipMemsetAsync((char*)RD->d_pool_rev.ptr + qrev.size(), 0, 192, lane->stream));
                if ((rc = build_peq(lane, RD->d_pool_rev.as<u8>(), qrev.size(), RD->d_peq_rev))) return rc;
                if (!RD->rev_event) FLX_HIP(hipEventCreateWithFlags(&RD->rev_event, hipEventDisableTiming));
                FLX_HIP(hipEventRecord(RD->rev_event, lane->stream));
                FLX_HIP(hipStreamSynchronize(lane->stream));
                RD->rev_built = true;
            }
        }
        FLX_HIP(hipStreamWaitEvent(lane->stream, RD->rev_event, 0));
        hvec<AlignRequest> rev(root_reqs.size());
        for (size_t i = 0; i < rev.size(); ++i)
            rev[i] = AlignRequest{H.n - root_reqs[i].ref_off - root_reqs[i].n, pool.size() - root_reqs[i].q_off - root_reqs[i].m,
                                  root_reqs[i].n, root_reqs[i].m, root_reqs[i].k};
        hvec<DevAlignOut> outs;
        if ((rc = run_score_jobs(lane, ctx->text_rev.as<u8>() + TEXT_PAD, RD->d_peq_rev.as<u64>(), rev, outs, "ed_align_exists"))) return rc;
        for (size_t i = 0; i < outs.size(); ++i)
            if (outs[i].score != 0xFFFFFFFFu) { root_res[i].exists = true; root_res[i].nm = root_res[i].ed = outs[i].score; root_res[i].start = root_spans[i].offset + (root_reqs[i].n - outs[i].end_col); }
    } else {
        hvec<TraceResult> tres;
        TailParams const tails{split_weight(R.split.error_weight), split_x_drop(R.split.x_drop), split_min_tail_rows(R.split.min_tail_rows)};
        if ((rc = S.trace_windows(lane, RD, root_reqs, tres, R.split.enable ? &tails : nullptr))) return rc;
        for (size_t i = 0; i < tres.size(); ++i)
            if (tres[i].exists)
                root_res[i] = RootAlignment{true, root_spans[i].offset + tres[i].begin, tres[i].nm, tres[i].cigar_off, tres[i].cigar_len, tres[i].md_off, tres[i].md_len, tres[i].tail, tres[i].ed, tres[i].cs_off, tres[i].cs_len};
    }
// ... 597 lines not shown
```

include/floxer_amd.h:

```cpp
#ifndef FLOXER_AMD_H
#define FLOXER_AMD_H

#include <stddef.h>
#include <stdint.h>

#ifdef __cplusplus
extern "C" {
#endif

typedef enum flx_status {
    FLX_OK = 0,
    FLX_ERR_INVALID = -1,
    FLX_ERR_NO_DEVICE = -2,
    FLX_ERR_CAPACITY = -3,
    FLX_ERR_UNSUPPORTED = -4,
    FLX_ERR_INTERNAL = -5,
    FLX_ERR_IO = -6
} flx_status;

const char* flx_last_error(void);
const char* flx_version(void);

uint64_t flx_ceil_div(uint64_t a, uint64_t b);
uint64_t flx_floating_point_error_aware_ceil(double value);
// ... 385 lines not shown
int  flx_grid_caps(uint32_t out[16]);

typedef struct flx_sv flx_sv;
typedef struct flx_sv_options { uint32_t min_length, max_distance, min_support, count_secondary, min_mapq; uint32_t reserved[3]; uint64_t initial_capacity; } flx_sv_options;
typedef struct flx_sv_signature { uint32_t type, side_a, side_b, reserved; int32_t ref_a, ref_b; uint32_t pos_a, q; } flx_sv_signature;
typedef struct flx_sv_cluster { uint32_t type, side_a, side_b, support; int32_t ref_a, ref_b; uint32_t pos_a_min, pos_a_max, q_min, q_median, q_max, reserved; } flx_sv_cluster;
int  flx_sv_create(flx_ctx* ctx, const flx_sv_options* o, flx_sv** out);
int  flx_sv_create_for_lengths(int hip_device, const uint64_t* ref_lens, uint32_t n_refs, const flx_sv_options* o, flx_sv** out);
void flx_sv_free(flx_sv* s);
int  flx_sv_add_records(flx_sv* s, const flx_record* records, uint64_t n, const uint32_t* cigar_words, uint64_t n_words,
                        const uint64_t* read_offsets, uint64_t n_reads);
int  flx_sv_add_run(flx_sv* s, const flx_run* run, const uint64_t* read_offsets, uint64_t n_reads);
int  flx_sv_absorb(flx_sv* into, flx_sv* from);
int  flx_sv_finish(flx_sv* s);
uint64_t flx_sv_num_signatures(const flx_sv* s);
int  flx_sv_copy_signatures(const flx_sv* s, uint64_t from, uint64_t to, flx_sv_signature* out);
uint64_t flx_sv_num_clusters(const flx_sv* s);
int  flx_sv_copy_clusters(const flx_sv* s, flx_sv_cluster* out, uint64_t capacity);
int  flx_sv_host(const uint64_t* ref_lens, uint32_t n_refs, const flx_sv_options* o, const flx_record* records, uint64_t n,
                 const uint32_t* cigar_words, uint64_t n_words, const uint64_t* read_offsets, uint64_t n_reads,
                 flx_sv_signature* out, uint64_t* n_signatures );
int  flx_sv_clusters_host(const flx_sv_options* o, const flx_sv_signature* signatures, uint64_t n, flx_sv_cluster* out,
                          uint64_t* n_clusters );

typedef struct flx_errprof flx_errprof;
typedef struct flx_errprof_options { uint32_t count_secondary, min_mapq, flush_threshold; uint32_t reserved[5]; } flx_errprof_options;
typedef struct flx_errprof_table {
    uint64_t pair_eq[36], pair_x[36], ins_len[64], del_len[64], ins_letter[6], del_letter[6], hp_del[34], hp_ins[34];
    uint64_t pos_match[100], pos_mismatch[100], pos_ins[100], pos_clip[100], pos_del[100], eq_run[256], identity[101], totals[8];
    uint64_t reserved[7];
} flx_errprof_table;
int  flx_errprof_create(flx_ctx* ctx, const flx_errprof_options* o, flx_errprof** out);
int  flx_errprof_create_for_text(int hip_device, const uint8_t* ref_ranks_concat, const uint64_t* ref_lens, uint32_t n_refs,
                                 const flx_errprof_options* o, flx_errprof** out);
void flx_errprof_free(flx_errprof* p);
int  flx_errprof_add_records(flx_errprof* p, const flx_record* records, uint64_t n, const uint32_t* cigar_words, uint64_t n_words,
                             const uint8_t* read_pool, const uint64_t* read_offsets, uint64_t n_reads);
int  flx_errprof_add_run(flx_errprof* p, const flx_run* run, const uint8_t* read_pool, const uint64_t* read_offsets, uint64_t n_reads);
int  flx_errprof_add_run_resident(flx_errprof* p, const flx_run* run, const flx_reads* reads);
int  flx_errprof_absorb(flx_errprof* into, flx_errprof* from);
int  flx_errprof_copy(const flx_errprof* p, flx_errprof_table* out);
int  flx_errprof_host(const uint8_t* ref_ranks_concat, const uint64_t* ref_lens, uint32_t n_refs, const flx_errprof_options* o,
                      const flx_record* records, uint64_t n, const uint32_t* cigar_words, uint64_t n_words, const uint8_t* read_pool,
                      const uint64_t* read_offsets, uint64_t n_reads, flx_errprof_table* table );

typedef struct flx_consensus flx_consensus;
typedef struct flx_consensus_options { uint32_t count_secondary, min_mapq, min_depth, min_count, min_permille, mask_low_depth; uint32_t reserved[2]; } flx_consensus_options;
typedef struct flx_consensus_change { int32_t reference_id; uint32_t position , kind, ref_rank, alt_rank, length, count, cov; uint64_t letters; } flx_consensus_change;
typedef struct flx_consensus_allele { int32_t reference_id; uint32_t position , length, count; uint64_t letters; } flx_consensus_allele;
int  flx_consensus_create(flx_ctx* ctx, const flx_consensus_options* o, flx_consensus** out);
int  flx_consensus_create_for_text(int hip_device, const uint8_t* ref_ranks_concat, const uint64_t* ref_lens, uint32_t n_refs,
                                   const flx_consensus_options* o, flx_consensus** out);
void flx_consensus_free(flx_consensus* p);
int  flx_consensus_add_records(flx_consensus* p, const flx_record* records, uint64_t n, const uint32_t* cigar_words, uint64_t n_words,
                               const uint8_t* read_pool, const uint64_t* read_offsets, uint64_t n_reads);
int  flx_consensus_add_run(flx_consensus* p, const flx_run* run, const uint8_t* read_pool, const uint64_t* read_offsets, uint64_t n_reads);
int  flx_consensus_add_run_resident(flx_consensus* p, const flx_run* run, const flx_reads* reads);
int  flx_consensus_finish(flx_consensus* p);
uint64_t flx_consensus_num_letters(const flx_consensus* p, uint32_t reference_id);
int  flx_consensus_copy_letters(const flx_consensus* p, uint32_t reference_id, char* out, uint64_t capacity);
uint64_t flx_consensus_num_changes(const flx_consensus* p);
int  flx_consensus_copy_changes(const flx_consensus* p, flx_consensus_change* out, uint64_t capacity);
uint64_t flx_consensus_num_alleles(const flx_consensus* p);
int  flx_consensus_copy_alleles(const flx_consensus* p, flx_consensus_allele* out, uint64_t capacity);
int  flx_consensus_geometry(uint32_t out[4]);
int  flx_consensus_host(const uint8_t* ref_ranks_concat, const uint64_t* ref_lens, uint32_t n_refs, const flx_consensus_options* o,
                        const flx_record* records, uint64_t n, const uint32_t* cigar_words, uint64_t n_words, const uint8_t* read_pool,
                        const uint64_t* read_offsets, uint64_t n_reads, uint64_t* letter_offsets, char* letters, uint64_t* n_letters,
                        flx_consensus_change* changes, uint64_t* n_changes, flx_consensus_allele* alleles, uint64_t* n_alleles);

typedef struct flx_variants flx_variants;
typedef struct flx_variants_options {
    uint32_t count_secondary, min_mapq, min_depth, min_qual, max_del, cost_match, cost_mismatch, cost_het, prior_het, prior_hom;
    uint32_t reserved[2];
} flx_variants_options;
typedef struct flx_variant {
    int32_t reference_id;
    uint32_t position , kind, ref_rank, alt_rank, length, ref_count, alt_count, cov, gt, gq, qual, pl[3], reserved;
    uint64_t letters;
} flx_variant;
typedef struct flx_variant_allele { int32_t reference_id; uint32_t position , kind, length, count, reserved; uint64_t letters; } flx_variant_allele;
int  flx_variants_create(flx_ctx* ctx, const flx_variants_options* o, flx_variants** out);
int  flx_variants_create_for_text(int hip_device, const uint8_t* ref_ranks_concat, const uint64_t* ref_lens, uint32_t n_refs,
                                  const flx_variants_options* o, flx_variants** out);
void flx_variants_free(flx_variants* p);
int  flx_variants_add_records(flx_variants* p, const flx_record* records, uint64_t n, const uint32_t* cigar_words, uint64_t n_words,
                              const uint8_t* read_pool, const uint64_t* read_offsets, uint64_t n_reads);
int  flx_variants_add_run(flx_variants* p, const flx_run* run, const uint8_t* read_pool, const uint64_t* read_offsets, uint64_t n_reads);
int  flx_variants_add_run_resident(flx_variants* p, const flx_run* run, const flx_reads* reads);
int  flx_variants_finish(flx_variants* p);
uint64_t flx_variants_num_rows(const flx_variants* p);
int  flx_variants_copy_rows(const flx_variants* p, flx_variant* out, uint64_t capacity);
uint64_t flx_variants_num_alleles(const flx_variants* p);
int  flx_variants_copy_alleles(const flx_variants* p, flx_variant_allele* out, uint64_t capacity);
int  flx_variants_geometry(uint32_t out[4]);
int  flx_variants_genotype(const flx_variants_options* o, uint64_t ref_n, uint64_t alt_n, uint64_t oth, uint32_t out[8]);
int  flx_variants_host(const uint8_t* ref_ranks_concat, const uint64_t* ref_lens, uint32_t n_refs, const flx_variants_options* o,
                       const flx_record* records, uint64_t n, const uint32_t* cigar_words, uint64_t n_words, const uint8_t* read_pool,
                       const uint64_t* read_offsets, uint64_t n_reads, flx_variant* rows, uint64_t* n_rows, flx_variant_allele* alleles,
                       uint64_t* n_alleles);

typedef struct flx_paf flx_paf;
typedef struct flx_paf_summary { uint32_t query_start, query_end, ref_end, matches , mismatches , ins_bases, del_bases, gap_opens; } flx_paf_summary;
typedef struct flx_paf_options { uint32_t write_cigar, write_unmapped, mapq_from_records, skip_secondary; uint32_t reserved[4]; } flx_paf_options;
typedef struct flx_paf_writer flx_paf_writer;
int  flx_paf_create(int hip_device, flx_paf** out);
void flx_paf_free(flx_paf* p);
int  flx_paf_summarize(flx_paf* p, const flx_record* records, uint64_t n, const uint32_t* cigar_words, uint64_t n_words,
                       const uint64_t* read_offsets, uint64_t n_reads, const uint64_t* ref_lens, uint32_t n_refs, flx_paf_summary* out);
int  flx_paf_summarize_host(const flx_record* records, uint64_t n, const uint32_t* cigar_words, uint64_t n_words,
                            const uint64_t* read_offsets, uint64_t n_reads, const uint64_t* ref_lens, uint32_t n_refs, flx_paf_summary* out);
int  flx_paf_open(const char* path, const char* const* ref_ids, const uint64_t* ref_lens, uint32_t n_refs, const flx_paf_options* o,
                  flx_paf_writer** out);
int  flx_paf_write(flx_paf_writer* w, const char* const* read_ids, const uint64_t* read_offsets, const flx_record* records, uint64_t n,
                   const uint32_t* cigar_words, const flx_paf_summary* summaries, const int32_t* scores ,
                   const flx_md_ref* cs_refs , const uint8_t* cs_bytes);
int  flx_paf_close(flx_paf_writer* w);

uint64_t flx_run_num_records(const flx_run* run);
uint64_t flx_run_num_cigar_words(const flx_run* run);
int flx_run_copy(const flx_run* run, flx_record* records, uint32_t* cigar_words, uint8_t* skipped);
void flx_run_free(flx_run* run);

typedef struct flx_kernel_stat {
    char name[32];
    uint64_t launches;
    double device_ms;
    uint64_t algorithmic_bytes;
    uint64_t work_units;
} flx_kernel_stat;
int flx_ctx_enable_kernel_timing(flx_ctx* ctx, int enable);
int flx_ctx_reset_kernel_stats(flx_ctx* ctx);
int flx_ctx_get_kernel_stats(flx_ctx* ctx, flx_kernel_stat* out, uint32_t* n );

typedef struct flx_path_counters {
    uint64_t seeds, seeds_with_anchors, seeds_excluded_by_hard_cap, seeds_selected_on_host, anchors, cursor_extensions;
    uint64_t inner_tests_requested, root_alignments_requested, root_alignments_found, records, reads;
    uint64_t search_reruns;
    uint64_t reserved[4];
} flx_path_counters;
int flx_ctx_get_path_counters(flx_ctx* ctx, flx_path_counters* out);
int flx_ctx_reset_path_counters(flx_ctx* ctx);

typedef struct flx_search_counters {
    uint64_t launches;
    uint64_t subtrees_queued;
    uint64_t lane_handovers;
    uint64_t wave_handovers;
    uint64_t walks_abandoned;
    uint64_t reserved[3];
} flx_search_counters;
int flx_ctx_get_search_counters(flx_ctx* ctx, flx_search_counters* out);

typedef struct flx_climb_anchor { uint32_t read, orientation, leaf, reference_id; uint64_t position; } flx_climb_anchor;
typedef struct flx_climb_options { uint32_t driver, reserved[3]; } flx_climb_options;
int flx_climb_anchors(flx_ctx* ctx, const flx_params* params, const flx_reads* reads, const flx_climb_anchor* anchors, uint64_t n_anchors,
                      const flx_climb_options* options, uint8_t* out_status, uint32_t* out_node, uint64_t* out_requests);

typedef struct flx_derived_info { uint32_t filter_k, filter_tmin, have_isa, have_filter, have_filter_mirrored, reserved[3]; } flx_derived_info;
int flx_ctx_derived_info(flx_ctx* ctx, flx_derived_info* out);
int flx_ctx_copy_derived(flx_ctx* ctx, int which, void* out, uint64_t bytes);

int flx_hw_queue_request(int* requested, int* found);

int flx_ctx_lane_overlap(flx_ctx* ctx, uint32_t n_lanes, uint32_t iterations, float* start_ms, float* stop_ms);

typedef struct flx_stats flx_stats;
int flx_stats_create(const char* input_hint, flx_stats** out);
void flx_stats_free(flx_stats* stats);
int flx_stats_merge(flx_stats* into, const flx_stats* other);
uint64_t flx_stats_num_queries(const flx_stats* stats);
int flx_stats_format(const flx_stats* stats, int toml, char* buf, uint64_t* len);
int flx_ctx_set_stats(flx_ctx* ctx, flx_stats* stats);

typedef struct flx_sam_writer flx_sam_writer;
int flx_sam_open(const char* path , const char* const* ref_ids, const uint64_t* ref_lens, uint32_t n_refs,
                 flx_sam_writer** out);
int flx_sam_write(flx_sam_writer* w, const char* const* read_ids, const uint8_t* read_pool, const uint64_t* read_offsets,
                  const char* const* quals, const flx_record* records, uint64_t n_records, const uint32_t* cigar_words);
int flx_sam_write_tagged(flx_sam_writer* w, const char* const* read_ids, const uint8_t* read_pool, const uint64_t* read_offsets,
                         const char* const* quals, const flx_record* records, uint64_t n_records, const uint32_t* cigar_words,
                         const flx_md_ref* md, const uint8_t* md_bytes);
int flx_sam_write_scored(flx_sam_writer* w, const char* const* read_ids, const uint8_t* read_pool, const uint64_t* read_offsets,
                         const char* const* quals, const flx_record* records, uint64_t n_records, const uint32_t* cigar_words,
                         const flx_md_ref* md, const uint8_t* md_bytes, const int32_t* scores);
int flx_sam_write_cs(flx_sam_writer* w, const char* const* read_ids, const uint8_t* read_pool, const uint64_t* read_offsets,
                     const char* const* quals, const flx_record* records, uint64_t n_records, const uint32_t* cigar_words,
                     const flx_md_ref* md, const uint8_t* md_bytes, const int32_t* scores, const flx_md_ref* cs_refs, const uint8_t* cs_bytes);
int flx_sam_close(flx_sam_writer* w);
int flx_sam_set_threads(flx_sam_writer* w, uint32_t n_threads);
int flx_sam_set_mapq(flx_sam_writer* w, int from_records);
int flx_sam_set_sa(flx_sam_writer* w, int on);
int flx_sam_open_sorted(const char* path , const char* spill_path, int hip_device, int write_index,
                        const char* const* ref_ids, const uint64_t* ref_lens, uint32_t n_refs, flx_sam_writer** out);

int flx_sim_genome(uint64_t length, uint64_t seed, uint8_t* out_ranks);
int flx_sim_genome_repeats(uint64_t length, uint64_t seed, uint8_t* out_ranks);
int flx_sim_reads(const uint8_t* genome_concat, const uint64_t* chrom_lens, uint32_t n_chrom, uint64_t n_reads, uint32_t base_len,
                  double error_rate, double revcomp_fraction, uint64_t seed, uint8_t* out_pool, uint64_t pool_capacity,
                  uint64_t* out_offsets, uint32_t* out_chrom, uint64_t* out_pos, uint8_t* out_reverse);

#ifdef __cplusplus
}
#endif
#endif
```

Measured before the change: 188,600.

## Run union verification jobs lazily in a second exists launch

When two anchor windows overlap, verification rounds used to align both the intersection job and the union job. Now the first exists launch runs only the first job of each cluster, via an order list. Clusters whose intersection fails are appended to a second list, and only those get the union job in a second, counted launch. This is meant to skip union alignments whenever the intersection already finds a hit. In exchange it adds an extra kernel launch per round, atomics, packed 16-bit counters in the prefix scan, and new diagnostic counters. The old behaviour stays available through an environment variable.

```diff
diff --git a/floxer_amd/__init__.py b/floxer_amd/__init__.py
--- a/floxer_amd/__init__.py
+++ b/floxer_amd/__init__.py
@@ -197,6 +197,11 @@
         sc = capi.SearchCounters()
         check(lib().flx_ctx_get_search_counters(self.h, C.byref(sc)))
         return {n: int(getattr(sc, n)) for n, _ in capi.SearchCounters._fields_ if n != "reserved"}
+
+    def rounds_counters(self):
+        rc = capi.RoundsCounters()
+        check(lib().flx_ctx_get_rounds_counters(self.h, C.byref(rc)))
+        return {n: int(getattr(rc, n)) for n, _ in capi.RoundsCounters._fields_ if n != "reserved"}
 
     def derived_info(self):
         di = capi.DerivedInfo()
diff --git a/floxer_amd/capi.py b/floxer_amd/capi.py
--- a/floxer_amd/capi.py
+++ b/floxer_amd/capi.py
@@ -276,6 +276,11 @@
 
 class SearchCounters(C.Structure):
     _fields_ = [(n, C.c_uint64) for n in ("launches", "subtrees_queued", "lane_handovers", "wave_handovers", "walks_abandoned")] + [("reserved", C.c_uint64 * 3)]
+
+
+class RoundsCounters(C.Structure):
+    _fields_ = [(n, C.c_uint64) for n in ("rounds", "jobs", "clusters", "second_launch_jobs", "unions_spared", "unions_needed", "unions_spared_word_steps",
+                                          "unions_needed_word_steps", "word_steps_requested")] + [("reserved", C.c_uint64 * 3)]
 
 
 class ClimbAnchor(C.Structure):
@@ -314,7 +319,7 @@
     "flx_align_shapes", "flx_align_reads_gaps", "flx_align_reads_resident_gaps", "flx_align_batch_gaps", "flx_left_align", "flx_left_align_batch",
     "flx_realign", "flx_realign_batch", "flx_align_batch_realign", "flx_ctx_get_realign_counters", "flx_align_reads_realign",
     "flx_align_reads_resident_realign", "flx_run_copy_scores", "flx_sam_write_scored",
-    "flx_ctx_get_search_counters", "flx_climb_anchors", "flx_ctx_derived_info", "flx_ctx_copy_derived",
+    "flx_ctx_get_search_counters", "flx_ctx_get_rounds_counters", "flx_climb_anchors", "flx_ctx_derived_info", "flx_ctx_copy_derived",
     "flx_hw_queue_request", "flx_ctx_lane_overlap",
     "flx_align_reads_cs", "flx_align_reads_resident_cs", "flx_run_num_cs_bytes", "flx_run_copy_cs", "flx_align_batch_cs", "flx_cs", "flx_cs_batch",
     "flx_sam_write_cs",
@@ -628,7 +633,8 @@
     L.flx_ctx_get_path_counters.argtypes = [C.c_void_p, C.POINTER(PathCounters)]
     L.flx_ctx_reset_path_counters.argtypes = [C.c_void_p]
     L.flx_ctx_get_search_counters.argtypes = [C.c_void_p, C.POINTER(SearchCounters)]
-    L.flx_climb_anchors.argtypes = [C.c_void_p, C.POINTER(Params), C.c_void_p, C.c_void_p, C.c_uint64, C.POINTER(ClimbOptions), u8p, u32p, u64p]
+    L.flx_ctx_get_rounds_counters.argtypes = [C.c_void_p, C.POINTER(RoundsCounters)]
+    L.flx_climb_anchors.argtypes =[C.c_void_p, C.POINTER(Params), C.c_void_p, C.c_void_p, C.c_uint64, C.POINTER(ClimbOptions), u8p, u32p, u64p]
     L.flx_ctx_derived_info.argtypes = [C.c_void_p, C.POINTER(DerivedInfo)]
     L.flx_ctx_copy_derived.argtypes = [C.c_void_p, C.c_int, C.c_void_p, C.c_uint64]
     L.flx_hw_queue_request.argtypes = [C.POINTER(C.c_int), C.POINTER(C.c_int)]
diff --git a/floxer_amd/csrc/flx_capi.cpp b/floxer_amd/csrc/flx_capi.cpp
--- a/floxer_amd/csrc/flx_capi.cpp
+++ b/floxer_amd/csrc/flx_capi.cpp
@@ -302,6 +302,7 @@
     std::lock_guard<std::mutex> g(ctx->mu);
     ctx->path = flx_path_counters{};
     ctx->search = flx_search_counters{};
+    ctx->rounds = flx_rounds_counters{};
     ctx->realign = flx_realign_counters{};
     return FLX_OK;
 }
@@ -315,6 +316,12 @@
     if (!ctx || !out) { set_error("null argument"); return FLX_ERR_INVALID; }
     std::lock_guard<std::mutex> g(ctx->mu);
     *out = ctx->search;
+    return FLX_OK;
+}
+int flx_ctx_get_rounds_counters(flx_ctx* ctx, flx_rounds_counters* out) {
+    if (!ctx || !out) { set_error("null argument"); return FLX_ERR_INVALID; }
+    std::lock_guard<std::mutex> g(ctx->mu);
+    *out = ctx->rounds;
     return FLX_OK;
 }
 
diff --git a/floxer_amd/csrc/flx_context.hpp b/floxer_amd/csrc/flx_context.hpp
--- a/floxer_amd/csrc/flx_context.hpp
+++ b/floxer_amd/csrc/flx_context.hpp
@@ -119,6 +119,7 @@
     flx_path_counters path{};
     flx_realign_counters realign{};
     flx_search_counters search{};
+    flx_rounds_counters rounds{};
     flx_stats* read_stats = nullptr;
 
     std::mutex lane_mu;
diff --git a/floxer_amd/csrc/flx_device.hip b/floxer_amd/csrc/flx_device.hip
--- a/floxer_amd/csrc/flx_device.hip
+++ b/floxer_amd/csrc/flx_device.hip
@@ -45,7 +45,8 @@
 template <int W, bool TRACE>
 __device__ __forceinline__ void ed_block_body(const u8* __restrict__ text, const u64* __restrict__ peq, const DevAlignJob* __restrict__ jobs, u32 n_jobs,
                                               u32 log2_r, DevAlignOut* __restrict__ out, u32 blk, u64* __restrict__ lds_eq,
-                                              u64* __restrict__ trace, u16* __restrict__ lastrow, u32 queue, u32* __restrict__ err) {
+                                              u64* __restrict__ trace, u16* __restrict__ lastrow, u32 queue, u32* __restrict__ err,
+                                              const u32* __restrict__ order = nullptr, u32* __restrict__ second = nullptr, u32* __restrict__ n_second = nullptr) {
     u32 const lane = lane_id();
     u32 const R = 1u << log2_r;
     u32 const p = lane & (R - 1u);
@@ -53,11 +54,19 @@
     u32 const job_id = blk * jobs_per_wave + (lane >> log2_r);
     bool valid = job_id < n_jobs;
     DevAlignJob job;
-    if (valid) job = jobs[job_id];
+    if (valid) job = jobs[order ? order[job_id] : job_id];
     else { job.ref_off = 0; job.q_off = 0; job.trace_off = 0; job.n = 0; job.m = 1; job.k = 0; job.out_index = 0; }
+    bool const has_union = !TRACE && second && job.trace_off == VR2_JOB_HAS_UNION;
+    auto store_out = [&](u32 score, u32 end_col) {
+        DevAlignOut o;
+        o.score = score;
+        o.end_col = end_col;
+        out[job.out_index] = o;
+        if (has_union && score == 0xFFFFFFFFu) second[atomicAdd(n_second, 1u)] = job.out_index + 1u;
+    };
     int const n = (int)job.n, m = (int)job.m, k = (int)job.k;
     if (valid && (n == 0 || n + k < m)) {
-        if (p == 0u) { DevAlignOut o; o.score = (n == 0 && m <= k) ? (u32)m : 0xFFFFFFFFu; o.end_col = 0u; out[job.out_index] = o; }
+        if (p == 0u) store_out((n == 0 && m <= k) ? (u32)m : 0xFFFFFFFFu, 0u);
         valid = false;
     }
     int const nw = (m + 63) >> 6;
@@ -67,7 +76,7 @@
     int delay = valid ? (int)ring_delay((u32)n, (u32)m, (u32)k, (u32)W, R) : 0;
     if (delay > 0 && (u32)delay + 1u > queue) {
         if (err && p == 0u) atomicOr(err, 1u);
-        if (p == 0u) { DevAlignOut o; o.score = 0xFFFFFFFFu; o.end_col = 0u; out[job.out_index] = o; }
+        if (p == 0u) store_out(0xFFFFFFFFu, 0u);
         valid = false;
         delay = 0;
     }
@@ -256,24 +265,20 @@
         }
     }
     flush();
-    if (valid && has_group && g == Lg - 1) {
-        DevAlignOut o;
-        o.score = best <= k ? (u32)best : 0xFFFFFFFFu;
-        o.end_col = (u32)best_col;
-        out[job.out_index] = o;
-    }
+    if (valid && has_group && g == Lg - 1) store_out(best <= k ? (u32)best : 0xFFFFFFFFu, (u32)best_col);
 }
 
 
 template <int W>
 __global__ void __launch_bounds__(64, (W <= 2 ? 4 : W <= 5 ? 3 : W <= 8 ? 2 : 1)) ed_exists_block_kernel(const u8* __restrict__ text, const u64* __restrict__ peq,
                                                              const DevAlignJob* __restrict__ jobs, u32 n_jobs, u32 log2_r,
-                                                             DevAlignOut* __restrict__ out, const u32* __restrict__ n_jobs_dev, u32 queue, u32* __restrict__ err) {
+                                                             DevAlignOut* __restrict__ out, const u32* __restrict__ n_jobs_dev, u32 queue, u32* __restrict__ err,
+                                                             const u32* __restrict__ order, u32* __restrict__ second, u32* __restrict__ n_second) {
     extern __shared__ __attribute__((aligned(16))) u64 lds_eq[];
     if (n_jobs_dev) n_jobs = min(n_jobs, *n_jobs_dev);
     u32 const jobs_per_wave = 64u >> log2_r;
     for (u32 blk = blockIdx.x; blk * jobs_per_wave < n_jobs; blk += gridDim.x)
-        ed_block_body<W, false>(text, peq, jobs, n_jobs, log2_r, out, blk, lds_eq, nullptr, nullptr, queue, err);
+        ed_block_body<W, false>(text, peq, jobs, n_jobs, log2_r, out, blk, lds_eq, nullptr, nullptr, queue, err, order, second, n_second);
 }
 
 template <int W>
@@ -381,26 +386,29 @@
         hipLaunchKernelGGL((ed_trace_block_kernel<W>), dim3(blocks), dim3(64), lds_b, s, d_text, d_peq, d_jobs, n_jobs, log2_g, d_trace, d_out, d_lastrow, queue);
     } else {
         (void)hipFuncSetAttribute(reinterpret_cast<const void*>(&ed_exists_block_kernel<W>), hipFuncAttributeMaxDynamicSharedMemorySize, (int)lds_b);
-        hipLaunchKernelGGL((ed_exists_block_kernel<W>), dim3(blocks), dim3(64), lds_b, s, d_text, d_peq, d_jobs, n_jobs, log2_g, d_out, (const u32*)nullptr, queue, (u32*)nullptr);
+        hipLaunchKernelGGL((ed_exists_block_kernel<W>), dim3(blocks), dim3(64), lds_b, s, d_text, d_peq, d_jobs, n_jobs, log2_g, d_out, (const u32*)nullptr, queue, (u32*)nullptr,
+                           (const u32*)nullptr, (u32*)nullptr, (u32*)nullptr);
     }
     return (int)hipGetLastError();
 }
 
 template <int W>
 static int launch_exists_counted(hipStream_t s, const u8* d_text, const u64* d_peq, const DevAlignJob* d_jobs, u32 max_jobs, u32 log2_g, DevAlignOut* d_out,
-                                 const u32* d_n_jobs, u32 max_waves, u32 queue, u32* d_err) {
+                                 const u32* d_n_jobs, u32 max_waves, u32 queue, u32* d_err, const u32* d_order, u32* d_second, u32* d_n_second) {
     u32 const jobs_per_wave = 64u >> log2_g;
     u32 const blocks = std::max(1u, std::min((max_jobs + jobs_per_wave - 1) / jobs_per_wave, max_waves));
     size_t const lds_b = block_lds_bytes(W, jobs_per_wave, queue);
     (void)hipFuncSetAttribute(reinterpret_cast<const void*>(&ed_exists_block_kernel<W>), hipFuncAttributeMaxDynamicSharedMemorySize, (int)lds_b);
-    hipLaunchKernelGGL((ed_exists_block_kernel<W>), dim3(blocks), dim3(64), lds_b, s, d_text, d_peq, d_jobs, max_jobs, log2_g, d_out, d_n_jobs, queue, d_err);
+    hipLaunchKernelGGL((ed_exists_block_kernel<W>), dim3(blocks), dim3(64), lds_b, s, d_text, d_peq, d_jobs, max_jobs, log2_g, d_out, d_n_jobs, queue, d_err,
+                       d_order, d_second, d_n_second);
     return (int)hipGetLastError();
 }
 int DeviceApi::align_exists_counted(void* stream, const u8* d_text, const u64* d_peq, const DevAlignJob* d_jobs, u32 max_jobs, const u32* d_n_jobs,
-                                    AlignShape shape, u32 max_waves, DevAlignOut* d_out, u32* d_err) {
+                                    AlignShape shape, u32 max_waves, DevAlignOut* d_out, u32* d_err, const u32* d_order, u32* d_second, u32* d_n_second) {
     if (max_jobs == 0) return 0;
     return with_words_per_lane(shape.words_per_lane, [&](auto w) {
-        return launch_exists_counted<decltype(w)::value>((hipStream_t)stream, d_text, d_peq, d_jobs, max_jobs, log2_lanes(shape), d_out, d_n_jobs, max_waves, shape.queue, d_err);
+        return launch_exists_counted<decltype(w)::value>((hipStream_t)stream, d_text, d_peq, d_jobs, max_jobs, log2_lanes(shape), d_out, d_n_jobs, max_waves, shape.queue, d_err,
+                                                         d_order, d_second, d_n_second);
     });
 }
 AlignShape DeviceApi::shape_holding(u32 nw, i64 width, bool parallel) {
diff --git a/floxer_amd/csrc/flx_internal.hpp b/floxer_amd/csrc/flx_internal.hpp
--- a/floxer_amd/csrc/flx_internal.hpp
+++ b/floxer_amd/csrc/flx_internal.hpp
@@ -200,7 +200,10 @@
 enum : u8 { VR_CLIMBING = 0, VR_DEAD = 1, VR_AT_ROOT = 2, VR_SOLO = 3 };
 
 enum : u32 { VR2_N_JOBS = 0 , VR2_N_CLIMBING = 2, VR2_SMALLEST = 3, VR2_WORD_STEPS = 4, VR2_BYTES = 6, VR2_N_REQ = 8, VR2_DONE = 9,
-             VR2_QUEUE_ERR = 11 , VR2_SCALARS = 16 };
+             VR2_QUEUE_ERR = 11 ,
+             VR2_N_FIRST = 12 , VR2_N_SECOND = 14 , VR2_UNIONS_SPARED = 16, VR2_UNIONS_NEEDED = 17,
+             VR2_SPARED_STEPS = 18, VR2_NEEDED_STEPS = 20, VR2_SCALARS = 32 };
+constexpr u64 VR2_JOB_HAS_UNION = 1;
 struct Vr2Buffers {
     const DevVrAnchor* anchors; const DevVrNode* nodes;
     const u32* q_first;
@@ -208,6 +211,8 @@
     u32* a_slot;
     DevAlignJob* jobs; DevAlignOut* outs;
     u32* scalars;
+    u32* order1;
+    u32* order2;
 };
 
 struct AlignShape { u32 words_per_lane; u32 lanes_per_job; u32 queue = 0; };
@@ -326,9 +331,10 @@
     static int align(void* stream, const u8* d_text, const u64* d_peq, const DevAlignJob* d_jobs, u32 n_jobs, AlignShape shape,
                      bool trace, u64* d_trace, DevAlignOut* d_out, u16* d_lastrow = nullptr);
     static int vr2_request(void* stream, Vr2Buffers const& B, u32 n_queries, u32 limit, u32 acct_words, u32 width_cap, u32 parity);
-    static int vr2_apply(void* stream, Vr2Buffers const& B, u32 n_anchors, u32* host_scalars);
+    static int vr2_apply(void* stream, Vr2Buffers const& B, u32 n_anchors, u32* host_scalars, u32 acct_words, u32 parity);
     static int align_exists_counted(void* stream, const u8* d_text, const u64* d_peq, const DevAlignJob* d_jobs, u32 max_jobs, const u32* d_n_jobs,
-                                    AlignShape shape, u32 max_waves, DevAlignOut* d_out, u32* d_err = nullptr);
+                                    AlignShape shape, u32 max_waves, DevAlignOut* d_out, u32* d_err = nullptr, const u32* d_order = nullptr,
+                                    u32* d_second = nullptr, u32* d_n_second = nullptr);
     static AlignShape shape_holding(u32 nw, i64 width, bool parallel);
     static u64 shape_width_cap(u32 nw, AlignShape sh);
     static int lastrow_min(void* stream, const u16* d_lastrow, const DevRowWindow* d_windows, u32 n_windows, DevAlignOut* d_out);
diff --git a/floxer_amd/csrc/flx_rounds.hip b/floxer_amd/csrc/flx_rounds.hip
--- a/floxer_amd/csrc/flx_rounds.hip
+++ b/floxer_amd/csrc/flx_rounds.hip
@@ -34,15 +34,17 @@
     __shared__ u16 s_val[VR2_TILE];
     __shared__ u8 s_flag[VR2_TILE];
     __shared__ u32 s_jobs[VR2_TILE];
-    __shared__ u32 s_count, s_base;
+    __shared__ u32 s_count, s_base, s_base1;
     u32 const tid = threadIdx.x;
     u32 const q = blockIdx.x;
     if (q == 0 && tid == 0) {
         B.scalars[VR2_N_CLIMBING] = 0u; B.scalars[VR2_SMALLEST] = 0xFFFFFFFFu; B.scalars[VR2_DONE] = 0u;
         B.scalars[VR2_N_JOBS + (parity ^ 1u)] = 0u;
+        B.scalars[VR2_N_FIRST + (parity ^ 1u)] = 0u; B.scalars[VR2_N_SECOND + (parity ^ 1u)] = 0u;
     }
     u32 const a0 = B.q_first[q], a1 = B.q_first[q + 1];
     u32* const n_jobs = &B.scalars[VR2_N_JOBS + parity];
+    u32* const n_first = &B.scalars[VR2_N_FIRST + parity];
     for (u32 tile = a0; tile < a1; tile += VR2_TILE) {
         u32 const n_here = min(VR2_TILE, a1 - tile);
         u32 size = 64;
@@ -140,21 +142,22 @@
             u32 const per = size / VR2_THREADS;
             u32 const first = tid * per;
             u32 run = 0;
-            for (u32 x = 0; x < per; ++x) run += s_jobs[first + x];
+            for (u32 x = 0; x < per; ++x) { u32 const v = s_jobs[first + x]; run += v | (v ? 0x10000u : 0u); }
             u32 incl = run;
 #pragma unroll
             for (u32 off = 1; off < 64u; off <<= 1) { u32 const up = (u32)__shfl_up((int)incl, off); if (tid >= off) incl += up; }
             u32 at = incl - run;
-            for (u32 x = 0; x < per; ++x) { u32 const v = s_jobs[first + x]; s_jobs[first + x] = at; at += v; }
-            if (tid == VR2_THREADS - 1u) s_base = incl ? atomicAdd(n_jobs, incl) : 0u;
+            for (u32 x = 0; x < per; ++x) { u32 const v = s_jobs[first + x]; s_jobs[first + x] = at; at += v | (v ? 0x10000u : 0u); }
+            if (tid == VR2_THREADS - 1u) { s_base = incl ? atomicAdd(n_jobs, incl & 0xFFFFu) : 0u; s_base1 = incl ? atomicAdd(n_first, incl >> 16) : 0u; }
             __syncthreads();
         }
-        u32 const base_slot = s_base;
+        u32 const base_slot = s_base, base_first = s_base1;
         u64 steps = 0, bytes = 0;
         u32 n_req = 0;
         for (u32 t = tid; t < cnt; t += VR2_THREADS) {
             if (!(s_flag[t] & 2u)) continue;
-            u32 const slot = base_slot + s_jobs[t];
+            u32 const slot = base_slot + (s_jobs[t] & 0xFFFFu);
+            B.order1[base_first + (s_jobs[t] >> 16)] = slot;
             u32 distinct = 0;
             u64 lo_start = 0, hi_start = 0, lo_end = 0, hi_end = 0;
             u32 last = t;
@@ -174,7 +177,7 @@
                 code = (slot << 2) | 1u;
                 steps += vr2_word_steps((u32)(hi_end - lo_start), nd.rows, nd.errors, acct_words); bytes += (hi_end - lo_start) + nd.rows;
             } else if (lo_end > hi_start) {
-                B.jobs[slot] = DevAlignJob{hi_start, q_off, 0, (u32)(lo_end - hi_start), nd.rows, nd.errors, slot, 0};
+                B.jobs[slot] = DevAlignJob{hi_start, q_off, VR2_JOB_HAS_UNION, (u32)(lo_end - hi_start), nd.rows, nd.errors, slot, 0};
                 B.jobs[slot + 1u] = DevAlignJob{lo_start, q_off, 0, (u32)(hi_end - lo_start), nd.rows, nd.errors, slot + 1u, 0};
                 code = (slot << 2) | 3u;
                 steps += vr2_word_steps((u32)(lo_end - hi_start), nd.rows, nd.errors, acct_words) + vr2_word_steps((u32)(hi_end - lo_start), nd.rows, nd.errors, acct_words);
@@ -197,9 +200,32 @@
     }
 }
 
-__global__ void __launch_bounds__(256) vr2_apply_kernel(Vr2Buffers B, u32 n, u32* __restrict__ host_scalars) {
+__global__ void __launch_bounds__(256) vr2_apply_kernel(Vr2Buffers B, u32 n, u32* __restrict__ host_scalars, u32 acct_words, u32 parity) {
     __shared__ u32 s_cnt[4], s_min[4];
     u32 count = 0, smallest = 0xFFFFFFFFu;
+    {
+        u32 const n_first = B.scalars[VR2_N_FIRST + parity];
+        u32 spared = 0, needed = 0;
+        u64 spared_steps = 0, needed_steps = 0;
+        for (u32 c = blockIdx.x * blockDim.x + threadIdx.x; c < n_first; c += gridDim.x * blockDim.x) {
+            u32 const s = B.order1[c];
+            if (B.jobs[s].trace_off != VR2_JOB_HAS_UNION) continue;
+            DevAlignJob const u = B.jobs[s + 1u];
+            u64 const steps = vr2_word_steps(u.n, u.m, u.k, acct_words);
+            if (B.outs[s].score != 0xFFFFFFFFu) { ++spared; spared_steps += steps; } else { ++needed; needed_steps += steps; }
+        }
+        if (__any(spared | needed)) {
+#pragma unroll
+            for (int off = 32; off > 0; off >>= 1) {
+                spared += (u32)__shfl_xor((int)spared, off); needed += (u32)__shfl_xor((int)needed, off);
+                spared_steps += __shfl_xor(spared_steps, off); needed_steps += __shfl_xor(needed_steps, off);
+            }
+            if ((threadIdx.x & 63u) == 0u) {
+                if (spared) { atomicAdd(&B.scalars[VR2_UNIONS_SPARED], spared); atomicAdd((unsigned long long*)&B.scalars[VR2_SPARED_STEPS], (unsigned long long)spared_steps); }
+                if (needed) { atomicAdd(&B.scalars[VR2_UNIONS_NEEDED], needed); atomicAdd((unsigned long long*)&B.scalars[VR2_NEEDED_STEPS], (unsigned long long)needed_steps); }
+            }
+        }
+    }
     for (u32 i = blockIdx.x * blockDim.x + threadIdx.x; i < n; i += gridDim.x * blockDim.x) {
         u8 st = B.status[i];
         u32 const code = B.a_slot[i];
@@ -250,9 +276,10 @@
     hipLaunchKernelGGL(vr2_request_kernel, dim3(n_queries), dim3(VR2_THREADS), 0, (hipStream_t)stream, B, limit, std::max(1u, acct_words), width_cap, parity & 1u);
     return (int)hipGetLastError();
 }
-int DeviceApi::vr2_apply(void* stream, Vr2Buffers const& B, u32 n_anchors, u32* host_scalars) {
+int DeviceApi::vr2_apply(void* stream, Vr2Buffers const& B, u32 n_anchors, u32* host_scalars, u32 acct_words, u32 parity) {
     if (n_anchors == 0) return 0;
-    hipLaunchKernelGGL(vr2_apply_kernel, dim3(std::min<u32>((n_anchors + 255) / 256, 1024u)), dim3(256), 0, (hipStream_t)stream, B, n_anchors, host_scalars);
+    hipLaunchKernelGGL(vr2_apply_kernel, dim3(std::min<u32>((n_anchors + 255) / 256, 1024u)), dim3(256), 0, (hipStream_t)stream, B, n_anchors, host_scalars,
+                       std::max(1u, acct_words), parity & 1u);
     return (int)hipGetLastError();
 }
 
diff --git a/floxer_amd/csrc/flx_verify.cpp b/floxer_amd/csrc/flx_verify.cpp
--- a/floxer_amd/csrc/flx_verify.cpp
+++ b/floxer_amd/csrc/flx_verify.cpp
@@ -293,7 +293,8 @@
     auto take = [&](size_t bytes) { size_t const at = off; off += (bytes + 255) & ~(size_t)255; return at; };
     size_t const o_anchors = take((size_t)n * sizeof(DevVrAnchor)), o_nodes = take(nodes.size() * sizeof(DevVrNode)), o_qfirst = take(((size_t)n_queries + 1) * 4),
                  o_node = take((size_t)n * 4), o_status = take(n), o_slot = take((size_t)n * 4), o_scalars = take(VR2_SCALARS * 4), image_bytes = off,
-                 o_jobs = take((size_t)n * 2 * sizeof(DevAlignJob)), o_outs = take((size_t)n * 2 * sizeof(DevAlignOut));
+                 o_jobs = take((size_t)n * 2 * sizeof(DevAlignJob)), o_outs = take((size_t)n * 2 * sizeof(DevAlignOut)),
+                 o_order1 = take((size_t)n * 4), o_order2 = take((size_t)n * 4);
     if ((rc = lane->vr.ensure(off))) return rc;
     char* const image = (char*)lane->stage_begin(image_bytes);
     if (!image) return FLX_ERR_NO_DEVICE;
@@ -326,6 +327,10 @@
     B.anchors = (const DevVrAnchor*)(base + o_anchors); B.nodes = (const DevVrNode*)(base + o_nodes); B.q_first = (const u32*)(base + o_qfirst);
     B.node = (u32*)(base + o_node); B.status = (u8*)(base + o_status); B.a_slot = (u32*)(base + o_slot);
     B.jobs = (DevAlignJob*)(base + o_jobs); B.outs = (DevAlignOut*)(base + o_outs); B.scalars = (u32*)(base + o_scalars);
+    B.order1 = (u32*)(base + o_order1); B.order2 = (u32*)(base + o_order2);
+    bool const eager_union = [] { const char* e = getenv("FLX_ROUNDS_EAGER_UNION"); return e && atoi(e) != 0; }();
+    bool const debug = getenv("FLX_ALIGN_DEBUG") != nullptr;
+    flx_rounds_counters rc_sum{};
     FLX_HIP(hipMemcpyAsync(base, image, image_bytes, hipMemcpyHostToDevice, lane->stream));
     if (!lane->vr_host_scalars) FLX_HIP(hipHostMalloc((void**)&lane->vr_host_scalars, VR2_SCALARS * 4, hipHostMallocMapped));
     vprof.mark("upload");
@@ -350,10 +355,16 @@
         if (e1) { set_error(std::string("verification round: ") + hipGetErrorString((hipError_t)e1)); return FLX_ERR_NO_DEVICE; }
         rc = timed_launch(lane, "ed_align_exists", 0, 0, [&] {
             static u32 const exists_waves = [] { const char* e = getenv("FLX_EXISTS_MAX_WAVES"); return (u32)(e ? std::max(64, atoi(e)) : 8192); }();
-            return DeviceApi::align_exists_counted(lane->stream, d_text, d_peq, B.jobs, max_jobs, B.scalars + VR2_N_JOBS + (round & 1u), shape, exists_waves, B.outs, B.scalars + VR2_QUEUE_ERR);
+            u32 const parity = round & 1u;
+            if (eager_union) return DeviceApi::align_exists_counted(lane->stream, d_text, d_peq, B.jobs, max_jobs, B.scalars + VR2_N_JOBS + parity, shape, exists_waves, B.outs, B.scalars + VR2_QUEUE_ERR);
+            int const e = DeviceApi::align_exists_counted(lane->stream, d_text, d_peq, B.jobs, (max_jobs + 1u) / 2u, B.scalars + VR2_N_FIRST + parity, shape, exists_waves, B.outs,
+                                                          B.scalars + VR2_QUEUE_ERR, B.order1, B.order2, B.scalars + VR2_N_SECOND + parity);
+            if (e) return e;
+            return DeviceApi::align_exists_counted(lane->stream, d_text, d_peq, B.jobs, (max_jobs + 3u) / 4u, B.scalars + VR2_N_SECOND + parity, shape, exists_waves, B.outs,
+                                                   B.scalars + VR2_QUEUE_ERR, B.order2);
         });
         if (rc) return rc;
-        int const e2 = DeviceApi::vr2_apply(lane->stream, B, n, lane->vr_host_scalars);
+        int const e2 = DeviceApi::vr2_apply(lane->stream, B, n, lane->vr_host_scalars, shape.words_per_lane, round);
         if (e2) { set_error(std::string("verification round: ") + hipGetErrorString((hipError_t)e2)); return FLX_ERR_NO_DEVICE; }
         if ((rc = lane->sync())) return rc;
         u32 sc[VR2_SCALARS];
@@ -368,6 +379,25 @@
             if (it != ctx->stats.end()) { it->second.algorithmic_bytes += by - acc_bytes; it->second.work_units += ws - acc_steps; }
         }
         u64 const round_req = sc[VR2_N_REQ] - acc_req;
+        {
+            u64 spared_steps, needed_steps;
+            memcpy(&spared_steps, &sc[VR2_SPARED_STEPS], 8);
+            memcpy(&needed_steps, &sc[VR2_NEEDED_STEPS], 8);
+            if (debug)
+                fprintf(stderr, "[rounds] round %u rows %u..%llu W %u R %u jobs %u clusters %u second launch %u word-steps %llu; unions so far: spared %u (%llu word-steps) needed %u (%llu)\n",
+                        round, smallest, (unsigned long long)limit, shape.words_per_lane, shape.lanes_per_job, sc[VR2_N_JOBS + (round & 1u)], sc[VR2_N_FIRST + (round & 1u)],
+                        sc[VR2_N_SECOND + (round & 1u)], (unsigned long long)(ws - acc_steps), sc[VR2_UNIONS_SPARED], (unsigned long long)spared_steps, sc[VR2_UNIONS_NEEDED],
+                        (unsigned long long)needed_steps);
+            rc_sum.rounds += 1;
+            rc_sum.jobs += sc[VR2_N_JOBS + (round & 1u)];
+            rc_sum.clusters += sc[VR2_N_FIRST + (round & 1u)];
+            rc_sum.second_launch_jobs += sc[VR2_N_SECOND + (round & 1u)];
+            rc_sum.unions_spared = sc[VR2_UNIONS_SPARED];
+            rc_sum.unions_needed = sc[VR2_UNIONS_NEEDED];
+            rc_sum.unions_spared_word_steps = spared_steps;
+            rc_sum.unions_needed_word_steps = needed_steps;
+            rc_sum.word_steps_requested = ws;
+        }
         acc_steps = ws; acc_bytes = by; acc_req = sc[VR2_N_REQ];
         S.n_inner_requested += round_req;
         if (round_req == 0 && sc[VR2_N_CLIMBING] >= n_climbing) { set_error("verification rounds do not advance"); return FLX_ERR_INTERNAL; }
@@ -375,6 +405,19 @@
         n_climbing = sc[VR2_N_CLIMBING];
         smallest = sc[VR2_SMALLEST];
         vprof.mark("round");
+    }
+    if (debug)
+        fprintf(stderr, "[rounds] climb of %u anchors%s: rounds %llu jobs %llu clusters %llu second-launch jobs %llu word-steps requested %llu, of unions spared %llu (%llu unions), of unions needed %llu (%llu unions)\n",
+                n, eager_union ? " (eager unions)" : "", (unsigned long long)rc_sum.rounds, (unsigned long long)rc_sum.jobs, (unsigned long long)rc_sum.clusters,
+                (unsigned long long)rc_sum.second_launch_jobs, (unsigned long long)rc_sum.word_steps_requested, (unsigned long long)rc_sum.unions_spared_word_steps,
+                (unsigned long long)rc_sum.unions_spared, (unsigned long long)rc_sum.unions_needed_word_steps, (unsigned long long)rc_sum.unions_needed);
+    {
+        std::lock_guard<std::mutex> g(ctx->mu);
+        flx_rounds_counters& t = ctx->rounds;
+        t.rounds += rc_sum.rounds; t.jobs += rc_sum.jobs; t.clusters += rc_sum.clusters; t.second_launch_jobs += rc_sum.second_launch_jobs;
+        t.unions_spared += rc_sum.unions_spared; t.unions_needed += rc_sum.unions_needed;
+        t.unions_spared_word_steps += rc_sum.unions_spared_word_steps; t.unions_needed_word_steps += rc_sum.unions_needed_word_steps;
+        t.word_steps_requested += rc_sum.word_steps_requested;
     }
     if ((rc = lane->wait_idle())) return rc;
     if (n) FLX_HIP(hipMemcpyAsync(image + o_node, base + o_node, o_status + n - o_node, hipMemcpyDeviceToHost, lane->stream));
diff --git a/include/floxer_amd.h b/include/floxer_amd.h
--- a/include/floxer_amd.h
+++ b/include/floxer_amd.h
@@ -561,6 +561,18 @@
 } flx_search_counters;
 int flx_ctx_get_search_counters(flx_ctx* ctx, flx_search_counters* out);
 
+typedef struct flx_rounds_counters {
+    uint64_t rounds;
+    uint64_t jobs, clusters;
+    uint64_t second_launch_jobs;
+    uint64_t unions_spared;
+    uint64_t unions_needed;
+    uint64_t unions_spared_word_steps, unions_needed_word_steps;
+    uint64_t word_steps_requested;
+    uint64_t reserved[3];
+} flx_rounds_counters;
+int flx_ctx_get_rounds_counters(flx_ctx* ctx, flx_rounds_counters* out);
+
 typedef struct flx_climb_anchor { uint32_t read, orientation, leaf, reference_id; uint64_t position; } flx_climb_anchor;
 typedef struct flx_climb_options { uint32_t driver, reserved[3]; } flx_climb_options;
 int flx_climb_anchors(flx_ctx* ctx, const flx_params* params, const flx_reads* reads, const flx_climb_anchor* anchors, uint64_t n_anchors,
```

New measurement: 185,600. 1.6% lower.
